# VITA-Group/Open-L2O

Hardware: AMD Instinct MI355X
Metric: unroll-steps/sec (batch x params x T), L2O-DM on Quadratic d=128 (higher is better)
Workload: dtype f32

## Files before the change

include/l2o_abi.h:

```cpp
#ifndef L2O_ABI_H_
#define L2O_ABI_H_

#include <stddef.h>
#include <stdint.h>

#ifdef __cplusplus
extern "C" {
#endif

#define L2O_ABI_VERSION 15

#define L2O_OK 0
#define L2O_ERR_ARG (-1)
#define L2O_ERR_UNSUPPORTED (-2)
#define L2O_ERR_HIP (-3)
#define L2O_ERR_TIMEOUT (-4)

#define L2O_NET_CW 0
#define L2O_NET_RNNPROP 1

#define L2O_PRE_IDENTITY 0
#define L2O_PRE_LOGSIGN 1
#define L2O_PRE_FC_ELU 2

#define L2O_PROB_SIMPLE 0
#define L2O_PROB_QUADRATIC 1
#define L2O_PROB_LASSO 2
#define L2O_PROB_RASTRIGIN 3
#define L2O_PROB_SQUARE_COS 4
#define L2O_PROB_MLP 5
#define L2O_PROB_MNIST_CONV 6
#define L2O_PROB_CIFAR_CONV 7
#define L2O_PROB_LENET 8
#define L2O_PROB_CONFOCAL 9

typedef struct l2o_net_cfg {
  int32_t kind;
  int32_t preprocess;
  int32_t n_layers;
  int32_t hidden;
  int32_t tanh_output;
  int32_t reserved;
  double scale;
  double logsign_k;
  double beta1;
  double beta2;
  uint64_t options;
} l2o_net_cfg;

#define L2O_PROB_W_SHARED 1
#define L2O_PROB_FG_TWO_PASS 2

typedef struct l2o_problem {
  int32_t kind;
  int32_t B_local;
  int32_t B_global;
  int32_t D;
  int32_t M;
  int32_t flags;
  double l1;
  double alpha;
  const float* W;
  const float* y;
  const float* C;
  const float* x_scale;
} l2o_problem;

int l2o_abi_version(void);
const char* l2o_last_error(void);
const char* l2o_build_id(void);
int l2o_last_unroll_form(void);
#define L2O_FORM_UNROLL 1
#define L2O_FORM_UNROLL_PAIR 2
#define L2O_FORM_UNROLL_LDS 5
#define L2O_FORM_UNROLL_CU 6
#define L2O_FORM_UNROLL_CU8 7
#define L2O_FORM_MLP_UNROLL 8
#define L2O_FORM_MLP_UNROLL_HIER 9
#define L2O_FORM_MLP_UNROLL_GENERIC 10
#define L2O_FORM_MLP_XCD 11
#define L2O_FORM_CONFOCAL_UNROLL 12
int l2o_last_unroll_variant(void);
#define L2O_VARIANT(ch, hist, exact, fast, kr, nv) \
  ((ch) | ((hist) << 4) | ((exact) << 5) | ((fast) << 6) | ((kr) << 8) | ((nv) << 12))
#define L2O_VARIANT_CH(w) ((w) & 0xf)
#define L2O_VARIANT_HIST(w) (((w) >> 4) & 1)
#define L2O_VARIANT_EXACT(w) (((w) >> 5) & 1)
#define L2O_VARIANT_FAST(w) (((w) >> 6) & 1)
#define L2O_VARIANT_KR(w) (((w) >> 8) & 7)
#define L2O_VARIANT_NV(w) (((w) >> 12) & 3)

#define L2O_OPT_PAIR 0
#define L2O_OPT_PAIR_PLAIN_STORES 1
#define L2O_OPT_UNROLL_CU 2
#define L2O_OPT_FG_TWO_PASS 3
#define L2O_OPT_MLP_GENERIC 4
#define L2O_OPT_BWD_BLOCKS 5
#define L2O_OPT_BWD_KERNEL 6
#define L2O_OPT_MLP_UNROLL 7
#define L2O_OPT_MLP_XCD_WAVES 8
#define L2O_OPT_EXACT_GATES 9
#define L2O_OPT_WPACK_NO_CLEAR 10
#define L2O_OPT_MLP_HIER 11
#define L2O_OPT_ONE_LDS 12
#define L2O_OPT_PAIR_FAST_LOAD 13
#define L2O_OPT_COUNT_ 14
#define L2O_OPT_FIELD_(o) ((o) == L2O_OPT_ONE_LDS ? L2O_OPT_BWD_BLOCKS : (o) == L2O_OPT_PAIR_FAST_LOAD ? 15 : (o))
#define L2O_OPTW(o, v) ((uint64_t)(8u | ((unsigned)(v) & 7u)) << (4 * L2O_OPT_FIELD_(o)))
#define L2O_OPTW_BWD_BLOCKS(n) ((uint64_t)((n) > 4095 ? 4095 : (n)) << 48)

int32_t l2o_coresident_workgroups(void* scratch, void* stream);

size_t l2o_wpack_floats(const l2o_net_cfg* cfg);
int l2o_wpack_host(const l2o_net_cfg* cfg,
                   const float* w_gates1, const float* b_gates1,
                   const float* w_gates2, const float* b_gates2,
                   const float* w_lin, const float* b_lin,
                   const float* w_fc, const float* b_fc,
                   float* wpack_out);

size_t l2o_state_floats(int64_t B, int64_t D);
int l2o_state_pack(const float* h1, const float* c1, const float* h2, const float* c2,
                   float* st, int64_t B, int64_t D, void* stream);
int l2o_state_unpack(const float* st, float* h1, float* c1, float* h2, float* c2,
                     int64_t B, int64_t D, void* stream);

int l2o_problem_fg(const l2o_problem* prob, const float* x ,
                   float* f_part , float* g ,
                   void* stream);

int l2o_problem_hvp(const l2o_problem* prob, const float* x , const float* u ,
                    float* out , float* scratch, void* stream);

#define L2O_MLP_GENERIC 1
typedef struct l2o_mlp {
  int32_t n_in;
  int32_t n_hidden;
  int32_t n_out;
  int32_t batch;
  int32_t activation;
  int32_t n_data;
  int32_t flags;
  int32_t reserved;
  const float* images;
  const int32_t* labels;
} l2o_mlp;
size_t l2o_mlp_scratch_floats(const l2o_mlp* mlp);
int l2o_mlp_fg(const l2o_mlp* mlp, const int32_t* indices ,
               const float* w1 , const float* b1 ,
               const float* w2 , const float* b2 ,
               float* loss , float* gw1, float* gb1, float* gw2, float* gb2,
               float* scratch , void* stream);

typedef struct l2o_mlp_deep {
  int32_t n_in, n_out, batch, activation , n_data, n_hidden_layers;
  int32_t hidden[3];
  int32_t reserved;
  const float* images;
  const int32_t* labels;
} l2o_mlp_deep;
size_t l2o_mlp_deep_scratch_floats(const l2o_mlp_deep* mlp);
int l2o_mlp_deep_fg(const l2o_mlp_deep* mlp, const int32_t* indices , const float* const* w,
                    float* loss , float* const* g, float* scratch , void* stream);

typedef struct l2o_mnist_conv {
  int32_t batch;
  int32_t n_data;
  int32_t batch_norm;
  int32_t flags;
  const float* images;
  const int32_t* labels;
} l2o_mnist_conv;
size_t l2o_mnist_conv_scratch_floats(const l2o_mnist_conv* conv);
int l2o_mnist_conv_fg(const l2o_mnist_conv* conv, const int32_t* indices ,
                      const float* const* w, float* loss , float* const* g,
                      float* scratch , void* stream);

typedef struct l2o_cifar_conv {
  int32_t batch;
  int32_t n_data;
  int32_t batch_norm;
  int32_t flags;
  const float* images;
  const int32_t* labels;
} l2o_cifar_conv;
size_t l2o_cifar_conv_scratch_floats(const l2o_cifar_conv* conv);
int l2o_cifar_conv_fg(const l2o_cifar_conv* conv, const int32_t* indices ,
                      const float* const* w, float* loss , float* const* g,
                      float* scratch , void* stream);

typedef struct l2o_lenet {
  int32_t batch;
  int32_t n_data;
  int32_t batch_norm;
  int32_t flags;
  const float* images;
  const int32_t* labels;
} l2o_lenet;
size_t l2o_lenet_scratch_floats(const l2o_lenet* net);
int l2o_lenet_fg(const l2o_lenet* net, const int32_t* indices ,
                 const float* const* w, float* loss , float* const* g,
                 float* scratch , void* stream);

typedef struct l2o_confocal {
  int32_t batch;
  int32_t num_points;
  int32_t roi[3];
  int32_t inference;
  int32_t flags;
  const float* img;
} l2o_confocal;
size_t l2o_confocal_scratch_floats(const l2o_confocal* net);
int l2o_confocal_fg(const l2o_confocal* net, const float* const* theta, const float* const* sim,
                    float* loss , float* const* g,
                    float* scratch , void* stream);

int l2o_mlp_unroll_supported(const l2o_net_cfg* cfg, const l2o_mlp* mlp, void* stream);
size_t l2o_mlp_unroll_workspace_bytes(const l2o_mlp* mlp);
int l2o_mlp_unroll(const l2o_net_cfg* cfg, const float* wpack , const l2o_mlp* mlp,
                   const int32_t* indices, float* const* x, float* const* st, float* const* m, float* const* v,
                   const float* const* x_scale, int32_t T, int32_t step0, float* fx, void* workspace, void* stream);
typedef struct l2o_mlp_hist {
  float* st[4];
  float* g[4];
  float* m[4];
  float* v[4];
} l2o_mlp_hist;
int l2o_mlp_unroll_record(const l2o_net_cfg* cfg, const float* wpack , const l2o_mlp* mlp,
                          const int32_t* indices, float* const* x, float* const* st, float* const* m, float* const* v,
                          const float* const* x_scale, int32_t T, int32_t step0, float* fx, const l2o_mlp_hist* hist,
                          void* workspace, void* stream);

typedef struct l2o_mlp_instance {
  const int32_t* indices;
  float* x[4];
  float* st[4];
  float* m[4];
  float* v[4];
  const float* x_scale[4];
  float* fx;
} l2o_mlp_instance;
int l2o_mlp_unroll_multi_supported(const l2o_net_cfg* cfg, const l2o_mlp* mlp, int32_t n_inst, void* stream);
size_t l2o_mlp_unroll_multi_workspace_bytes(const l2o_mlp* mlp, int32_t n_inst);
int l2o_mlp_unroll_multi(const l2o_net_cfg* cfg, const float* wpack , const l2o_mlp* mlp,
                         const l2o_mlp_instance* inst , int32_t n_inst, int32_t T, int32_t step0,
                         void* workspace, void* stream);
int l2o_mlp_unroll_multi_record(const l2o_net_cfg* cfg, const float* wpack , const l2o_mlp* mlp,
                                const l2o_mlp_instance* inst , int32_t n_inst, int32_t T, int32_t step0,
                                const l2o_mlp_hist* hist , void* workspace, void* stream);

int l2o_cwlstm_step(const l2o_net_cfg* cfg, const float* wpack ,
                    const float* g , float* m, float* v ,
                    double pow1, double pow2,
                    float* st , float* x ,
                    int64_t B, int64_t D, void* stream);

typedef struct l2o_gen_net {
  int32_t n_layers;
  int32_t hidden[3];
  int32_t in_dim;
  int32_t direct_inputs;
  const float* w_gates[3];
  const float* b_gates[3];
  const float* w_lin;
  const float* b_lin;
  const float* w_fc;
  const float* b_fc;
} l2o_gen_net;
size_t l2o_gen_state_floats(const l2o_gen_net* net, int64_t N);
int l2o_cwlstm_step_generic(const l2o_net_cfg* cfg ,
                            const l2o_gen_net* net, const float* g ,
                            const float* m_tilde ,
                            float* m, float* v ,
                            double pow1, double pow2, float* state ,
                            float* x , int64_t N, void* stream);

typedef struct l2o_gen_bwd_io {
  const float* g;
  const float* m;
  const float* v;
  const float* st_prev;
  const float* dx_next;
  const float* carry_in;
  float* carry_out;
  float* act[3];
  float* dz[3];
  float* tc;
  float* h_last;
  float* dd;
  float* feats;
  float* du;
  float* dg;
} l2o_gen_bwd_io;
int l2o_cwlstm_bwd_step_generic(const l2o_net_cfg* cfg, const l2o_gen_net* net, const l2o_gen_bwd_io* io, double pow1,
                                double pow2, int64_t N, void* stream);

typedef struct l2o_step_seg {
  const float* g;
  float* m;
  float* v;
  float* st;
  float* x;
  int64_t B, D;
  float* st_out;
  float* m_out;
  float* v_out;
} l2o_step_seg;
int l2o_cwlstm_step_multi(const l2o_net_cfg* cfg, const float* wpack , const l2o_step_seg* segs,
                          int32_t nseg, double pow1, double pow2, void* stream);

typedef struct l2o_net_weights {
  const float *w_gates1, *b_gates1, *w_gates2, *b_gates2, *w_lin, *b_lin, *w_fc, *b_fc;
  const float* wpack;
} l2o_net_weights;
typedef struct l2o_bwd_io {
  const float* g;
  const float* m;
  const float* v;
  const float* st_prev;
  const float* dx_next;
  const float* carry_in;
  float* carry_out;
  float* act1;
  float* dz1;
  float* act2;
  float* dz2;
  float* h2;
  float* dd;
  float* feats;
  float* du;
  int64_t a_stride;
  int64_t b_stride;
  float* dg;
} l2o_bwd_io;
int l2o_cwlstm_bwd_step(const l2o_net_cfg* cfg, const l2o_net_weights* w, const l2o_bwd_io* io,
                        double pow1, double pow2, int64_t B, int64_t D, void* stream);

typedef struct l2o_bwd_seg {
  const float* g;
  const float* m;
  const float* v;
  const float* st_prev;
  const float* dx_next;
  int64_t B, D;
} l2o_bwd_seg;
int l2o_cwlstm_bwd_multi(const l2o_net_cfg* cfg, const l2o_net_weights* w, const l2o_bwd_seg* segs, int32_t nseg,
                         const float* carry_in, float* carry_out, float* A, float* Bm,
                         double pow1, double pow2, void* stream);

typedef struct l2o_bwd_unroll_seg {
  int64_t B, D;
  const float* g_final;
} l2o_bwd_unroll_seg;
int l2o_cwlstm_bwd_unroll(const l2o_net_cfg* cfg, const l2o_net_weights* w, const l2o_bwd_unroll_seg* segs,
                          int32_t nseg, const float* const* table, int32_t T, int64_t step0,
                          const float* carry_in, float* carry_out, float* A, float* Bm, void* stream);
int l2o_cwlstm_bwd_unroll_compact(const l2o_net_cfg* cfg, const l2o_net_weights* w, const l2o_bwd_unroll_seg* segs,
                                  int32_t nseg, const float* const* table, int32_t T, int64_t step0,
                                  const float* carry_in, float* carry_out, float* Ac ,
                                  float* Bm , void* stream);

size_t l2o_atb_workspace_bytes(int64_t R, int32_t KA, int32_t KB);
int l2o_atb(const float* A, const float* B, int64_t R, int32_t KA, int32_t KB, float* out, void* workspace, void* stream);
int32_t l2o_cwlstm_wgrad_dims(const l2o_net_cfg* cfg, int32_t* KA, int32_t* KB);
int l2o_cwlstm_wgrad(const l2o_net_cfg* cfg, const float* A, const float* Bm, int64_t R, float* G ,
                     void* workspace, void* stream);
int l2o_cwlstm_wgrad_compact(const l2o_net_cfg* cfg, const float* Ac, const float* Bm, int32_t T, int64_t rows,
                             float* G , void* workspace, void* stream);

int l2o_adam_step(float* w, float* m, float* v, const float* g, int64_t n, float lr_t, double beta1,
                  double beta2, double epsilon, void* stream);
int l2o_adam_step_guarded(float* w, float* m, float* v, const float* g, int64_t n, float lr_t, double beta1,
                          double beta2, double epsilon, const void* unroll_workspace, void* stream);
int l2o_adam_step_gather(float* w, float* m, float* v, const float* G, const int32_t* map, int64_t n, float lr_t,
                         double beta1, double beta2, double epsilon, const void* unroll_workspace, void* stream);
int l2o_wpack_device(const l2o_net_cfg* cfg, const l2o_net_weights* w, float* wpack_out ,
                     void* stream);

size_t l2o_unroll_workspace_bytes(const l2o_net_cfg* cfg, const l2o_problem* prob, int32_t T);
int l2o_unroll(const l2o_net_cfg* cfg, const float* wpack ,
               const l2o_problem* prob, float* x ,
               float* st , float* m, float* v,
               int32_t T, int32_t step0,
               float* fx_part , void* workspace, void* stream);
typedef struct l2o_unroll_hist {
  float* st;
  float* g;
  float* m;
  float* v;
  float* g_final;
} l2o_unroll_hist;
int l2o_unroll_record(const l2o_net_cfg* cfg, const float* wpack ,
                      const l2o_problem* prob, float* x, float* st, float* m, float* v,
                      int32_t T, int32_t step0, float* fx_part, void* workspace,
                      const l2o_unroll_hist* hist, void* stream);
#define L2O_UNROLL_ZERO_STATE 1
int l2o_unroll_reduce(const l2o_net_cfg* cfg, const float* wpack , const l2o_problem* prob,
                      const float* x0 , float* x, float* st, float* m, float* v, int32_t T,
                      int32_t step0, int32_t flags, float* fx_part, float* fx , void* workspace,
                      const l2o_unroll_hist* hist, void* stream);
int l2o_unroll_workspace_init(void* workspace, size_t bytes, void* stream);
int64_t l2o_unroll_workspace_layout(const l2o_net_cfg* cfg, const l2o_problem* prob);
int l2o_unroll_status(const void* workspace_header_host );
int l2o_unroll_supported(const l2o_net_cfg* cfg, const l2o_problem* prob);
int l2o_unroll_record_supported(const l2o_net_cfg* cfg, const l2o_problem* prob);

int l2o_reduce_fx(const float* fx_part, int32_t T1, int32_t B_local, int32_t B_global,
                  float* fx , void* stream);

int l2o_suffix_sums(const float* const* g , const float* g_final, float* out, int64_t n, int32_t T,
                    void* stream);
size_t l2o_colsum_scratch_floats(int64_t batch, int32_t cols);
int l2o_colsum(const float* A, int64_t batch, int64_t rows, int32_t cols, float* out ,
               int32_t accumulate, float* scratch, void* stream);
int l2o_lincomb(float* out, const float* a, float ca, const float* b, float cb, const float* c, float cc, int64_t n,
                void* stream);
int l2o_rnnprop_input_adjoint(const float* Bm, int64_t ldb, int32_t du_col, int32_t H, const float* w_fc,
                              const float* g, const float* m, const float* v, double pow1, double pow2,
                              double beta1, double beta2, float* dm, float* dv, float* dg, int64_t n, void* stream);

#ifdef __cplusplus
}
#endif
#endif
```

open_l2o_amd/_abi.py:

```python
from __future__ import annotations

import ctypes as C
import os

_HERE = os.path.dirname(os.path.abspath(__file__))
LIB_PATH = os.environ.get("L2O_HIP_LIB") or os.path.join(_HERE, "libl2o_hip.so")

L2O_ABI_VERSION = 15
L2O_OK, L2O_ERR_ARG, L2O_ERR_UNSUPPORTED, L2O_ERR_HIP, L2O_ERR_TIMEOUT = 0, -1, -2, -3, -4

NET_CW, NET_RNNPROP = 0, 1
PRE_IDENTITY, PRE_LOGSIGN, PRE_FC_ELU = 0, 1, 2
PROB_SIMPLE, PROB_QUADRATIC, PROB_LASSO, PROB_RASTRIGIN, PROB_SQUARE_COS, PROB_MLP = 0, 1, 2, 3, 4, 5
PROB_MNIST_CONV = 6
PROB_CIFAR_CONV = 7
PROB_LENET = 8
PROB_CONFOCAL = 9
PROB_VGG16 = 10
PROB_NAS = 11

OPT_PAIR, OPT_PAIR_PLAIN_STORES, OPT_UNROLL_CU, OPT_FG_TWO_PASS, OPT_MLP_GENERIC, OPT_BWD_BLOCKS, OPT_BWD_KERNEL, \
    OPT_MLP_UNROLL, OPT_MLP_XCD_WAVES, OPT_EXACT_GATES, OPT_WPACK_NO_CLEAR, OPT_MLP_HIER, OPT_ONE_LDS, \
    OPT_PAIR_FAST_LOAD = range(14)
OPT_DEFAULTS = {OPT_PAIR: 1, OPT_PAIR_PLAIN_STORES: 1, OPT_UNROLL_CU: 1, OPT_FG_TWO_PASS: 0, OPT_MLP_GENERIC: 0,
                OPT_BWD_BLOCKS: 0, OPT_BWD_KERNEL: 0, OPT_MLP_UNROLL: 1, OPT_MLP_XCD_WAVES: 0, OPT_EXACT_GATES: 0,
                OPT_WPACK_NO_CLEAR: 0, OPT_MLP_HIER: 1, OPT_ONE_LDS: 1, OPT_PAIR_FAST_LOAD: 1}
FORM_NAMES = {1: "k_unroll", 2: "k_unroll_pair", 5: "k_unroll_lds", 6: "k_unroll_cu", 7: "k_unroll_cu8",
              8: "k_mlp_unroll (flat all-reduce)", 9: "k_mlp_unroll (XCD-hierarchical all-reduce)", 10: "k_mlp_unroll (generic loops)",
              11: "k_mlp_xcd (one optimizee instance per XCD)", 12: "k_cf_unroll (one workgroup per batch row)",
              13: "k_cf_unroll (several instances per launch: one workgroup per row of every instance)"}
FORMS_WITH_EXCHANGE = (2, 8, 9, 10, 11)
PROB_FG_TWO_PASS = 2
MLP_GENERIC = 1
_options = {}
OPTION_NAMES = {"pair": OPT_PAIR, "pair_plain_stores": OPT_PAIR_PLAIN_STORES, "unroll_cu": OPT_UNROLL_CU,
                "fg_two_pass": OPT_FG_TWO_PASS, "mlp_generic": OPT_MLP_GENERIC, "bwd_blocks": OPT_BWD_BLOCKS,
                "bwd_kernel": OPT_BWD_KERNEL, "mlp_unroll": OPT_MLP_UNROLL, "exact_gates": OPT_EXACT_GATES,
                "mlp_hier": OPT_MLP_HIER, "one_lds": OPT_ONE_LDS, "mlp_xcd_waves": OPT_MLP_XCD_WAVES,
                "pair_fast_load": OPT_PAIR_FAST_LOAD}
if os.environ.get("L2O_EXACT_GATES"):
    _options[OPT_EXACT_GATES] = 1
for _item in filter(None, os.environ.get("L2O_OPTIONS", "").split(",")):
    _name, _, _val = _item.partition("=")
    if _name.strip() not in OPTION_NAMES:
        raise ValueError("L2O_OPTIONS: unknown option %r (known: %s)" % (_name, ", ".join(sorted(OPTION_NAMES))))
    _options[OPTION_NAMES[_name.strip()]] = int(_val)


def set_option(opt, value):
    if opt not in OPT_DEFAULTS:
        raise ValueError("unknown option %r" % (opt,))
    old = get_option(opt)
    value = int(value)
    if value == OPT_DEFAULTS[opt]:
        _options.pop(opt, None)
    else:
        if not 0 <= value <= (4095 if opt == OPT_BWD_BLOCKS else 7):
            raise ValueError("option %d: value %d out of range" % (opt, value))
        _options[opt] = value
    return old


class option_scope(object):

    def __init__(self, settings):
        self.settings = dict(settings)

    def __enter__(self):
        self.old = {o: set_option(o, v) for o, v in self.settings.items()}
        return self

    def __exit__(self, *exc):
        for o, v in self.old.items():
            set_option(o, v)
        return False


def get_option(opt):
    if opt not in OPT_DEFAULTS:
        return -1
    return _options.get(opt, OPT_DEFAULTS[opt])


def options_word():
    w = 0
    for o, v in _options.items():
        if o == OPT_BWD_BLOCKS:
            w |= (v & 0xfff) << 48
        else:
            w |= (8 | (v & 7)) << (4 * {OPT_ONE_LDS: OPT_BWD_BLOCKS, OPT_PAIR_FAST_LOAD: 15}.get(o, o))
    return w


class NetCfg(C.Structure):
    _fields_ = [
        ("kind", C.c_int32), ("preprocess", C.c_int32), ("n_layers", C.c_int32),
        ("hidden", C.c_int32), ("tanh_output", C.c_int32), ("reserved", C.c_int32),
        ("scale", C.c_double), ("logsign_k", C.c_double),
        ("beta1", C.c_double), ("beta2", C.c_double), ("options", C.c_uint64),
    ]


class Problem(C.Structure):
    _fields_ = [
        ("kind", C.c_int32), ("B_local", C.c_int32), ("B_global", C.c_int32),
        ("D", C.c_int32), ("M", C.c_int32), ("flags", C.c_int32),
        ("l1", C.c_double), ("alpha", C.c_double),
        ("W", C.c_void_p), ("y", C.c_void_p), ("C", C.c_void_p), ("x_scale", C.c_void_p),
    ]


class Mlp(C.Structure):
    _fields_ = [
        ("n_in", C.c_int32), ("n_hidden", C.c_int32), ("n_out", C.c_int32), ("batch", C.c_int32),
        ("activation", C.c_int32), ("n_data", C.c_int32), ("flags", C.c_int32), ("reserved", C.c_int32),
        ("images", C.c_void_p), ("labels", C.c_void_p),
    ]


class MlpHist(C.Structure):
    _fields_ = [("st", C.c_void_p * 4), ("g", C.c_void_p * 4), ("m", C.c_void_p * 4), ("v", C.c_void_p * 4)]


class MlpDeep(C.Structure):
    _fields_ = [("n_in", C.c_int32), ("n_out", C.c_int32), ("batch", C.c_int32), ("activation", C.c_int32),
                ("n_data", C.c_int32), ("n_hidden_layers", C.c_int32), ("hidden", C.c_int32 * 3), ("reserved", C.c_int32),
                ("images", C.c_void_p), ("labels", C.c_void_p)]


class ImageNet(C.Structure):
    _fields_ = [("batch", C.c_int32), ("n_data", C.c_int32), ("batch_norm", C.c_int32), ("flags", C.c_int32),
                ("images", C.c_void_p), ("labels", C.c_void_p)]


class MnistConv(ImageNet):
    """struct l2o_mnist_conv"""


class CifarConv(ImageNet):
    """struct l2o_cifar_conv"""


class Lenet(ImageNet):
    """struct l2o_lenet"""


class Nas(ImageNet):
    """struct l2o_nas (include/l2o_nas_abi.h)"""


class Confocal(C.Structure):
    _fields_ = [("batch", C.c_int32), ("num_points", C.c_int32), ("roi", C.c_int32 * 3), ("inference", C.c_int32),
                ("flags", C.c_int32), ("img", C.c_void_p)]


CONFOCAL_MAX_VARS = 49


class ConfocalHist(C.Structure):
    _fields_ = [("st", C.c_void_p * CONFOCAL_MAX_VARS), ("g", C.c_void_p * CONFOCAL_MAX_VARS),
                ("m", C.c_void_p * CONFOCAL_MAX_VARS), ("v", C.c_void_p * CONFOCAL_MAX_VARS)]


CONFOCAL_MAX_INSTANCES = 32


class ConfocalInstance(C.Structure):
    _fields_ = [(n, C.c_void_p * CONFOCAL_MAX_VARS) for n in ("x", "st", "m", "v", "x_scale", "sim")] + \
               [("img", C.c_void_p), ("fx", C.c_void_p)]


class MlpInstance(C.Structure):
    _fields_ = [("indices", C.c_void_p), ("x", C.c_void_p * 4), ("st", C.c_void_p * 4), ("m", C.c_void_p * 4),
                ("v", C.c_void_p * 4), ("x_scale", C.c_void_p * 4), ("fx", C.c_void_p)]


class Vgg16(C.Structure):
    _fields_ = [("batch", C.c_int32), ("n_data", C.c_int32), ("flags", C.c_int32), ("channels", C.c_int32 * 5),
                ("images", C.c_void_p), ("labels", C.c_void_p)]


STEP_FG = ((MlpDeep, "l2o_mlp_deep"), (MnistConv, "l2o_mnist_conv"), (CifarConv, "l2o_cifar_conv"), (Lenet, "l2o_lenet"),
           (Confocal, "l2o_confocal"), (Vgg16, "l2o_vgg16"), (Nas, "l2o_nas"))


class GenNet(C.Structure):
    _fields_ = [("n_layers", C.c_int32), ("hidden", C.c_int32 * 3), ("in_dim", C.c_int32), ("direct_inputs", C.c_int32),
                ("w_gates", C.c_void_p * 3), ("b_gates", C.c_void_p * 3), ("w_lin", C.c_void_p), ("b_lin", C.c_void_p),
                ("w_fc", C.c_void_p), ("b_fc", C.c_void_p)]


class GenBwdIO(C.Structure):
    _fields_ = [(n, C.c_void_p) for n in ("g", "m", "v", "st_prev", "dx_next", "carry_in", "carry_out")] + \
               [("act", C.c_void_p * 3), ("dz", C.c_void_p * 3)] + \
               [(n, C.c_void_p) for n in ("tc", "h_last", "dd", "feats", "du", "dg")]


class KlstmNet(C.Structure):
    _fields_ = [("kw", C.c_int32), ("kh", C.c_int32), ("n_layers", C.c_int32), ("hidden", C.c_int32 * 2),
                ("preprocess", C.c_int32), ("tanh_output", C.c_int32), ("flags", C.c_int32), ("logsign_k", C.c_double),
                ("scale", C.c_double), ("w_gates", C.c_void_p * 2), ("b_gates", C.c_void_p * 2), ("w_lin", C.c_void_p),
                ("b_lin", C.c_void_p)]


class KlstmBwdIO(C.Structure):
    _fields_ = [(n, C.c_void_p) for n in ("g", "st_prev", "dx_next", "carry_in", "carry_out")] + \
               [("act", C.c_void_p * 2), ("dz", C.c_void_p * 2)] + [(n, C.c_void_p) for n in ("tc", "h_last", "dd")]


class NetWeights(C.Structure):
    _fields_ = [(n, C.c_void_p) for n in ("w_gates1", "b_gates1", "w_gates2", "b_gates2", "w_lin", "b_lin",
                                          "w_fc", "b_fc", "wpack")]


class BwdIO(C.Structure):
    _fields_ = [(n, C.c_void_p) for n in ("g", "m", "v", "st_prev", "dx_next", "carry_in", "carry_out", "act1",
                                          "dz1", "act2", "dz2", "h2", "dd", "feats", "du")] + \
               [("a_stride", C.c_int64), ("b_stride", C.c_int64), ("dg", C.c_void_p)]


UNROLL_ZERO_STATE = 1
PROB_W_SHARED = 1


class StepSeg(C.Structure):
    _fields_ = [("g", C.c_void_p), ("m", C.c_void_p), ("v", C.c_void_p), ("st", C.c_void_p), ("x", C.c_void_p),
                ("B", C.c_int64), ("D", C.c_int64), ("st_out", C.c_void_p), ("m_out", C.c_void_p), ("v_out", C.c_void_p)]


class BwdSeg(C.Structure):
    _fields_ = [(n, C.c_void_p) for n in ("g", "m", "v", "st_prev", "dx_next")] + [("B", C.c_int64), ("D", C.c_int64)]


class BwdUnrollSeg(C.Structure):
    _fields_ = [("B", C.c_int64), ("D", C.c_int64), ("g_final", C.c_void_p)]


class UnrollHist(C.Structure):
    _fields_ = [(n, C.c_void_p) for n in ("st", "g", "m", "v", "g_final")]


def _step_fg(pairs):
    out = {}
    for struct, stem in pairs:
        out[stem + "_fg"] = (C.c_int, [C.POINTER(struct)] + [C.c_void_p] * 6)
        out[stem + "_scratch_floats"] = (C.c_size_t, [C.POINTER(struct)])
    return out


def _prototypes():
    P, vp, i32, i64, dbl, flt, I, Z = C.POINTER, C.c_void_p, C.c_int32, C.c_int64, C.c_double, C.c_float, C.c_int, C.c_size_t
    cfg, prob, mlp, conf = P(NetCfg), P(Problem), P(Mlp), P(Confocal)
    bwd_unroll = [cfg, P(NetWeights), P(BwdUnrollSeg), i32, vp, i32, i64, vp, vp, vp, vp, vp]
    return {
        "l2o_abi.h": {
            "l2o_abi_version": (I, []),
            "l2o_last_error": (C.c_char_p, []),
            "l2o_build_id": (C.c_char_p, []),
            "l2o_last_unroll_form": (I, []),
            "l2o_last_unroll_variant": (I, []),
            "l2o_coresident_workgroups": (i32, [vp, vp]),
            "l2o_wpack_floats": (Z, [cfg]),
            "l2o_wpack_host": (I, [cfg] + [vp] * 9),
            "l2o_state_floats": (Z, [i64, i64]),
            "l2o_state_pack": (I, [vp, vp, vp, vp, vp, i64, i64, vp]),
            "l2o_state_unpack": (I, [vp, vp, vp, vp, vp, i64, i64, vp]),
            "l2o_problem_fg": (I, [prob, vp, vp, vp, vp]),
            "l2o_problem_hvp": (I, [prob, vp, vp, vp, vp, vp]),
            "l2o_mlp_fg": (I, [mlp] + [vp] * 12),
            "l2o_mlp_scratch_floats": (Z, [mlp]),
            "l2o_mlp_unroll": (I, [cfg, vp, mlp, vp, vp, vp, vp, vp, vp, i32, i32, vp, vp, vp]),
            "l2o_mlp_unroll_record": (I, [cfg, vp, mlp, vp, vp, vp, vp, vp, vp, i32, i32, vp, P(MlpHist), vp, vp]),
            "l2o_mlp_unroll_supported": (I, [cfg, mlp, vp]),
            "l2o_mlp_unroll_workspace_bytes": (Z, [mlp]),
            "l2o_mlp_unroll_multi": (I, [cfg, vp, mlp, P(MlpInstance), i32, i32, i32, vp, vp]),
            "l2o_mlp_unroll_multi_record": (I, [cfg, vp, mlp, P(MlpInstance), i32, i32, i32, P(MlpHist), vp, vp]),
            "l2o_mlp_unroll_multi_supported": (I, [cfg, mlp, i32, vp]),
            "l2o_mlp_unroll_multi_workspace_bytes": (Z, [mlp, i32]),
            **_step_fg(STEP_FG[:5]),
            "l2o_cwlstm_step": (I, [cfg, vp, vp, vp, vp, dbl, dbl, vp, vp, i64, i64, vp]),
            "l2o_cwlstm_step_multi": (I, [cfg, vp, P(StepSeg), i32, dbl, dbl, vp]),
            "l2o_cwlstm_step_generic": (I, [cfg, P(GenNet), vp, vp, vp, vp, dbl, dbl, vp, vp, i64, vp]),
            "l2o_cwlstm_bwd_step_generic": (I, [cfg, P(GenNet), P(GenBwdIO), dbl, dbl, i64, vp]),
            "l2o_gen_state_floats": (Z, [P(GenNet), i64]),
            "l2o_cwlstm_bwd_step": (I, [cfg, P(NetWeights), P(BwdIO), dbl, dbl, i64, i64, vp]),
            "l2o_cwlstm_bwd_multi": (I, [cfg, P(NetWeights), P(BwdSeg), i32, vp, vp, vp, vp, dbl, dbl, vp]),
            "l2o_cwlstm_bwd_unroll": (I, bwd_unroll),
            "l2o_cwlstm_bwd_unroll_compact": (I, bwd_unroll),
            "l2o_cwlstm_wgrad_compact": (I, [cfg, vp, vp, i32, i64, vp, vp, vp]),
            "l2o_unroll": (I, [cfg, vp, prob, vp, vp, vp, vp, i32, i32, vp, vp, vp]),
            "l2o_unroll_record": (I, [cfg, vp, prob, vp, vp, vp, vp, i32, i32, vp, vp, P(UnrollHist), vp]),
            "l2o_unroll_reduce": (I, [cfg, vp, prob, vp, vp, vp, vp, vp, i32, i32, i32, vp, vp, vp, P(UnrollHist), vp]),
            "l2o_unroll_workspace_init": (I, [vp, Z, vp]),
            "l2o_unroll_workspace_layout": (i64, [cfg, prob]),
            "l2o_cwlstm_wgrad": (I, [cfg, vp, vp, i64, vp, vp, vp]),
            "l2o_cwlstm_wgrad_dims": (i32, [cfg, P(i32), P(i32)]),
            "l2o_unroll_supported": (I, [cfg, prob]),
            "l2o_unroll_record_supported": (I, [cfg, prob]),
            "l2o_adam_step": (I, [vp, vp, vp, vp, i64, flt, dbl, dbl, dbl, vp]),
            "l2o_adam_step_guarded": (I, [vp, vp, vp, vp, i64, flt, dbl, dbl, dbl, vp, vp]),
            "l2o_adam_step_gather": (I, [vp, vp, vp, vp, vp, i64, flt, dbl, dbl, dbl, vp, vp]),
            "l2o_wpack_device": (I, [cfg, P(NetWeights), vp, vp]),
            "l2o_unroll_workspace_bytes": (Z, [cfg, prob, i32]),
            "l2o_unroll_status": (I, [vp]),
            "l2o_reduce_fx": (I, [vp, i32, i32, i32, vp, vp]),
            "l2o_atb": (I, [vp, vp, i64, i32, i32, vp, vp, vp]),
            "l2o_atb_workspace_bytes": (Z, [i64, i32, i32]),
            "l2o_suffix_sums": (I, [vp, vp, vp, i64, i32, vp]),
            "l2o_colsum": (I, [vp, i64, i64, i32, vp, i32, vp, vp]),
            "l2o_colsum_scratch_floats": (Z, [i64, i32]),
            "l2o_lincomb": (I, [vp, vp, flt, vp, flt, vp, flt, i64, vp]),
            "l2o_rnnprop_input_adjoint": (I, [vp, i64, i32, i32, vp, vp, vp, vp, dbl, dbl, dbl, dbl, vp, vp, vp, i64, vp]),
        },
        "l2o_confocal_unroll_abi.h": {
            "l2o_confocal_unroll": (I, [cfg, vp, conf, vp, vp, vp, vp, vp, vp, i32, i32, vp, vp, vp]),
            "l2o_confocal_unroll_record": (I, [cfg, vp, conf, vp, vp, vp, vp, vp, vp, i32, i32, vp, P(ConfocalHist), vp, vp]),
            "l2o_confocal_unroll_supported": (I, [cfg, conf, vp]),
            "l2o_confocal_unroll_scratch_floats": (Z, [conf, i32]),
        },
        "l2o_confocal_multi_abi.h": {
            "l2o_confocal_unroll_multi": (I, [cfg, vp, conf, P(ConfocalInstance), i32, i32, i32, vp, vp]),
            "l2o_confocal_unroll_multi_record": (I, [cfg, vp, conf, P(ConfocalInstance), i32, i32, i32, P(ConfocalHist), vp, vp]),
            "l2o_confocal_unroll_multi_supported": (I, [cfg, conf, i32, vp]),
            "l2o_confocal_unroll_multi_scratch_floats": (Z, [conf, i32, i32]),
        },
        "l2o_mlp_hvp_abi.h": {
            "l2o_mlp_hvp": (I, [P(MlpDeep)] + [vp] * 6),
            "l2o_mlp_hvp_scratch_floats": (Z, [P(MlpDeep)]),
        },
        "l2o_vgg16_abi.h": _step_fg(STEP_FG[5:6]),
        "l2o_nas_abi.h": _step_fg(STEP_FG[6:7]),
        "l2o_klstm_abi.h": {
            "l2o_klstm_supported": (I, [P(KlstmNet)]),
            "l2o_klstm_state_floats": (Z, [P(KlstmNet), i64]),
            "l2o_klstm_step": (I, [P(KlstmNet), vp, vp, vp, vp, i64, vp]),
            "l2o_klstm_bwd_step": (I, [P(KlstmNet), P(KlstmBwdIO), i64, vp]),
        },
    }


PROTOTYPES = _prototypes()
SYMBOLS, CONFOCAL_UNROLL_SYMBOLS, CONFOCAL_MULTI_SYMBOLS, MLP_HVP_SYMBOLS, VGG16_SYMBOLS, NAS_SYMBOLS, KLSTM_SYMBOLS = (
    tuple(PROTOTYPES[h]) for h in ("l2o_abi.h", "l2o_confocal_unroll_abi.h", "l2o_confocal_multi_abi.h", "l2o_mlp_hvp_abi.h",
                                   "l2o_vgg16_abi.h", "l2o_nas_abi.h", "l2o_klstm_abi.h"))


class L2OError(RuntimeError):
    def __init__(self, code, msg):
        super().__init__("libl2o_hip error %d: %s" % (code, msg))
        self.code = code


class L2OUnsupported(L2OError):
    """L2O_ERR_UNSUPPORTED: no fused kernel for this configuration."""


class L2OPartnerTimeout(L2OError):
    """L2O_ERR_TIMEOUT (l2o_unroll_status): a workgroup of a kernel that exchanges data with partner workgroups gave up
    waiting -- that launch's outputs are invalid.  Recoverable: the host re-runs the unroll on an exchange-free form."""


def source_build_id():
    import glob
    import hashlib
    csrc = os.path.join(_HERE, "csrc")
    names = ["Makefile"] + \
        [os.path.basename(p) for ext in ("*.hip", "*.h") for p in glob.glob(os.path.join(csrc, ext))] + \
        ["../../include/" + os.path.basename(p) for p in glob.glob(os.path.join(csrc, "../../include/*.h"))]
    h = hashlib.sha256()
    try:
        for n in sorted(names):
            with open(os.path.join(csrc, n), "rb") as f:
                h.update(f.read())
    except OSError:
        return None
    return h.hexdigest()[:16]


_lib = None


def build_id():
    return lib().l2o_build_id().decode("ascii", "replace")


def last_unroll_form():
    w = int(lib().l2o_last_unroll_form())
    return FORM_NAMES.get(w & 0xff), w >> 8


def last_unroll_variant():
    w = int(lib().l2o_last_unroll_variant())
    return {"CH": w & 0xf, "HIST": (w >> 4) & 1, "EXACT": (w >> 5) & 1, "FAST": (w >> 6) & 1, "KR": (w >> 8) & 7,
            "NV": (w >> 12) & 3}


def declare(library):
    missing = [name for protos in PROTOTYPES.values() for name in protos if not hasattr(library, name)]
    if missing:
        raise RuntimeError("open_l2o_amd: %s has no %s: the library is stale (built from older sources) -- rebuild it with "
                           "`make -C open_l2o_amd/csrc`" % (LIB_PATH, ", ".join(missing)))
    for protos in PROTOTYPES.values():
        for name, (restype, argtypes) in protos.items():
            fn = getattr(library, name)
            fn.restype, fn.argtypes = restype, argtypes
    return library


def lib():
    global _lib
    if _lib is not None:
        return _lib
    if not os.path.exists(LIB_PATH):
        raise RuntimeError(
            "open_l2o_amd: %s is missing -- build it with `python -c 'import __graft_entry__ as g; "
            "g.build()'` or `make -C open_l2o_amd/csrc`.  There is no CPU fallback." % LIB_PATH)
    L = declare(C.CDLL(LIB_PATH))
    if L.l2o_abi_version() != L2O_ABI_VERSION:
        raise RuntimeError("libl2o_hip.so ABI version %d != binding version %d"
                           % (L.l2o_abi_version(), L2O_ABI_VERSION))
    _lib = L
    return L


def check(rc):
    if rc == L2O_OK:
        return
    msg = lib().l2o_last_error().decode("utf-8", "replace")
    if rc == L2O_ERR_UNSUPPORTED:
        raise L2OUnsupported(rc, msg)
    if rc == L2O_ERR_TIMEOUT:
        raise L2OPartnerTimeout(rc, msg)
    if rc == L2O_ERR_ARG:
        raise ValueError("libl2o_hip: " + msg)
    raise L2OError(rc, msg)
```

open_l2o_amd/_engine.py:

```python
from __future__ import annotations

import collections
import ctypes as C
import dataclasses
from typing import Optional

import numpy as np
import torch

from . import _abi


@dataclasses.dataclass
class NetSpec:
    kind: int
    preprocess: int
    layers: tuple
    scale: float = 1.0
    tanh_output: bool = False
    logsign_k: float = 0.0
    beta1: float = 0.95
    beta2: float = 0.95

    @property
# ... 76 lines not shown
    """problems.NAS (struct l2o_nas): images [n_data, 3072] (32x32x3)"""


@dataclasses.dataclass
class Vgg16Desc:
    batch: int
    channels: tuple
    images: torch.Tensor
    labels: torch.Tensor


@dataclasses.dataclass
class ConfocalDesc:
    batch: int
    num_points: int
    roi: tuple
    img: torch.Tensor = None


StepOptimizee = collections.namedtuple("StepOptimizee", "method desc struct stem scratch nvars sampled")
STEP_OPTIMIZEES = {
    _abi.PROB_MLP: StepOptimizee("mlp_deep_fg", MlpDeepDesc, _abi.MlpDeep, "l2o_mlp_deep", "_mlp_deep_scratch",
                                 lambda d: 2 * len(d.hidden) + 2, True),
    _abi.PROB_MNIST_CONV: StepOptimizee("mnist_conv_fg", MnistConvDesc, _abi.MnistConv, "l2o_mnist_conv",
                                        "_mnist_conv_scratch", lambda d: 10 if d.batch_norm else 6, True),
    _abi.PROB_CIFAR_CONV: StepOptimizee("cifar_conv_fg", CifarConvDesc, _abi.CifarConv, "l2o_cifar_conv",
                                        "_cifar_conv_scratch", lambda d: 10 if d.batch_norm else 6, True),
    _abi.PROB_LENET: StepOptimizee("lenet_fg", LenetDesc, _abi.Lenet, "l2o_lenet", "_lenet_scratch",
                                   lambda d: 14 if d.batch_norm else 10, True),
    _abi.PROB_CONFOCAL: StepOptimizee("confocal_fg", ConfocalDesc, _abi.Confocal, "l2o_confocal", "_confocal_scratch",
                                      lambda d: 6 * d.num_points + 1, False),
    _abi.PROB_VGG16: StepOptimizee("vgg16_fg", Vgg16Desc, _abi.Vgg16, "l2o_vgg16", "_vgg16_scratch", lambda d: 28, True),
    _abi.PROB_NAS: StepOptimizee("nas_fg", NasDesc, _abi.Nas, "l2o_nas", "_nas_scratch",
                                 lambda d: 18 if d.batch_norm else 10, True),
}
_ENTRY_OF_METHOD = {entry.method: entry for entry in STEP_OPTIMIZEES.values()}


def step_optimizee(kind):
    return STEP_OPTIMIZEES.get(kind)


def _ptr(t):
    if t is None:
        return None
    assert t.dtype == torch.float32 and t.is_contiguous(), "C-ABI wants contiguous fp32"
    return C.c_void_p(t.data_ptr())


def _addr(t):
    return 0 if t is None else t.data_ptr()


def _ptr_array(ts, optional=False):
    if ts is None or (optional and all(t is None for t in ts)):
        return None
    return (C.c_void_p * len(ts))(*[None if t is None else _ptr(t).value for t in ts])


def _fill(s, values, checked=False):
    for name, ctype in s._fields_:
        v = values.get(name)
        if v is None:
            continue
        if ctype is C.c_void_p:
            setattr(s, name, _ptr(v).value if checked else v.data_ptr())
        elif issubclass(ctype, C.Array):
            field = getattr(s, name)
            for k, t in enumerate(v):
                if t is not None:
                    field[k] = _ptr(t).value if checked else t.data_ptr()
        else:
            setattr(s, name, int(v))
    return s


def _net_weights(weights):
    return _fill(_abi.NetWeights(), weights)


def _check_confocal(name, d, lists, sim, img):
    nv, inference = 6 * d.num_points + 1, d.img is not None
    if any(len(ts) != nv for ts in lists) or (sim is None) != inference or (sim is not None and len(sim) != nv):
        raise ValueError("%s: %d variables for %d points" % (name, len(lists[0]), d.num_points))
    if any(t.numel() != d.batch for t in lists[0]) \
            or (inference and (img is None or img.numel() != d.batch * int(np.prod(d.roi)))):
        raise ValueError("%s: every variable holds [batch] floats, img [batch, V]" % name)


def _upload_lstm_stack(engine, c, params, layers):
    c.n_layers = len(layers)
    tensors = []
    for l, H in enumerate(layers):
        c.hidden[l] = H
        for name, field in (("w_gates", c.w_gates), ("b_gates", c.b_gates)):
            t = engine.tensor(params["lstm_%d" % (l + 1)][name])
            tensors.append(t)
            field[l] = t.data_ptr()
    wl, bl = engine.tensor(params["linear"]["w"]), engine.tensor(params["linear"]["b"])
    c.w_lin, c.b_lin = wl.data_ptr(), bl.data_ptr()
    return tensors + [wl, bl]


class HipEngine(object):

    name = "hip"

    def __init__(self, device=None):
        if not torch.cuda.is_available():
            raise RuntimeError("open_l2o_amd.HipEngine needs a ROCm GPU (torch.cuda.is_available() is "
                               "False); there is no CPU fallback")
        self.lib = _abi.lib()
        self.device = torch.device(device if device is not None else "cuda:%d" % torch.cuda.current_device())
        self._workspace = None
        self._last_ws = None
        self._mlp_scratch = None
        with torch.cuda.device(self.device):
            scratch = torch.zeros(16, dtype=torch.int32, device=self.device)
            self.coresident_cus = int(self.lib.l2o_coresident_workgroups(C.c_void_p(scratch.data_ptr()), self._stream()))
        if self.coresident_cus <= 0:
            _abi.check(self.coresident_cus)

    def tensor(self, a):
        return torch.as_tensor(np.ascontiguousarray(a, dtype=np.float32)).to(self.device)

    def sample(self, kind, shape, a, b, seed):
        g = self.__dict__.get("_gen")
        if g is None:
            g = self._gen = torch.Generator(device=self.device)
        g.manual_seed(int(seed))
        if kind == "normal":
            t = torch.randn(shape, generator=g, device=self.device, dtype=torch.float32)
            return t.mul_(float(b)).add_(float(a))
        t = torch.rand(shape, generator=g, device=self.device, dtype=torch.float32)
        return t.mul_(float(b) - float(a)).add_(float(a))

    def sample_int(self, out, high, seed):
        g = self.__dict__.get("_gen_int")
        if g is None:
            g = self._gen_int = torch.Generator(device=self.device)
        g.manual_seed(int(seed))
        return torch.randint(0, int(high), tuple(out.shape), generator=g, device=self.device, dtype=torch.int32, out=out)

    def empty_int(self, *shape):
        return torch.empty(*shape, dtype=torch.int32, device=self.device)

    def zeros(self, *shape):
        return torch.zeros(*shape, dtype=torch.float32, device=self.device)

    def empty(self, *shape):
        return torch.empty(*shape, dtype=torch.float32, device=self.device)

    def to_numpy(self, t):
        return t.detach().cpu().numpy()

    def _stream(self):
        return C.c_void_p(torch.cuda.current_stream(self.device).cuda_stream)

    def pack_weights(self, spec: NetSpec, params: dict, key=None):
        host = pack_weights_host(self.lib, spec, params)
        return self.tensor(host) if key is None else self.upload(key, host)

    def pack_weights_device(self, spec: NetSpec, weights: dict, out):
        cc = spec.to_c()
        w = _net_weights(weights)
        w.wpack = None
        sig = (spec.preprocess, tuple(spec.layers), spec.kind)
        if getattr(out, "_l2o_packed", None) == sig:
            cc.options |= (8 | 1) << (4 * _abi.OPT_WPACK_NO_CLEAR)
        _abi.check(self.lib.l2o_wpack_device(C.byref(cc), C.byref(w), _ptr(out), self._stream()))
        try:
            out._l2o_packed = sig
        except AttributeError:
            pass

    def adam_step(self, w, m, v, g, lr_t, beta1, beta2, epsilon, guarded=False):
        ws = self._last_ws if guarded else None
        if ws is not None:
            _abi.check(self.lib.l2o_adam_step_guarded(_ptr(w), _ptr(m), _ptr(v), _ptr(g), int(w.numel()), float(lr_t),
                                                      float(beta1), float(beta2), float(epsilon), C.c_void_p(ws.data_ptr()),
                                                      self._stream()))
        else:
            _abi.check(self.lib.l2o_adam_step(_ptr(w), _ptr(m), _ptr(v), _ptr(g), int(w.numel()), float(lr_t),
                                              float(beta1), float(beta2), float(epsilon), self._stream()))

    def adam_step_gather(self, w, m, v, G, gmap, lr_t, beta1, beta2, epsilon, guarded=False):
        ws = self._last_ws if guarded else None
        _abi.check(self.lib.l2o_adam_step_gather(_ptr(w), _ptr(m), _ptr(v), _ptr(G), C.c_void_p(gmap.data_ptr()),
                                                 int(w.numel()), float(lr_t), float(beta1), float(beta2), float(epsilon),
                                                 None if ws is None else C.c_void_p(ws.data_ptr()), self._stream()))

    def upload(self, key, a):
        a = np.ascontiguousarray(a, dtype=np.float32).reshape(-1)
        ups = self.__dict__.setdefault("_uploads", {})
        ent = ups.get(key)
        if ent is None or ent[0].numel() != a.size:
            ent = ups[key] = [self.empty(a.size), torch.empty(a.size, dtype=torch.float32).pin_memory(), None]
        dev, pin, ev = ent
        if ev is not None:
            ev.synchronize()
        pin.numpy()[:] = a
        dev.copy_(pin, non_blocking=True)
        ent[2] = torch.cuda.Event()
        ent[2].record(torch.cuda.current_stream(self.device))
        return dev

    def state_floats(self, B, D):
        return int(self.lib.l2o_state_floats(B, D))

    def state_alloc(self, B, D):
        return self.zeros(self.state_floats(B, D))

    def state_pack(self, h1, c1, h2, c2, B, D):
        st = self.empty(self.state_floats(B, D))
        _abi.check(self.lib.l2o_state_pack(_ptr(h1), _ptr(c1), _ptr(h2), _ptr(c2), _ptr(st), B, D,
                                           self._stream()))
        return st

    def state_unpack(self, st, B, D, H=20):
        outs = [self.empty(B * D, H) for _ in range(4)]
        _abi.check(self.lib.l2o_state_unpack(_ptr(st), *[_ptr(o) for o in outs], B, D, self._stream()))
        return outs

    def _cprob(self, p: ProblemDesc):
        c = _abi.Problem()
        c.kind, c.B_local, c.B_global, c.D, c.M = p.kind, p.B_local, p.B_global, p.D, p.M
        c.l1, c.alpha = float(p.l1), float(p.alpha)
        c.flags = (_abi.PROB_W_SHARED if p.w_shared else 0) | \
                  (_abi.PROB_FG_TWO_PASS if _abi.get_option(_abi.OPT_FG_TWO_PASS) else 0)
        c.W, c.y, c.C, c.x_scale = _ptr(p.W), _ptr(p.y), _ptr(p.C), _ptr(p.x_scale)
        return c

    def problem_fg(self, p: ProblemDesc, x, f_part, g):
        cp = self._cprob(p)
        _abi.check(self.lib.l2o_problem_fg(C.byref(cp), _ptr(x), _ptr(f_part), _ptr(g), self._stream()))

    def problem_hvp(self, p: ProblemDesc, x, u, out):
        cp = self._cprob(p)
        scr = self._cached_buffer("_hvp_scratch", max(p.B_local, 1))
        _abi.check(self.lib.l2o_problem_hvp(C.byref(cp), _ptr(x), _ptr(u), _ptr(out), _ptr(scr), self._stream()))

    def int_tensor(self, a):
        return torch.as_tensor(np.ascontiguousarray(a, dtype=np.int32)).to(self.device)

    def mlp_fg(self, d: MlpDesc, indices, w1, b1, w2, b2, loss, grads):
        c = self._cmlp(d)
        g = [None] * 4 if grads is None else [_ptr(t) for t in grads]
        scr = self._cached_buffer("_mlp_scratch", int(self.lib.l2o_mlp_scratch_floats(C.byref(c))))
        _abi.check(self.lib.l2o_mlp_fg(C.byref(c), C.c_void_p(indices.data_ptr()), _ptr(w1), _ptr(b1), _ptr(w2),
                                       _ptr(b2), _ptr(loss), *g, _ptr(scr), self._stream()))

    def _cmlp(self, d: MlpDesc):
        c = _abi.Mlp()
        c.n_in, c.n_hidden, c.n_out, c.batch = d.n_in, d.n_hidden, d.n_out, d.batch
        c.activation, c.n_data = d.activation, int(d.images.shape[0])
        c.flags = _abi.MLP_GENERIC if _abi.get_option(_abi.OPT_MLP_GENERIC) else 0
        c.images, c.labels = C.c_void_p(d.images.data_ptr()), C.c_void_p(d.labels.data_ptr())
        return c

    def _cached_buffer(self, attr, n, dtype=torch.float32):
        buf = self.__dict__.get(attr)
        if buf is None or buf.numel() < n:
            buf = (torch.zeros if dtype == torch.uint8 else torch.empty)(n, dtype=dtype, device=self.device)
            setattr(self, attr, buf)
        return buf

    def _step_fg(self, entry, c, d, indices, ws, loss, grads, unsupported, miscount=None):
        n = int(getattr(self.lib, entry.stem + "_scratch_floats")(C.byref(c))) if c is not None else 0
        if not n:
            raise _abi.L2OUnsupported(_abi.L2O_ERR_UNSUPPORTED, unsupported)
        scr = self._cached_buffer(entry.scratch, n)
        if miscount is not None and (len(ws) != entry.nvars(d) or (grads is not None and len(grads) != len(ws))):
            raise ValueError(miscount)
        _abi.check(getattr(self.lib, entry.stem + "_fg")(C.byref(c), C.c_void_p(indices.data_ptr()), _ptr_array(ws),
                                                         _ptr(loss), _ptr_array(grads), _ptr(scr), self._stream()))

    def mlp_deep_fg(self, d: MlpDeepDesc, indices, ws, loss, grads):
        self._step_fg(STEP_OPTIMIZEES[_abi.PROB_MLP], self._cmlp_deep(d, d.hidden), d, indices, ws, loss, grads,
                      "l2o_mlp_deep_fg: unsupported MLP shape %r" % (d.hidden,))

    @staticmethod
    def _cmlp_deep(d, hidden):
        c = _abi.MlpDeep()
        c.n_in, c.n_out, c.batch, c.activation = d.n_in, d.n_out, d.batch, d.activation
        c.n_data, c.n_hidden_layers = int(d.images.shape[0]), len(hidden)
        for k, h in enumerate(hidden[:len(c.hidden)]):
            c.hidden[k] = int(h)
        c.images, c.labels = C.c_void_p(d.images.data_ptr()), C.c_void_p(d.labels.data_ptr())
        return c

    def mlp_hvp(self, d, indices, ws, us, outs):
        hidden = (d.n_hidden,) if isinstance(d, MlpDesc) else tuple(d.hidden)
        c = self._cmlp_deep(d, hidden)
        n = int(self.lib.l2o_mlp_hvp_scratch_floats(C.byref(c)))
        if not n:
            raise _abi.L2OUnsupported(_abi.L2O_ERR_UNSUPPORTED, "l2o_mlp_hvp: unsupported MLP shape %r" % (hidden,))
        if not len(ws) == len(us) == len(outs) == 2 * len(hidden) + 2:
            raise ValueError("l2o_mlp_hvp: %d / %d / %d arrays for hidden layers %r" % (len(ws), len(us), len(outs), hidden))
        scr = self._cached_buffer("_mlp_hvp_scratch", n)
        _abi.check(self.lib.l2o_mlp_hvp(C.byref(c), C.c_void_p(indices.data_ptr()), _ptr_array(ws), _ptr_array(us),
                                        _ptr_array(outs), _ptr(scr), self._stream()))

    def _image_net_fg(self, method, d, indices, ws, loss, grads):
        entry = _ENTRY_OF_METHOD[method]
        c = entry.struct()
        c.batch, c.n_data, c.batch_norm, c.flags = d.batch, int(d.images.shape[0]), 1 if d.batch_norm else 0, 0
# ... 202 lines not shown
            if len(seg) > 7:
                a.st_out, a.m_out, a.v_out = _ptr(seg[7]), _ptr(seg[8]), _ptr(seg[9])
        cc = spec.to_c()
        ccp, n, stream = C.byref(cc), len(segs), self._stream()
        fn, check = self.lib.l2o_cwlstm_step_multi, _abi.check
        keep = (cc, arr, segs)

        def call(wpack_ptr, pow1, pow2, _keep=keep):
            rc = fn(ccp, wpack_ptr, arr, n, pow1, pow2, stream)
            if rc:
                check(rc)
        return call

    class GenNet(object):

        def __init__(self, engine, spec, params, direct=False):
            layers = tuple(int(h) for h in spec.layers)
            c = _abi.GenNet()
            self.tensors = _upload_lstm_stack(engine, c, params, layers)
            c.in_dim = 2 if spec.preprocess == _abi.PRE_LOGSIGN else 1
            if spec.preprocess == _abi.PRE_FC_ELU:
                wf, bf = engine.tensor(params["input_projection"]["w"]), engine.tensor(params["input_projection"]["b"])
                self.tensors += [wf, bf]
                c.w_fc, c.b_fc = wf.data_ptr(), bf.data_ptr()
                c.in_dim = int(wf.shape[1])
            c.direct_inputs = 1 if direct else 0
            self.c, self.layers = c, layers

    def gen_net(self, spec: NetSpec, params: dict, direct=False):
        return HipEngine.GenNet(self, spec, params, direct)

    def gen_state_alloc(self, gen, N):
        return self.zeros(int(self.lib.l2o_gen_state_floats(C.byref(gen.c), int(N))))

    def lstm_step_generic(self, spec: NetSpec, gen, g, m_tilde, m, v, pow1, pow2, st, x, N):
        cc = spec.to_c()
        _abi.check(self.lib.l2o_cwlstm_step_generic(C.byref(cc), C.byref(gen.c), _ptr(g), _ptr(m_tilde), _ptr(m), _ptr(v),
                                                    float(pow1), float(pow2), _ptr(st), _ptr(x), int(N), self._stream()))

    def bwd_step_generic(self, spec: NetSpec, gen, io: dict, pow1, pow2, N):
        c, cc = _fill(_abi.GenBwdIO(), io), spec.to_c()
        _abi.check(self.lib.l2o_cwlstm_bwd_step_generic(C.byref(cc), C.byref(gen.c), C.byref(c), float(pow1), float(pow2),
                                                        int(N), self._stream()))

    class KlstmNet(object):

        def __init__(self, engine, net):
            c = _abi.KlstmNet()
            c.kw, c.kh = net.kernel_shape
            c.preprocess, c.tanh_output, c.flags = int(net.preprocess), int(bool(net.tanh_output)), 0
            c.logsign_k, c.scale = float(net.logsign_k), float(net.scale)
            self.tensors = _upload_lstm_stack(engine, c, net.variables, net.layers)
            self.c = c

    def klstm_net(self, net):
        return HipEngine.KlstmNet(self, net)

    def klstm_step(self, net, g, st_in, st_out, x, N):
        _abi.check(self.lib.l2o_klstm_step(C.byref(net.device_net(self).c), _ptr(g), _ptr(st_in), _ptr(st_out), _ptr(x),
                                           int(N), self._stream()))

    def klstm_bwd_step(self, net, io: dict, N):
        c = _fill(_abi.KlstmBwdIO(), io, checked=True)
        _abi.check(self.lib.l2o_klstm_bwd_step(C.byref(net.device_net(self).c), C.byref(c), int(N), self._stream()))

    def lstm_step(self, spec: NetSpec, wpack, g, m, v, pow1, pow2, st, x, B, D):
        if isinstance(wpack, HipEngine.GenNet):
            return self.lstm_step_generic(spec, wpack, g, None, m, v, pow1, pow2, st, x, B * D)
        cc = spec.to_c()
        _abi.check(self.lib.l2o_cwlstm_step(C.byref(cc), _ptr(wpack), _ptr(g), _ptr(m), _ptr(v),
                                            float(pow1), float(pow2), _ptr(st), _ptr(x), B, D,
                                            self._stream()))

    MAX_STEP_SEGS = 8

    def lstm_step_multi(self, spec: NetSpec, wpack, segs, pow1, pow2):
        if isinstance(wpack, HipEngine.GenNet):
            for seg in segs:
                g, m, v, st, x, B, D = seg[:7]
                if len(seg) > 7 and seg[7] is not None:
                    st_out, m_out, v_out = seg[7:10]
                    st_out.copy_(st)
                    if m is not None:
                        m_out.copy_(m); v_out.copy_(v)
                        m, v = m_out, v_out
                    st = st_out
                self.lstm_step_generic(spec, wpack, g, None, m, v, pow1, pow2, st, x, B * D)
            return
        for i in range(0, len(segs), self.MAX_STEP_SEGS):
            chunk = segs[i:i + self.MAX_STEP_SEGS]
            arr = (_abi.StepSeg * len(chunk))()
            for a, seg in zip(arr, chunk):
                g, m, v, st, x, B, D = seg[:7]
                a.g, a.m, a.v, a.st, a.x, a.B, a.D = _ptr(g), _ptr(m), _ptr(v), _ptr(st), _ptr(x), B, D
                if len(seg) > 7:
                    a.st_out, a.m_out, a.v_out = _ptr(seg[7]), _ptr(seg[8]), _ptr(seg[9])
            cc = spec.to_c()
            _abi.check(self.lib.l2o_cwlstm_step_multi(C.byref(cc), _ptr(wpack), arr, len(chunk), float(pow1),
                                                      float(pow2), self._stream()))

    def bwd_step(self, spec: NetSpec, weights: dict, io: dict, pow1, pow2, B, D):
        cc = spec.to_c()
        w = _net_weights(weights)
        b = _fill(_abi.BwdIO(), io)
        _abi.check(self.lib.l2o_cwlstm_bwd_step(C.byref(cc), C.byref(w), C.byref(b), float(pow1), float(pow2),
                                                B, D, self._stream()))

    def bwd_multi(self, spec: NetSpec, weights: dict, segs, carry_in, carry_out, A, Bm, pow1, pow2):
        cc = spec.to_c()
        w = _net_weights(weights)
        arr = (_abi.BwdSeg * len(segs))()
        for a, sg in zip(arr, segs):
            _fill(a, sg)
        _abi.check(self.lib.l2o_cwlstm_bwd_multi(C.byref(cc), C.byref(w), arr, len(segs), _ptr(carry_in),
                                                 _ptr(carry_out), _ptr(A), _ptr(Bm), float(pow1), float(pow2),
                                                 self._stream()))

    bwd_unroll_any_d = True

    bwd_unroll_compact = True

    def bwd_unroll(self, spec: NetSpec, weights: dict, panels, T, step0, A, Bm, carry_in=None, carry_out=None,
                   table=None, compact=False):
        cc = spec.to_c()
        w = _net_weights(weights)
        if table is None:
            table = self.bwd_table(panels, T)
        arr = (_abi.BwdUnrollSeg * len(panels))()
        for a, pn in zip(arr, panels):
            a.B, a.D = int(pn["B"]), int(pn["D"])
            a.g_final = None if pn.get("g_final") is None else pn["g_final"].data_ptr()
        fn = self.lib.l2o_cwlstm_bwd_unroll_compact if compact else self.lib.l2o_cwlstm_bwd_unroll
        _abi.check(fn(C.byref(cc), C.byref(w), arr, len(panels), C.c_void_p(table.data_ptr()), int(T),
                      int(step0), _ptr(carry_in), _ptr(carry_out), _ptr(A), _ptr(Bm), self._stream()))
        self._bwd_table = table

    def bwd_table(self, panels, T):
        ptr = lambda x: 0 if x is None else x.data_ptr()
        rows = []
        for t in range(T):
            for pn in panels:
                rows.append([ptr(pn["gs"][t]), ptr(pn["ms"][t]) if pn.get("ms") else 0, ptr(pn["vs"][t]) if pn.get("vs") else 0,
                             ptr(pn["sts"][t]), ptr(pn["dxs"][t]) if pn.get("dxs") else 0])
        return torch.tensor(rows, dtype=torch.int64).to(self.device, non_blocking=False)

    def unroll_supported(self, spec: NetSpec, p: ProblemDesc, record=False):
        cc, cp = spec.to_c(), self._cprob(p)
        fn = self.lib.l2o_unroll_record_supported if record else self.lib.l2o_unroll_supported
        return bool(fn(C.byref(cc), C.byref(cp)))

    def unroll(self, spec: NetSpec, wpack, p: ProblemDesc, x, st, m, v, T, step0, fx_part, hist=None, fx=None, x0=None,
               zero_state=False):
        assert fx is not None or (x0 is None and not zero_state)
        cc, cp = spec.to_c(), self._cprob(p)
        nbytes = int(self.lib.l2o_unroll_workspace_bytes(C.byref(cc), C.byref(cp), int(T)))
        ws = None
        if nbytes:
            old = self._workspace
            layout = int(self.lib.l2o_unroll_workspace_layout(C.byref(cc), C.byref(cp)))
            ws = self._cached_buffer("_workspace", nbytes, torch.uint8)
            if ws is old and layout != self.__dict__.get("_ws_layout"):
                _abi.check(self.lib.l2o_unroll_workspace_init(C.c_void_p(ws.data_ptr()), ws.numel(), self._stream()))
            self._ws_layout = layout
        self._last_ws = ws
        wsp = None if ws is None else C.c_void_p(ws.data_ptr())
        flags = _abi.UNROLL_ZERO_STATE if zero_state else 0
        h = None if hist is None else _fill(_abi.UnrollHist(), hist)
        if fx is not None:
            _abi.check(self.lib.l2o_unroll_reduce(C.byref(cc), _ptr(wpack), C.byref(cp), _ptr(x0), _ptr(x), _ptr(st), _ptr(m),
                                                  _ptr(v), int(T), int(step0), flags, _ptr(fx_part), _ptr(fx),
                                                  wsp, None if h is None else C.byref(h), self._stream()))
        elif hist is None:
            _abi.check(self.lib.l2o_unroll(C.byref(cc), _ptr(wpack), C.byref(cp), _ptr(x), _ptr(st), _ptr(m),
                                           _ptr(v), int(T), int(step0), _ptr(fx_part), wsp, self._stream()))
        else:
            _abi.check(self.lib.l2o_unroll_record(C.byref(cc), _ptr(wpack), C.byref(cp), _ptr(x), _ptr(st), _ptr(m),
                                                  _ptr(v), int(T), int(step0), _ptr(fx_part), wsp, C.byref(h),
                                                  self._stream()))

    def prepared_unroll(self, spec: NetSpec, wpack, p: ProblemDesc, x, st, m, v, T, fx_part, x0, zero_state):
        cc, cp = spec.to_c(), self._cprob(p)
        nbytes = int(self.lib.l2o_unroll_workspace_bytes(C.byref(cc), C.byref(cp), int(T)))
        ws, layout = None, None
        if nbytes:
            ws = self._workspace
            layout = int(self.lib.l2o_unroll_workspace_layout(C.byref(cc), C.byref(cp)))
            if ws is None or ws.numel() < nbytes or layout != self.__dict__.get("_ws_layout"):
                return None
        wsp = None if ws is None else C.c_void_p(ws.data_ptr())
        flags = _abi.UNROLL_ZERO_STATE if zero_state else 0
        args_a = (C.byref(cc), _ptr(wpack), C.byref(cp), _ptr(x0), _ptr(x), _ptr(st), _ptr(m), _ptr(v), int(T))
        args_b = (flags, _ptr(fx_part))
        fn, check, stream = self.lib.l2o_unroll_reduce, _abi.check, self._stream
        keep = (cc, cp, wpack, p, x, st, m, v, fx_part, x0, ws)
        eng = self

        def call(fx, step0=1, _keep=keep):
            if eng._workspace is not ws or (ws is not None and eng.__dict__.get("_ws_layout") != layout):
                return False
            rc = fn(*args_a, int(step0), *args_b, C.c_void_p(fx.data_ptr()), wsp, None, stream())
            if rc:
                check(rc)
            eng._last_ws = ws
            return True
        return call

    def prefetch_unroll_status(self):
        ws = self._last_ws
        if ws is None:
            return
        pin = self.__dict__.get("_status_pin")
        if pin is None:
            pin = self._status_pin = torch.zeros(4, dtype=torch.uint8).pin_memory()
        pin.copy_(ws[:4], non_blocking=True)
        self._status_pending = ws

    def last_unroll_form(self):
        return _abi.last_unroll_form()

    def last_unroll_variant(self):
        return _abi.last_unroll_variant()

    def last_unroll_exchanges(self):
        return (int(self.lib.l2o_last_unroll_form()) & 0xff) in _abi.FORMS_WITH_EXCHANGE

    def last_loop_ticks(self):
        ws = self._last_ws
        if ws is None:
            return None
        loop, total = (int(v) for v in ws[16:32].view(torch.int64).cpu())
        return (loop, total) if loop > 0 and total >= loop else None

    def unroll_status_tensor(self):
        ws = self._last_ws
        return None if ws is None else ws[:4].view(torch.int32)

    def inject_unroll_fault(self, on=True):
        for ws in (self._workspace, self.__dict__.get("_mlp_ws")):
            if ws is not None:
                ws[8:12].view(torch.int32).fill_(1 if on else 0)

    def check_unroll_status(self):
        ws = self._last_ws
        if ws is not None:
            if self.__dict__.pop("_status_pending", None) is ws:
                hdr = self._status_pin.numpy().tobytes()
            else:
                hdr = ws[:4].cpu().numpy().tobytes()
            if hdr != b"\0\0\0\0":
                ws.zero_()
            _abi.check(self.lib.l2o_unroll_status(hdr))

    def _atb_workspace(self, R, KA, KB):
        n = int(self.lib.l2o_atb_workspace_bytes(int(R), int(KA), int(KB)))
        return self._cached_buffer("_atb_ws", (n + 3) // 4)

    def atb(self, A, B):
        R, KA = A.shape
        KB = B.shape[1]
        ws = self._atb_workspace(R, KA, KB)
        out = self.empty(KA, KB)
        _abi.check(self.lib.l2o_atb(_ptr(A), _ptr(B), int(R), int(KA), int(KB), _ptr(out), _ptr(ws), self._stream()))
        return out

    def wgrad(self, spec: NetSpec, A, B):
        R, KA = A.shape
        KB = B.shape[1]
        cc = spec.to_c()
        ka, kb = C.c_int32(0), C.c_int32(0)
        _abi.check(self.lib.l2o_cwlstm_wgrad_dims(C.byref(cc), C.byref(ka), C.byref(kb)))
        assert (ka.value, kb.value) == (KA, KB), ((ka.value, kb.value), (KA, KB))
        ws = self._atb_workspace(R, KA, KB)
        out = self.empty(KA, KB)
        _abi.check(self.lib.l2o_cwlstm_wgrad(C.byref(cc), _ptr(A), _ptr(B), int(R), _ptr(out), _ptr(ws), self._stream()))
        return out

    def wgrad_compact(self, spec: NetSpec, Ac, Bm):
        T, R, KB = Bm.shape
        cc = spec.to_c()
        ka, kb = C.c_int32(0), C.c_int32(0)
        _abi.check(self.lib.l2o_cwlstm_wgrad_dims(C.byref(cc), C.byref(ka), C.byref(kb)))
        KA = ka.value
        assert kb.value == KB and tuple(Ac.shape) == (T + 1, R, KA - 40), (tuple(Ac.shape), (T + 1, R, KA - 40), KB)
        ws = self._atb_workspace(T * R, KA, KB)
        out = self.empty(KA, KB)
        _abi.check(self.lib.l2o_cwlstm_wgrad_compact(C.byref(cc), _ptr(Ac), _ptr(Bm), int(T), int(R), _ptr(out), _ptr(ws),
                                                     self._stream()))
        return out

    def suffix_sums(self, gs, g_final, out):
        T, n = len(gs), g_final.numel()
        if T == 0:
            return out
        ptrs = tuple(g.data_ptr() for g in gs)
        cache = self.__dict__.setdefault("_suffix_tables", {})
        table = cache.get(ptrs)
        if table is None:
            if len(cache) >= 16:
                cache.clear()
            pin = torch.tensor(ptrs, dtype=torch.int64).pin_memory()
            table = torch.empty(T, dtype=torch.int64, device=self.device)
            table.copy_(pin, non_blocking=True)
            cache[ptrs] = table
            self._suffix_pin = pin
        _abi.check(self.lib.l2o_suffix_sums(C.c_void_p(table.data_ptr()), _ptr(g_final), _ptr(out), n, T, self._stream()))
        return out

    def colsum(self, A, out=None, accumulate=False):
        A3 = A if A.dim() == 3 else A.unsqueeze(0)
        assert A3.is_contiguous()
        b, rows, cols = A3.shape
        if out is None:
            out = self.empty(b, cols) if A.dim() == 3 else self.empty(cols)
        scr = self._cached_buffer("_colsum_scratch", int(self.lib.l2o_colsum_scratch_floats(b, cols)))
        _abi.check(self.lib.l2o_colsum(_ptr(A3), b, rows, cols, _ptr(out), 1 if accumulate else 0, _ptr(scr), self._stream()))
        return out

    def lincomb(self, out, a, ca=1.0, b=None, cb=0.0, c=None, cc=0.0):
        _abi.check(self.lib.l2o_lincomb(_ptr(out), _ptr(a), float(ca), _ptr(b), float(cb), _ptr(c), float(cc), out.numel(),
                                        self._stream()))
        return out

    def rnnprop_input_adjoint(self, Bm, du_col, H, w_fc, g, m, v, pow1, pow2, beta1, beta2, dm, dv, dg):
        n = g.numel()
        _abi.check(self.lib.l2o_rnnprop_input_adjoint(_ptr(Bm), int(Bm.stride(0)), int(du_col), int(H), _ptr(w_fc), _ptr(g),
                                                      _ptr(m), _ptr(v), float(pow1), float(pow2), float(beta1), float(beta2),
                                                      _ptr(dm), _ptr(dv), _ptr(dg), n, self._stream()))

    def reduce_fx(self, fx_part, T1, B_local, B_global, fx):
        _abi.check(self.lib.l2o_reduce_fx(_ptr(fx_part), int(T1), int(B_local), int(B_global), _ptr(fx),
                                          self._stream()))

    def synchronize(self):
        torch.cuda.synchronize(self.device)


def pack_weights_host(lib, spec: NetSpec, params: dict):
    cc = spec.to_c()
    n = int(lib.l2o_wpack_floats(C.byref(cc)))
    if n == 0:
        raise _abi.L2OUnsupported(
            _abi.L2O_ERR_UNSUPPORTED,
            "no HIP kernel for an optimizer net with layers=%r (implemented: (20, 20) and ())" % (spec.layers,))
    out = np.zeros((n,), np.float32)

    def arr(mod, var):
        if mod not in params:
            return None
        return np.ascontiguousarray(params[mod][var], dtype=np.float32)

    keep = [arr("lstm_1", "w_gates"), arr("lstm_1", "b_gates"), arr("lstm_2", "w_gates"),
            arr("lstm_2", "b_gates"), arr("linear", "w"), arr("linear", "b"),
            arr("input_projection", "w"), arr("input_projection", "b")]
    ptrs = [None if a is None else a.ctypes.data_as(C.c_void_p) for a in keep]
    _abi.check(lib.l2o_wpack_host(C.byref(cc), *ptrs, out.ctypes.data_as(C.c_void_p)))
    return out


_default_engine = None


def default_engine():
    global _default_engine
    if _default_engine is None:
        _default_engine = HipEngine()
    return _default_engine


def set_default_engine(engine):
    global _default_engine
    _default_engine = engine
```

open_l2o_amd/csrc/l2o_unroll.hip:

```cpp
#include "l2o_host.h"
#include "l2o_step.h"
#include "l2o_problem_fg.h"
#include "l2o_unroll.h"
#include "l2o_unroll_pair.h"
#include "l2o_unroll_lds.h"
#include "l2o_unroll_cu.h"
#include "l2o_unroll_cu8.h"
#include "l2o_ilp_kernels.h"

__global__ void k_combine_halves(const float* __restrict__ fx_half, float* __restrict__ fx_part, int nb, int nparts,
                                 float inv_bg, float* __restrict__ fx, unsigned long long* __restrict__ xbuf, long xwords,
                                 PairWs* ws, int b0, int B_local);
__global__ void k_coresident_probe(unsigned* ctr, unsigned* min_seen);

static int check_problem(const l2o_problem* p) {
  if (!p) return fail(L2O_ERR_ARG, "problem is NULL");
  if (p->B_local <= 0 || p->B_global < p->B_local || p->D <= 0)
    return fail(L2O_ERR_ARG, "bad problem sizes B_local=%d B_global=%d D=%d", p->B_local, p->B_global, p->D);
  switch (p->kind) {
    case L2O_PROB_SIMPLE: return L2O_OK;
    case L2O_PROB_QUADRATIC:
    case L2O_PROB_LASSO:
      if (!p->W || !p->y || p->M <= 0) return fail(L2O_ERR_ARG, "problem needs W, y and M > 0");
      if (p->kind == L2O_PROB_QUADRATIC && p->M != p->D) return fail(L2O_ERR_ARG, "quadratic needs M == D");
      return L2O_OK;
    case L2O_PROB_RASTRIGIN:
    case L2O_PROB_SQUARE_COS:
      if (!p->W || !p->y || !p->C || p->M != p->D)
        return fail(L2O_ERR_ARG, "rastrigin / square_cos need W, y, C and M == D");
      return L2O_OK;
    default: return fail(L2O_ERR_UNSUPPORTED, "problem kind %d has no HIP kernel", p->kind);
  }
}

struct UnrollGeom { int CH, nw; size_t lds; };
static bool unroll_geom(const l2o_problem* p, UnrollGeom* g) {
  const int D = p->D, M = p->M;
  g->nw = tiles_per_problem(D);
  if (g->nw > 8 || M > 16 * g->nw) return false;
  const int need = g->nw;
  g->CH = need <= 1 ? 1 : (need <= 2 ? 2 : (need <= 4 ? 4 : 8));
  const int SQ = 16 * g->CH, S = SQ + 16;
  g->lds = sizeof(float) * (2 * (size_t)SQ * S + 3 * (size_t)SQ + 8);
  return g->lds <= 160 * 1024;
}

static int pair_chunk(const l2o_problem* p, const UnrollGeom& g, hipStream_t s) {
  if (!opt(L2O_OPT_PAIR) || g.CH < 2) return 0;
  const int cap = coresident_cus(s) / 2;
  if (p->B_local <= cap) return p->B_local;
  if (cap < 8) return 0;
  const int n = (p->B_local + cap - 1) / cap;
  const int chunk = (((p->B_local + n - 1) / n) + 7) & ~7;
  return chunk <= cap ? chunk : (cap & ~7);
}
struct PairLayout { size_t xbuf_off, xbuf_bytes, fxh_off, total; int npg; size_t lds; };
static PairLayout pair_layout(const l2o_problem* p, const UnrollGeom& g, int T) {
  PairLayout L;
  const int SQ = 16 * g.CH;
  L.npg = SQ;
  L.xbuf_off = sizeof(PairWs);
  L.xbuf_bytes = (size_t)p->B_local * 2 * 2 * L.npg * sizeof(unsigned long long);
  L.fxh_off = L.xbuf_off + L.xbuf_bytes;
  L.total = L.fxh_off + sizeof(float) * (size_t)(T + 1) * g.CH * p->B_local;
  L.lds = 0;
  return L;
}

template <int PRE, int KIND>
static int launch_unroll_ch(const UnrollArgs& a, const UnrollGeom& g, hipStream_t s, const l2o_problem* prob,
                            void* workspace, float* fx, bool* fx_done) {
  const bool hist = a.hist_st != nullptr;
  int chunk = workspace ? pair_chunk(prob, g, s) : 0;
  {
    const int one_lds = (int)opt(L2O_OPT_ONE_LDS);
#ifdef L2O_LDS_ABL_ANYNW
    const bool shape_ok = g.nw >= 1 && a.pp.M <= 16 * g.nw;
#else
    const bool shape_ok = g.CH == 8 && g.nw >= 5;
#endif
    const bool plain = !(opt(L2O_OPT_EXACT_GATES) && !hist);
    if ((one_lds == 2 || (one_lds == 1 && (chunk == 0 || a.pp.B_local > chunk))) && shape_ok && plain) {
      UnrollArgs al = a;
      al.ticks = workspace ? &reinterpret_cast<PairWs*>(workspace)->ticks : nullptr;
      void (*fl)(UnrollArgs) = hist ? k_unroll_lds<PRE, KIND, true> : k_unroll_lds<PRE, KIND, false>;
      const size_t lds = sizeof(float) * ((size_t)LstmCoreLds<PRE>::kFragWords + 2 * 128 + 8);
      const int rc = launch(fl, dim3(a.pp.B_local), dim3(64 * g.nw), lds, s, al);
      if (rc) return rc;
      note_form(L2O_FORM_UNROLL_LDS);
      note_variant(0, hist, false, false, 0, 0);
      return L2O_OK;
    }
  }
  if (chunk > 0) {
    const PairLayout L = pair_layout(prob, g, a.T);
    UnrollPairArgs pa;
    pa.u = a;
    pa.ws = reinterpret_cast<PairWs*>(workspace);
    pa.xbuf = reinterpret_cast<unsigned long long*>(static_cast<char*>(workspace) + L.xbuf_off);
    pa.fx_half = reinterpret_cast<float*>(static_cast<char*>(workspace) + L.fxh_off);
    pa.use_salt = a.T + 1 < 0xffff ? 1u : 0u;
    pa.plain_stores = opt(L2O_OPT_PAIR_PLAIN_STORES) ? 1u : 0u;
    pa.b0 = 0;
    pa.nb = a.pp.B_local;
    const int B = a.pp.B_local;
    const bool one_launch = chunk >= B;
    const bool exact = opt(L2O_OPT_EXACT_GATES) != 0 && !hist;
    bool fast_launched = false;
    {
      void (*fn)(UnrollPairArgs) = nullptr;
      const size_t dyn_lds = L.lds;
      const int SQ = 16 * g.CH;
      const bool fast = opt(L2O_OPT_PAIR_FAST_LOAD) != 0 && a.pp.M == SQ && a.pp.D == SQ;
      pa.fast_load = fast ? 1u : 0u;
      fast_launched = fast;
#define L2O_PAIR_FN(C)                                                                                       \
  (fast ? (hist ? k_unroll_pair<PRE, KIND, C, true, false, true>                                             \
                : (exact ? k_unroll_pair<PRE, KIND, C, false, true, true> : k_unroll_pair<PRE, KIND, C, false, false, true>)) \
        : (hist ? k_unroll_pair<PRE, KIND, C, true> : (exact ? k_unroll_pair<PRE, KIND, C, false, true> : k_unroll_pair<PRE, KIND, C, false>)))
      switch (g.CH) {
        case 2: fn = L2O_PAIR_FN(2); break;
        case 4: fn = L2O_PAIR_FN(4); break;
        default: fn = L2O_PAIR_FN(8); break;
      }
#undef L2O_PAIR_FN
      for (int b0 = 0; b0 < B; b0 += chunk) {
        pa.b0 = b0;
        pa.nb = B - b0 < chunk ? B - b0 : chunk;
        hipLaunchKernelGGL(fn, dim3((pa.nb + 7) / 8 * 16), dim3(64 * (g.CH / 2)), dyn_lds, s, pa);
        HIP_TRY(hipGetLastError());
        hipLaunchKernelGGL(k_combine_halves, dim3(a.T + 1), dim3(256), 0, s, pa.fx_half, a.fx_part, pa.nb, g.CH,
                           a.pp.inv_bg, one_launch ? fx : nullptr, pa.xbuf, (long)pa.nb * 2 * 2 * L.npg, pa.ws, b0, B);
        HIP_TRY(hipGetLastError());
      }
    }
    note_form(L2O_FORM_UNROLL_PAIR, (B + chunk - 1) / chunk);
    note_variant(g.CH, hist, exact, fast_launched, 0, 0);
    if (fx_done) *fx_done = fx != nullptr && one_launch;
    return L2O_OK;
  }
  void (*fn)(UnrollArgs) = nullptr;
  const bool exact1 = opt(L2O_OPT_EXACT_GATES) != 0 && !hist;
  switch (g.CH) {
    case 1: fn = hist ? k_unroll<PRE, KIND, 1, true> : (exact1 ? k_unroll<PRE, KIND, 1, false, true> : k_unroll<PRE, KIND, 1, false>); break;
    case 2: fn = hist ? k_unroll<PRE, KIND, 2, true> : (exact1 ? k_unroll<PRE, KIND, 2, false, true> : k_unroll<PRE, KIND, 2, false>); break;
    case 4: fn = hist ? k_unroll<PRE, KIND, 4, true> : (exact1 ? k_unroll<PRE, KIND, 4, false, true> : k_unroll<PRE, KIND, 4, false>); break;
    default: fn = hist ? k_unroll<PRE, KIND, 8, true> : k_unroll<PRE, KIND, 8, false>; break;
  }
  const int rc = launch(fn, dim3(a.pp.B_local), dim3(64 * g.nw), g.lds, s, a);
  if (rc) return rc;
  note_form(L2O_FORM_UNROLL);
  note_variant(g.CH, hist, exact1 && g.CH <= 4, false, 0, 0);
  return L2O_OK;
}

template <int PRE>
static int launch_unroll_kind(const UnrollArgs& a, const UnrollGeom& g, int kind, hipStream_t s,
                              const l2o_problem* prob, void* workspace, float* fx, bool* fx_done) {
  switch (kind) {
    case L2O_PROB_QUADRATIC: return launch_unroll_ch<PRE, L2O_PROB_QUADRATIC>(a, g, s, prob, workspace, fx, fx_done);
    case L2O_PROB_LASSO: return launch_unroll_ch<PRE, L2O_PROB_LASSO>(a, g, s, prob, workspace, fx, fx_done);
    case L2O_PROB_RASTRIGIN: return launch_unroll_ch<PRE, L2O_PROB_RASTRIGIN>(a, g, s, prob, workspace, fx, fx_done);
    case L2O_PROB_SQUARE_COS: return launch_unroll_ch<PRE, L2O_PROB_SQUARE_COS>(a, g, s, prob, workspace, fx, fx_done);
    default: return fail(L2O_ERR_UNSUPPORTED, "no fused kernel for problem kind %d", kind);
  }
}

static bool unroll_cu_eligible(const l2o_problem* p) {
  if (!opt(L2O_OPT_UNROLL_CU)) return false;
  if (p->D < 4 || p->D > 512 || (p->D & 3) || p->M <= 0) return false;
  return unroll_cu_layout(p->D).lds + sizeof(float) * bx::kBiasWords <= 160 * 1024;
}
template <int PRE, int KR>
static int launch_unroll_cu8(const UnrollArgs& a, hipStream_t s) {
  const UnrollCu8Layout L = unroll_cu8_layout(a.pp.D, PRE, KR);
  const bool hist = a.hist_st != nullptr;
  void (*fn)(UnrollArgs) = a.pp.D <= 256 ? (hist ? k_unroll_cu8<PRE, 1, KR, true> : k_unroll_cu8<PRE, 1, KR, false>)
                                         : (hist ? k_unroll_cu8<PRE, 2, KR, true> : k_unroll_cu8<PRE, 2, KR, false>);
  note_form(L2O_FORM_UNROLL_CU8);
  note_variant(0, hist, false, false, KR, a.pp.D <= 256 ? 1 : 2);
  return launch(fn, dim3(a.pp.B_local), dim3(kCu8Threads), L.lds, s, a);
}
template <int PRE>
static int launch_unroll_cu(const UnrollArgs& a_in, hipStream_t s) {
  const int form = (int)opt(L2O_OPT_UNROLL_CU);
  const bool hist0 = a_in.hist_st != nullptr;
  auto fits = [&](int kr) { return unroll_cu8_layout(a_in.pp.D, PRE, kr).lds + sizeof(float) * bx::kBiasWords <= 160 * 1024; };
  int KR = 0;
  if (form == 1) {
    KR = hist0 ? 2 : (PRE == L2O_PRE_FC_ELU ? 4 : 3);
    if (hist0 && !fits(2) && PRE != L2O_PRE_FC_ELU) KR = 3;
  } else if (form >= 3 && form <= 5) KR = 7 - form;
  if (KR && fits(KR))
    return KR == 4 ? launch_unroll_cu8<PRE, 4>(a_in, s) : (KR == 3 ? launch_unroll_cu8<PRE, 3>(a_in, s) : launch_unroll_cu8<PRE, 2>(a_in, s));
  const UnrollCuLayout L = unroll_cu_layout(a_in.pp.D);
  const UnrollArgs& a = a_in;
  const bool hist = a.hist_st != nullptr;
  void (*fn)(UnrollArgs) = a.pp.D <= 256 ? (hist ? k_unroll_cu<PRE, 1, true> : k_unroll_cu<PRE, 1, false>)
                                         : (hist ? k_unroll_cu<PRE, 2, true> : k_unroll_cu<PRE, 2, false>);
  note_form(L2O_FORM_UNROLL_CU);
  note_variant(0, hist, false, false, 0, a.pp.D <= 256 ? 1 : 2);
  return launch(fn, dim3(a.pp.B_local), dim3(kCuThreads), L.lds, s, a);
}

extern "C" {

static int launch_problem_fg(const ProbParams& pp, const float* x, float* f_part, float* g, void* stream) {
  const size_t lds = sizeof(float) * ((size_t)((pp.D + 3) & ~3) + ((pp.M + 3) & ~3) + 4 * kFgThreads + kFgWaves);
  if (lds > 160 * 1024) return fail(L2O_ERR_UNSUPPORTED, "problem too large for k_problem_fg (D=%d M=%d)", pp.D, pp.M);
  const bool vec = pp.kind != L2O_PROB_SIMPLE && (pp.D & 3) == 0 && ((uintptr_t)pp.W & 15) == 0;
  if (vec && pp.D >= 64 && pp.D <= 2048 && ((uintptr_t)x & 15) == 0 && (!pp.x_scale || ((uintptr_t)pp.x_scale & 15) == 0) &&
      !pp.w_shared && !opt(L2O_OPT_FG_TWO_PASS)) {
    const size_t lds1 = sizeof(float) * ((size_t)kFgWaves * pp.D + kFgWaves);
    void (*f1)(ProbParams, const float*, float*, float*) =
        pp.D <= 256 ? k_problem_fg1<1> : pp.D <= 512 ? k_problem_fg1<2> : pp.D <= 1024 ? k_problem_fg1<4> : k_problem_fg1<8>;
    return launch(f1, dim3(pp.B_local), dim3(kFgThreads), lds1, (hipStream_t)stream, pp, x, f_part, g);
  }
  void (*fn)(ProbParams, const float*, float*, float*) = vec ? k_problem_fg<true> : k_problem_fg<false>;
  return launch(fn, dim3(pp.B_local), dim3(kFgThreads), lds, (hipStream_t)stream, pp, x, f_part, g);
}

int l2o_problem_fg(const l2o_problem* prob, const float* x, float* f_part, float* g, void* stream) {
  OptScope opt_scope((prob && (prob->flags & L2O_PROB_FG_TWO_PASS)) ? L2O_OPTW(L2O_OPT_FG_TWO_PASS, 1) : 0);
  int rc = check_problem(prob);
  if (rc) return rc;
  if (!x || !f_part) return fail(L2O_ERR_ARG, "l2o_problem_fg: NULL x / f_part");
  return launch_problem_fg(make_prob_params(prob), x, f_part, g, stream);
}

int l2o_problem_hvp(const l2o_problem* prob, const float* x, const float* u, float* out, float* scratch, void* stream) {
  OptScope opt_scope((prob && (prob->flags & L2O_PROB_FG_TWO_PASS)) ? L2O_OPTW(L2O_OPT_FG_TWO_PASS, 1) : 0);
  int rc = check_problem(prob);
  if (rc) return rc;
  if (!x || !u || !out || !scratch) return fail(L2O_ERR_ARG, "l2o_problem_hvp: NULL argument");
  ProbParams pp = make_prob_params(prob);
  pp.hvp = 1;
  rc = launch_problem_fg(pp, u, scratch, out, stream);
  if (rc) return rc;
  if (pp.kind == L2O_PROB_RASTRIGIN || pp.kind == L2O_PROB_SQUARE_COS) {
    const size_t n = (size_t)pp.B_local * pp.D;
    hipLaunchKernelGGL(k_hvp_sep, dim3((unsigned)((n + 255) / 256)), dim3(256), 0, (hipStream_t)stream, pp, x, u, out, n);
    HIP_TRY(hipGetLastError());
  }
  return L2O_OK;
}

int l2o_cwlstm_step_multi(const l2o_net_cfg* cfg, const float* wpack, const l2o_step_seg* segs, int32_t nseg,
                          double pow1, double pow2, void* stream) {
  OptScope opt_scope(cfg_optw(cfg));
  if (!cfg || !wpack || !segs || nseg < 1) return fail(L2O_ERR_ARG, "l2o_cwlstm_step: bad argument");
  if (nseg > kMaxStepSegs) return fail(L2O_ERR_UNSUPPORTED, "l2o_cwlstm_step_multi: at most %d segments", kMaxStepSegs);
  for (int i = 0; i < nseg; ++i)
    if (!segs[i].g || !segs[i].x || segs[i].B <= 0 || segs[i].D <= 0)
      return fail(L2O_ERR_ARG, "l2o_cwlstm_step: bad argument (segment %d)", i);
  const NetParams np = make_net_params(cfg, wpack);
  hipStream_t s = (hipStream_t)stream;
  if (cfg->n_layers == 0) {
    if (cfg->kind != L2O_NET_CW || cfg->preprocess == L2O_PRE_FC_ELU)
      return fail(L2O_ERR_UNSUPPORTED, "layers=() is implemented for CoordinateWiseDeepLSTM only");
    for (int i = 0; i < nseg; ++i) {
      const size_t n = (size_t)segs[i].B * segs[i].D;
      const dim3 grid((unsigned)((n + 255) / 256));
      if (cfg->preprocess == L2O_PRE_LOGSIGN)
        hipLaunchKernelGGL(k_linear_step<L2O_PRE_LOGSIGN>, grid, dim3(256), 0, s, np, segs[i].g, segs[i].x, n);
      else
        hipLaunchKernelGGL(k_linear_step<L2O_PRE_IDENTITY>, grid, dim3(256), 0, s, np, segs[i].g, segs[i].x, n);
    }
    HIP_TRY(hipGetLastError());
    return L2O_OK;
  }
  if (!net_ok_for_mfma(cfg)) return fail(L2O_ERR_UNSUPPORTED, "l2o_cwlstm_step: only layers=(20,20) / () nets");
  StepSegs sg;
  std::memset(&sg, 0, sizeof(sg));
  sg.n = nseg;
  int64_t ntiles = 0;
  for (int i = 0; i < nseg; ++i) {
    if (!segs[i].st) return fail(L2O_ERR_ARG, "l2o_cwlstm_step: NULL state");
    if (cfg->preprocess == L2O_PRE_FC_ELU && (!segs[i].m || !segs[i].v))
      return fail(L2O_ERR_ARG, "l2o_cwlstm_step: RNNProp needs m and v");
    sg.tpp[i] = tiles_per_problem(segs[i].D);
    sg.D[i] = (int)segs[i].D;
    ntiles += segs[i].B * sg.tpp[i];
    if (ntiles > INT32_MAX) return fail(L2O_ERR_UNSUPPORTED, "l2o_cwlstm_step: too many coordinates");
    sg.tile_end[i] = (int)ntiles;
    sg.g[i] = segs[i].g; sg.m[i] = segs[i].m; sg.v[i] = segs[i].v; sg.st[i] = segs[i].st; sg.x[i] = segs[i].x;
    sg.st_out[i] = segs[i].st_out ? segs[i].st_out : segs[i].st;
    sg.m_out[i] = segs[i].m_out ? segs[i].m_out : segs[i].m;
    sg.v_out[i] = segs[i].v_out ? segs[i].v_out : segs[i].v;
  }
  int blocks = (int)((ntiles + 3) / 4);
  if (blocks > 256) blocks = 256;
  const dim3 grid(blocks), block(256);
  const float om1 = (float)(1.0 - pow1), om2 = (float)(1.0 - pow2);
  with_pre(cfg->preprocess, [&](auto pre) { hipLaunchKernelGGL(k_cwlstm_step<decltype(pre)::value>, grid, block, 0, s, np, sg, om1, om2); });
  HIP_TRY(hipGetLastError());
  return L2O_OK;
}

int l2o_cwlstm_step(const l2o_net_cfg* cfg, const float* wpack, const float* g, float* m, float* v, double pow1,
                    double pow2, float* st, float* x, int64_t B, int64_t D, void* stream) {
  OptScope opt_scope(cfg_optw(cfg));
  l2o_step_seg seg;
  std::memset(&seg, 0, sizeof(seg));
  seg.g = g; seg.m = m; seg.v = v; seg.st = st; seg.x = x; seg.B = B; seg.D = D;
  return l2o_cwlstm_step_multi(cfg, wpack, &seg, 1, pow1, pow2, stream);
}

int l2o_unroll_supported(const l2o_net_cfg* cfg, const l2o_problem* prob) {
  OptScope opt_scope(cfg_optw(cfg));
  if (!cfg || !prob || !net_ok_for_mfma(cfg)) return 0;
  if (prob->kind != L2O_PROB_QUADRATIC && prob->kind != L2O_PROB_LASSO && prob->kind != L2O_PROB_RASTRIGIN &&
      prob->kind != L2O_PROB_SQUARE_COS)
    return 0;
  if (prob->D <= 0 || prob->M <= 0) return 0;
  UnrollGeom g;
  return (unroll_geom(prob, &g) || unroll_cu_eligible(prob)) ? 1 : 0;
}

int l2o_unroll_record_supported(const l2o_net_cfg* cfg, const l2o_problem* prob) {
  OptScope opt_scope(cfg_optw(cfg));
  return l2o_unroll_supported(cfg, prob);
}

size_t l2o_unroll_workspace_bytes(const l2o_net_cfg* cfg, const l2o_problem* prob, int32_t T) {
  OptScope opt_scope(cfg_optw(cfg));
  if (!l2o_unroll_supported(cfg, prob) || T < 0) return 0;
  UnrollGeom g;
  if (!unroll_geom(prob, &g) || g.CH < 2) return 0;
  return pair_layout(prob, g, T).total;
}

int l2o_unroll_status(const void* workspace_header_host) {
  if (!workspace_header_host) return L2O_OK;
  const unsigned st = *static_cast<const unsigned*>(workspace_header_host);
  if (st == 0) return L2O_OK;
  if (st == 2)
    return fail(L2O_ERR_TIMEOUT, "l2o_mlp_unroll: a workgroup's all-reduce inputs never arrived (status 2): the persistent "
                             "launch was not fully co-resident (a shared / masked device?); the iterate and LSTM state "
                             "of that launch are invalid.  Run l2o_coresident_workgroups once so that the library "
                             "sizes against what is really available, or switch the fused form off "
                             "(L2O_OPT_MLP_UNROLL = 0 / L2O_NO_MLP_UNROLL=1)");
  return fail(L2O_ERR_TIMEOUT, "l2o_unroll: partner workgroup timed out (status %u): the two halves of a problem were not "
                           "co-resident (a shared / masked device?); the iterate and LSTM state of that launch are "
                           "invalid.  Run l2o_coresident_workgroups once so that the library sizes against what is "
                           "really available, or use one CU per problem (L2O_OPT_PAIR = 0 / L2O_NO_PAIR=1)", st);
}

static int unroll_impl(const l2o_net_cfg* cfg, const float* wpack, const l2o_problem* prob, float* x, float* st,
                       float* m, float* v, int32_t T, int32_t step0, float* fx_part, void* workspace,
                       const l2o_unroll_hist* hist, float* fx, void* stream, const float* x0 = nullptr, int flags = 0);

int l2o_unroll(const l2o_net_cfg* cfg, const float* wpack, const l2o_problem* prob, float* x, float* st, float* m,
               float* v, int32_t T, int32_t step0, float* fx_part, void* workspace, void* stream) {
  OptScope opt_scope(cfg_optw(cfg));
  return unroll_impl(cfg, wpack, prob, x, st, m, v, T, step0, fx_part, workspace, nullptr, nullptr, stream);
}

int l2o_unroll_record(const l2o_net_cfg* cfg, const float* wpack, const l2o_problem* prob, float* x, float* st,
                      float* m, float* v, int32_t T, int32_t step0, float* fx_part, void* workspace,
                      const l2o_unroll_hist* hist, void* stream) {
  OptScope opt_scope(cfg_optw(cfg));
  return unroll_impl(cfg, wpack, prob, x, st, m, v, T, step0, fx_part, workspace, hist, nullptr, stream);
}

int l2o_unroll_reduce(const l2o_net_cfg* cfg, const float* wpack, const l2o_problem* prob, const float* x0, float* x,
                      float* st, float* m, float* v, int32_t T, int32_t step0, int32_t flags, float* fx_part, float* fx,
                      void* workspace, const l2o_unroll_hist* hist, void* stream) {
  OptScope opt_scope(cfg_optw(cfg));
  if (!fx) return fail(L2O_ERR_ARG, "l2o_unroll_reduce: NULL fx");
  if (flags & ~L2O_UNROLL_ZERO_STATE)
    return fail(L2O_ERR_ARG, "l2o_unroll_reduce: unknown flags %d", flags);
  return unroll_impl(cfg, wpack, prob, x, st, m, v, T, step0, fx_part, workspace, hist, fx, stream, x0, flags);
}

int32_t l2o_coresident_workgroups(void* scratch, void* stream) {
  if (!scratch) return fail(L2O_ERR_ARG, "l2o_coresident_workgroups: NULL scratch");
  hipStream_t s = (hipStream_t)stream;
  const int dev = device_ordinal(s);
  if (dev >= 0 && dev < 64) {
    const int m = g_measured_cus[dev].load(std::memory_order_relaxed);
    if (m > 0) return m;
  }
  const int n = device_cu_count(s);
  if (n <= 0) return fail(L2O_ERR_HIP, "l2o_coresident_workgroups: no device");
  unsigned* d = static_cast<unsigned*>(scratch);
  constexpr int kLds = 100 * 1024;
  HIP_TRY(hipFuncSetAttribute(reinterpret_cast<const void*>(k_coresident_probe), hipFuncAttributeMaxDynamicSharedMemorySize, kLds));
  int got = 0;
  for (int pass = 0; pass < 3; ++pass) {
    const unsigned init[2] = {0u, 0xffffffffu};
    HIP_TRY(hipMemcpyAsync(d, init, sizeof(init), hipMemcpyHostToDevice, s));
    hipLaunchKernelGGL(k_coresident_probe, dim3(n), dim3(256), kLds, s, d, d + 1);
    HIP_TRY(hipGetLastError());
    unsigned out[2] = {0u, 0u};
    HIP_TRY(hipMemcpyAsync(out, d, sizeof(out), hipMemcpyDeviceToHost, s));
    HIP_TRY(hipStreamSynchronize(s));
    const int seen = (int)out[1];
    if (seen > got && seen <= n) got = seen;
    if (got == n) break;
  }
  if (got <= 0) got = n;
  if (dev >= 0 && dev < 64) g_measured_cus[dev].store(got, std::memory_order_relaxed);
  return got;
}

int l2o_unroll_workspace_init(void* workspace, size_t bytes, void* stream) {
  if (!workspace && bytes) return fail(L2O_ERR_ARG, "l2o_unroll_workspace_init: NULL workspace");
  if (bytes) HIP_TRY(hipMemsetAsync(workspace, 0, bytes, (hipStream_t)stream));
  return L2O_OK;
}

int64_t l2o_unroll_workspace_layout(const l2o_net_cfg* cfg, const l2o_problem* prob) {
  OptScope opt_scope(cfg_optw(cfg));
  UnrollGeom g;
  if (!cfg || !prob || !l2o_unroll_supported(cfg, prob) || !unroll_geom(prob, &g) || g.CH < 2) return 0;
  return ((int64_t)prob->B_local << 8) | g.CH;
}

static int unroll_impl(const l2o_net_cfg* cfg, const float* wpack, const l2o_problem* prob, float* x, float* st,
                       float* m, float* v, int32_t T, int32_t step0, float* fx_part, void* workspace,
                       const l2o_unroll_hist* hist, float* fx, void* stream, const float* x0, int flags) {
  int rc = check_problem(prob);
  if (rc) return rc;
  if (!cfg || !wpack || !x || !st || !fx_part || T < 0) return fail(L2O_ERR_ARG, "l2o_unroll: bad argument");
  if (hist && (!hist->st || !hist->g || !hist->g_final ||
               (cfg->preprocess == L2O_PRE_FC_ELU && (!hist->m || !hist->v))))
    return fail(L2O_ERR_ARG, "l2o_unroll_record: incomplete history buffers");
  if (!l2o_unroll_supported(cfg, prob))
    return fail(L2O_ERR_UNSUPPORTED, "l2o_unroll: no fused kernel for kind=%d D=%d M=%d net(kind=%d,layers=%d)",
                prob->kind, prob->D, prob->M, cfg->kind, cfg->n_layers);
  UnrollGeom g;
  const bool lds_form = unroll_geom(prob, &g);
  UnrollArgs a;
  a.np = make_net_params(cfg, wpack);
  a.pp = make_prob_params(prob);
  a.x = x; a.st = st; a.m = m; a.v = v; a.fx_part = fx_part;
  a.x_in = x0; a.zero_state = (flags & L2O_UNROLL_ZERO_STATE) ? 1 : 0;
  a.ticks = nullptr;
  a.T = T;
  a.hist_st = hist ? hist->st : nullptr;
  a.hist_g = hist ? hist->g : nullptr;
  a.hist_m = hist ? hist->m : nullptr;
  a.hist_v = hist ? hist->v : nullptr;
  a.hist_gfinal = hist ? hist->g_final : nullptr;
  pow_ff(cfg->beta1, step0, &a.p1_hi, &a.p1_lo);
  pow_ff(cfg->beta2, step0, &a.p2_hi, &a.p2_lo);
  hipStream_t s = (hipStream_t)stream;
  bool fx_done = false;
  rc = L2O_OK;
  if (cfg->preprocess == L2O_PRE_FC_ELU && (!m || !v)) return fail(L2O_ERR_ARG, "l2o_unroll: RNNProp needs m and v");
  if (!lds_form) {
    rc = with_pre(cfg->preprocess, [&](auto pre) { return launch_unroll_cu<decltype(pre)::value>(a, s); });
  } else {
    rc = with_pre(cfg->preprocess, [&](auto pre) {
      return launch_unroll_kind<decltype(pre)::value>(a, g, prob->kind, s, prob, workspace, fx, &fx_done);
    });
  }
  if (rc) return rc;
  if (fx && !fx_done)
    return l2o_reduce_fx(fx_part, T + 1, prob->B_local, prob->B_global, fx, stream);
  return L2O_OK;
}

}
```

open_l2o_amd/csrc/l2o_unroll_pair.h:

```cpp
#pragma once
#include "l2o_lstm_bx3.h"
#include "l2o_params.h"

struct PairWs {
  unsigned status;
  unsigned seq;
  unsigned fault;
  unsigned pad0;
  long long ticks;
  long long ticks_total;
  unsigned pad[8];
  long long phases[16];
};
static_assert(sizeof(PairWs) == 64 + 128, "workspace header layout (include/l2o_abi.h)");

struct UnrollPairArgs {
  UnrollArgs u;
  PairWs* ws;
  unsigned long long* xbuf;
  float* fx_half;
  unsigned use_salt;
  unsigned plain_stores;
  int b0, nb;
  unsigned fast_load;
};

__device__ __forceinline__ unsigned long long pack_granule(float v, unsigned tag) {
  return ((unsigned long long)tag << 32) | (unsigned long long)__float_as_uint(v);
}

template <int N>
__device__ __forceinline__ void lds_read_f4(float4 (&v)[N], const float* p) {
  const unsigned addr = (unsigned)(size_t)(__attribute__((address_space(3))) const char*)p;
  static_assert(N == 1 || N == 2 || N == 4 || N == 8, "");
  if constexpr (N == 1)
    asm volatile("ds_read_b128 %0, %1\n\ts_waitcnt lgkmcnt(0)" : "=&v"(v[0]) : "v"(addr) : "memory");
  if constexpr (N == 2)
    asm volatile("ds_read_b128 %0, %2\n\tds_read_b128 %1, %2 offset:64\n\ts_waitcnt lgkmcnt(0)"
                 : "=&v"(v[0]), "=&v"(v[1]) : "v"(addr) : "memory");
  if constexpr (N == 4)
    asm volatile("ds_read_b128 %0, %4\n\tds_read_b128 %1, %4 offset:64\n\tds_read_b128 %2, %4 offset:128\n\t"
                 "ds_read_b128 %3, %4 offset:192\n\ts_waitcnt lgkmcnt(0)"
                 : "=&v"(v[0]), "=&v"(v[1]), "=&v"(v[2]), "=&v"(v[3]) : "v"(addr) : "memory");
  if constexpr (N == 8)
    asm volatile("ds_read_b128 %0, %8\n\tds_read_b128 %1, %8 offset:64\n\tds_read_b128 %2, %8 offset:128\n\t"
                 "ds_read_b128 %3, %8 offset:192\n\tds_read_b128 %4, %8 offset:256\n\tds_read_b128 %5, %8 offset:320\n\t"
                 "ds_read_b128 %6, %8 offset:384\n\tds_read_b128 %7, %8 offset:448\n\ts_waitcnt lgkmcnt(0)"
                 : "=&v"(v[0]), "=&v"(v[1]), "=&v"(v[2]), "=&v"(v[3]), "=&v"(v[4]), "=&v"(v[5]), "=&v"(v[6]), "=&v"(v[7])
                 : "v"(addr) : "memory");
}

template <int N>
__device__ __forceinline__ void lds_load_f4(l2o::f32x4 (&v)[N], const float* p) {
  const auto* q = reinterpret_cast<const __attribute__((address_space(3))) l2o::f32x4*>(
      (const __attribute__((address_space(3))) float*)p);
#pragma unroll
  for (int m = 0; m < N; ++m) v[m] = q[4 * m];
}
__device__ __forceinline__ void dot4v(const float4 a, const l2o::f32x4 b, float4& acc) {
  acc.x = __builtin_fmaf(a.x, b[0], acc.x);
  acc.y = __builtin_fmaf(a.y, b[1], acc.y);
  acc.z = __builtin_fmaf(a.z, b[2], acc.z);
  acc.w = __builtin_fmaf(a.w, b[3], acc.w);
}

#ifndef L2O_GEMV_PK
#define L2O_GEMV_PK 1
#endif
#ifndef L2O_GEMV_PK_G
#define L2O_GEMV_PK_G L2O_GEMV_PK
#endif
struct Acc4pk { l2o::bx::f32x2 lo, hi; };
__device__ __forceinline__ void dot4pk(const l2o::f32x4 a, const l2o::f32x4 b, Acc4pk& acc) {
  acc.lo = __builtin_elementwise_fma(__builtin_shufflevector(a, a, 0, 1), __builtin_shufflevector(b, b, 0, 1), acc.lo);
  acc.hi = __builtin_elementwise_fma(__builtin_shufflevector(a, a, 2, 3), __builtin_shufflevector(b, b, 2, 3), acc.hi);
}
__device__ __forceinline__ float hsum4pk(const Acc4pk& a) { return (a.lo.x + a.lo.y) + (a.hi.x + a.hi.y); }
__device__ __forceinline__ l2o::f32x4 as_quad(const float4 v) { return l2o::f32x4{v.x, v.y, v.z, v.w}; }
__device__ __forceinline__ void dot4q(const l2o::f32x4 a, const l2o::f32x4 b, float4& acc) {
  acc.x = __builtin_fmaf(a[0], b[0], acc.x);
  acc.y = __builtin_fmaf(a[1], b[1], acc.y);
  acc.z = __builtin_fmaf(a[2], b[2], acc.z);
  acc.w = __builtin_fmaf(a[3], b[3], acc.w);
}

#ifndef L2O_PAIR_LDS_BARRIERS
#define L2O_PAIR_LDS_BARRIERS 0
#endif
#ifdef L2O_PROFILE_PHASES
#define L2O_LAUNCH_MARK(i)                                                                  \
  do {                                                                                      \
    __builtin_amdgcn_sched_barrier(0);                                                      \
    launch_marks[i] = (unsigned)(__builtin_readcyclecounter() - kernel_t0);                 \
    __builtin_amdgcn_sched_barrier(0);                                                      \
  } while (0)
#define L2O_LAUNCH_MARK_LANDED(i)                                                           \
  do {                                                                                      \
    __builtin_amdgcn_sched_barrier(0);                                                      \
    asm volatile("s_waitcnt vmcnt(0) lgkmcnt(0)" ::: "memory");                             \
    L2O_LAUNCH_MARK(i);                                                                     \
  } while (0)
#else
#define L2O_LAUNCH_MARK(i) do {} while (0)
#define L2O_LAUNCH_MARK_LANDED(i) do {} while (0)
#endif

template <int PRE, int KIND, int CH, bool HIST, bool EXACT>
__device__ __forceinline__ void unroll_pair_body_gather(const UnrollPairArgs& pa) {
  const long long kernel_t0 = __builtin_readcyclecounter();
#ifdef L2O_PROFILE_PHASES
  unsigned launch_marks[8] = {0, 0, 0, 0, 0, 0, 0, 0};
#endif
  constexpr int SQ = 16 * CH;
  constexpr int NWH = CH / 2;
  constexpr int NC = 16 * NWH;
  __shared__ __attribute__((aligned(16))) float xs[NC];
  __shared__ __attribute__((aligned(16))) float rs[SQ];
  const UnrollArgs& a = pa.u;
  const ProbParams& pp = a.pp;
  const int D = pp.D, M = pp.M;
  const int tid = threadIdx.x, lane = tid & 63, wv = tid >> 6;
  const int c = lane & 15, q = lane >> 4;
  const int bid = blockIdx.x;
  const unsigned salt = pa.use_salt ? ((pa.ws->seq + 1u) & 0x7fffu) << 16 : 0u;
#ifdef L2O_PROFILE_PHASES
  asm volatile("" ::"s"(salt));
#endif
  L2O_LAUNCH_MARK(0);
  const int half = (bid >> 3) & 1;
  const int bl = ((bid >> 4) << 3) | (bid & 7);
  if (bl >= pa.nb) return;
  const int b = pa.b0 + bl;
  const int tile_in_prob = half * NWH + wv;
  const int gq = q, gr = c;

  const float* Wb = pp.W + (pp.w_shared ? (size_t)0 : (size_t)b * M * D);
  const int col0 = half * NC;
  float4 wr[2][NWH], wt[CH];
#pragma unroll
  for (int p = 0; p < 2; ++p) {
    const int row = (2 * wv + p) * kTile + gr;
#pragma unroll
    for (int m = 0; m < NWH; ++m) {
      float e[4];
#pragma unroll
      for (int k = 0; k < 4; ++k) {
        const int col = col0 + 16 * m + 4 * gq + k;
        e[k] = (row < M && col < D) ? Wb[(size_t)row * D + col] : 0.0f;
      }
      wr[p][m] = make_float4(e[0], e[1], e[2], e[3]);
    }
  }
  {
    const int col = col0 + wv * kTile + gr;
#pragma unroll
    for (int m = 0; m < CH; ++m) {
      float e[4];
#pragma unroll
      for (int k = 0; k < 4; ++k) {
        const int row = 16 * m + 4 * gq + k;
        e[k] = (row < M && col < D) ? Wb[(size_t)row * D + col] : 0.0f;
      }
      wt[m] = make_float4(e[0], e[1], e[2], e[3]);
    }
  }
  constexpr bool kPk = L2O_GEMV_PK != 0;
  l2o::f32x4 wrq[2][NWH], wtq[CH];
#pragma unroll
  for (int m = 0; m < NWH; ++m) { wrq[0][m] = as_quad(wr[0][m]); wrq[1][m] = as_quad(wr[1][m]); }
#pragma unroll
  for (int m = 0; m < CH; ++m) wtq[m] = as_quad(wt[m]);
  const int myrow = (2 * wv + (gq & 1)) * kTile + gr;
  const float myy = (gq < 2 && myrow < M) ? pp.y[(size_t)b * M + myrow] : 0.0f;
  const bool row_counted = gq < 2 && (half == 0 ? (myrow < NC) : (myrow >= NC));

  using Core = LstmCorePair<PRE, !EXACT, false>;
  Core core;
  core.load(a.np.wpack, lane);
  core.pin();
  __shared__ __attribute__((aligned(16))) float bias_s[Core::kBiasFloats];
  core.stage_bias(bias_s, a.np.wpack, tid, blockDim.x, q);
  L2O_LAUNCH_MARK(1);
  const int j = tile_in_prob * kTile + c;
  const bool live = j < D;
  const size_t idx = (size_t)b * D + j;
  const int tpp = (D + kTile - 1) / kTile;
  const bool tile_real = tile_in_prob < tpp;
  TileState s;
  float* st_tile = a.st + ((size_t)b * tpp + (tile_real ? tile_in_prob : 0)) * kStateFloatsPerTile;
  if (tile_real && !a.zero_state) load_tile_state(s, st_tile, lane);
  else {
#pragma unroll
    for (int t = 0; t < kNT; ++t) s.h1[t] = s.c1[t] = s.h2[t] = s.c2[t] = 0.0f;
  }
  float xv = live ? (a.x_in ? a.x_in : a.x)[idx] : 0.0f;
  const float sc = (live && pp.x_scale) ? pp.x_scale[idx] : 1.0f;
  float cj = 0.0f;
  constexpr bool kCos = KIND == L2O_PROB_RASTRIGIN || KIND == L2O_PROB_SQUARE_COS;
  if (kCos) cj = live ? pp.C[idx] : 0.0f;
  float mv = 0.0f, vv = 0.0f;
  if (PRE == L2O_PRE_FC_ELU && !a.zero_state) { mv = live ? a.m[idx] : 0.0f; vv = live ? a.v[idx] : 0.0f; }
  float p1h = a.p1_hi, p1l = a.p1_lo, p2h = a.p2_hi, p2l = a.p2_lo;
  constexpr bool kSq = KIND == L2O_PROB_QUADRATIC || KIND == L2O_PROB_SQUARE_COS;
  const float coef = kSq ? 1.0f : 0.5f;
  const float cg = (KIND == L2O_PROB_QUADRATIC ? 2.0f : 1.0f) * pp.inv_bg;
  const float kTwoPi = pp.twopi;
  const float* xsq = xs + 4 * gq;
  const float* rsq = rs + 4 * gq;
  unsigned long long* mine = pa.xbuf + ((size_t)bl * 2 + half) * 2 * SQ;
  const unsigned long long* theirs = pa.xbuf + ((size_t)bl * 2 + (half ^ 1)) * 2 * SQ;
  bool dead = false;
  if (pa.ws->fault != 0) {
    dead = true;
    if (tid == 0) atomicExch(&pa.ws->status, 1u);
  }
  L2O_LAUNCH_MARK_LANDED(2);
  __shared__ __attribute__((aligned(16))) int same_xcd_s4[4];
  int& same_xcd_s = same_xcd_s4[0];
  if (tid == 0) {
    unsigned my_xcc;
    asm volatile("s_getreg_b32 %0, hwreg(HW_REG_XCC_ID)" : "=s"(my_xcc));
    my_xcc &= 0xfu;
    const unsigned kHsTag = 0x80000000u | salt | 0xffffu;
    __hip_atomic_store(mine + SQ, ((unsigned long long)kHsTag << 32) | my_xcc, __ATOMIC_RELAXED, __HIP_MEMORY_SCOPE_AGENT);
    unsigned long long g = 0;
    int spins = 0;
    bool ok = true;
#pragma nounroll
    for (;;) {
      g = __hip_atomic_load(theirs + SQ, __ATOMIC_RELAXED, __HIP_MEMORY_SCOPE_AGENT);
      if ((unsigned)(g >> 32) == kHsTag) break;
      if (dead || ++spins > (1 << 20)) { ok = false; break; }
      __builtin_amdgcn_s_sleep(1);
    }
    same_xcd_s = ok && pa.plain_stores && ((unsigned)g & 0xfu) == my_xcc;
  }
  __syncthreads();
  const bool same_xcd = same_xcd_s != 0;
  L2O_LAUNCH_MARK(3);

  constexpr bool kBiasRegs = kPairBiasRegs<PRE, KIND, CH, HIST, EXACT, false>;
#define L2O_PAIR_FX_PTR 0
#include "l2o_unroll_pair_loop.h"
#undef L2O_PAIR_FX_PTR
}

template <int PRE, int KIND, int CH, bool HIST, bool EXACT>
__device__ __forceinline__ void unroll_pair_body(const UnrollPairArgs& pa) {
  const long long kernel_t0 = __builtin_readcyclecounter();
#ifdef L2O_PROFILE_PHASES
  unsigned launch_marks[8] = {0, 0, 0, 0, 0, 0, 0, 0};
#endif
  constexpr int SQ = 16 * CH;
  constexpr int NWH = CH / 2;
  constexpr int NC = 16 * NWH;
  __shared__ __attribute__((aligned(16))) float xs[NC];
  __shared__ __attribute__((aligned(16))) float rs[SQ];
  const UnrollArgs& a = pa.u;
  const ProbParams& pp = a.pp;
  const int D = pp.D, M = pp.M;
  const int tid = threadIdx.x, lane = tid & 63, wv = tid >> 6;
  const int c = lane & 15, q = lane >> 4;
  const int bid = blockIdx.x;
  const int half = (bid >> 3) & 1;
  const int bl = ((bid >> 4) << 3) | (bid & 7);
  if (bl >= pa.nb) return;
  const int b = pa.b0 + bl;
  const int tile_in_prob = half * NWH + wv;
  const int gq = q, gr = c;

  using Core = LstmCorePair<PRE, !EXACT, true>;
  constexpr bool kStage = Core::kStageFrags > 0 && NWH >= 2;
  __shared__ float4 frag_stage[kStage ? Core::kStageFrags * 64 : 1];
  static_assert(sizeof(frag_stage) + sizeof(float) * (NC + SQ + Core::kBiasFloats + 4) <= 64 * 1024, "static LDS");
  if constexpr (kStage) {
    const int wvs = __builtin_amdgcn_readfirstlane(wv);
    const float* src = a.np.wpack + Core::kStageOff + lane * 4;
#pragma unroll
    for (int f = 0; f < (Core::kStageFrags + NWH - 1) / NWH; ++f) {
      const int fr = NWH * f + wvs;
      if (Core::kStageFrags % NWH == 0 || fr < Core::kStageFrags)
        __builtin_amdgcn_global_load_lds((gbl_void*)(src + fr * bx::kFragWords), (lds_void*)(frag_stage + fr * 64), 16, 0, 0);
    }
  }

  const float* Wb = pp.W + (pp.w_shared ? (size_t)0 : (size_t)b * M * D);
  const int col0 = half * NC;
  float4 wr[2][NWH], wt[CH];
  if (pa.fast_load && M == SQ && D == SQ && (reinterpret_cast<size_t>(pp.W) & 15) == 0) {
    const float4* Wq = reinterpret_cast<const float4*>(Wb + (size_t)(2 * wv * kTile + gr) * SQ + col0 + 4 * gq);
#pragma unroll
    for (int p = 0; p < 2; ++p)
#pragma unroll
      for (int m = 0; m < NWH; ++m) wr[p][m] = Wq[(p * kTile * SQ + 16 * m) / 4];
    const float* Wc = Wb + (size_t)(4 * gq) * SQ + col0 + wv * kTile + gr;
#pragma unroll
    for (int m = 0; m < CH; ++m)
      wt[m] = make_float4(Wc[(16 * m + 0) * SQ], Wc[(16 * m + 1) * SQ], Wc[(16 * m + 2) * SQ], Wc[(16 * m + 3) * SQ]);
  } else {
#pragma unroll
    for (int p = 0; p < 2; ++p) {
      const int row = (2 * wv + p) * kTile + gr;
#pragma unroll
      for (int m = 0; m < NWH; ++m) {
        float e[4];
#pragma unroll
        for (int k = 0; k < 4; ++k) {
          const int col = col0 + 16 * m + 4 * gq + k;
          e[k] = (row < M && col < D) ? Wb[(size_t)row * D + col] : 0.0f;
        }
        wr[p][m] = make_float4(e[0], e[1], e[2], e[3]);
      }
    }
    const int col = col0 + wv * kTile + gr;
#pragma unroll
    for (int m = 0; m < CH; ++m) {
      float e[4];
#pragma unroll
      for (int k = 0; k < 4; ++k) {
        const int row = 16 * m + 4 * gq + k;
        e[k] = (row < M && col < D) ? Wb[(size_t)row * D + col] : 0.0f;
      }
      wt[m] = make_float4(e[0], e[1], e[2], e[3]);
    }
  }
  unsigned hdr_lane = 0;
  asm volatile("" : "+v"(hdr_lane));
  const unsigned* hdr = &pa.ws->seq + hdr_lane;
  const unsigned seq_v = hdr[0], fault_v = hdr[1];
  static_assert(offsetof(PairWs, fault) == offsetof(PairWs, seq) + sizeof(unsigned), "seq and fault are neighbours");
  const int myrow = (2 * wv + (gq & 1)) * kTile + gr;
  const float y_ld = pp.y[(size_t)b * M + (myrow < M ? myrow : 0)];
  const bool row_counted = gq < 2 && (half == 0 ? (myrow < NC) : (myrow >= NC));
  const int j = tile_in_prob * kTile + c;
  const bool live = j < D;
  const size_t idx = (size_t)b * D + j;
  const size_t idx_ld = (size_t)b * D + (live ? j : 0);
  const int tpp = (D + kTile - 1) / kTile;
  const bool tile_real = tile_in_prob < tpp;
  float* st_tile = a.st + ((size_t)b * tpp + (tile_real ? tile_in_prob : 0)) * kStateFloatsPerTile;
  float4 st_ld[5];
  fetch_tile_state(st_ld, st_tile, lane);
  const float x_ld = (a.x_in ? a.x_in : a.x)[idx_ld];
  float sc_ld = 1.0f;
  if (pp.x_scale) sc_ld = pp.x_scale[idx_ld];
  constexpr bool kCos = KIND == L2O_PROB_RASTRIGIN || KIND == L2O_PROB_SQUARE_COS;
  float cj_ld = 0.0f;
  if (kCos) cj_ld = pp.C[idx_ld];
  float m_ld = 0.0f, v_ld = 0.0f;
  if (PRE == L2O_PRE_FC_ELU && !a.zero_state) { m_ld = a.m[idx_ld]; v_ld = a.v[idx_ld]; }

  Core core;
  float bias_ld[kStage ? (Core::kBiasFloats + 64 * NWH - 1) / (64 * NWH) : 1];
  if constexpr (kStage) {
    core.load_small(a.np.wpack, lane);
    core.template fetch_bias<64 * NWH>(bias_ld, a.np.wpack, tid);
    asm volatile("" ::"s"(a.zero_state));
  } else
    core.load(a.np.wpack, lane);
  __builtin_amdgcn_sched_barrier(0);
  L2O_LAUNCH_MARK(1);

  if constexpr (kStage) {
    L2O_LAUNCH_MARK_LANDED(2);
    asm volatile("s_waitcnt vmcnt(0)" ::: "memory");
  }
  const unsigned seq_w = __builtin_amdgcn_readfirstlane(seq_v), fault_w = __builtin_amdgcn_readfirstlane(fault_v);
  const unsigned salt = pa.use_salt ? ((seq_w + 1u) & 0x7fffu) << 16 : 0u;
  unsigned long long* mine = pa.xbuf + ((size_t)bl * 2 + half) * 2 * SQ;
  const unsigned long long* theirs = pa.xbuf + ((size_t)bl * 2 + (half ^ 1)) * 2 * SQ;
  const unsigned kHsTag = 0x80000000u | salt | 0xffffu;
  unsigned my_xcc = 0;
  if (tid == 0) {
    asm volatile("s_getreg_b32 %0, hwreg(HW_REG_XCC_ID)" : "=s"(my_xcc));
    my_xcc &= 0xfu;
    __hip_atomic_store(mine + SQ, ((unsigned long long)kHsTag << 32) | my_xcc, __ATOMIC_RELAXED, __HIP_MEMORY_SCOPE_AGENT);
  }
  L2O_LAUNCH_MARK(0);
  __builtin_amdgcn_sched_barrier(0);
  __shared__ __attribute__((aligned(16))) float bias_s[Core::kBiasFloats];
  if constexpr (kStage) core.template put_bias<64 * NWH>(bias_s, bias_ld, tid, q);
  else core.stage_bias(bias_s, a.np.wpack, tid, 64 * NWH, q);
  if constexpr (kStage) {
    asm volatile("s_waitcnt lgkmcnt(0)" ::: "memory");
    __builtin_amdgcn_s_barrier();
    asm volatile("" ::: "memory");
    core.read_stage(frag_stage, lane);
    __builtin_amdgcn_sched_barrier(0);
  } else
    core.pin();
  constexpr bool kPk = L2O_GEMV_PK != 0;
  l2o::f32x4 wrq[2][NWH], wtq[CH];
#pragma unroll
  for (int m = 0; m < NWH; ++m) { wrq[0][m] = as_quad(wr[0][m]); wrq[1][m] = as_quad(wr[1][m]); }
#pragma unroll
  for (int m = 0; m < CH; ++m) wtq[m] = as_quad(wt[m]);
  TileState s;
  unpack_tile_state(s, st_ld);
  if (!(tile_real && !a.zero_state)) {
#pragma unroll
    for (int t = 0; t < kNT; ++t) s.h1[t] = s.c1[t] = s.h2[t] = s.c2[t] = 0.0f;
  }
  const float myy = (gq < 2 && myrow < M) ? y_ld : 0.0f;
  float xv = live ? x_ld : 0.0f;
  const float sc = live ? sc_ld : 1.0f;
  const float cj = live ? cj_ld : 0.0f;
  float mv = live ? m_ld : 0.0f, vv = live ? v_ld : 0.0f;
  float p1h = a.p1_hi, p1l = a.p1_lo, p2h = a.p2_hi, p2l = a.p2_lo;
  constexpr bool kSq = KIND == L2O_PROB_QUADRATIC || KIND == L2O_PROB_SQUARE_COS;
  const float coef = kSq ? 1.0f : 0.5f;
  const float cg = (KIND == L2O_PROB_QUADRATIC ? 2.0f : 1.0f) * pp.inv_bg;
  const float kTwoPi = pp.twopi;
  const float* xsq = xs + 4 * gq;
  const float* rsq = rs + 4 * gq;
  bool dead = false;
  if (fault_w != 0) {
    dead = true;
    if (tid == 0) atomicExch(&pa.ws->status, 1u);
  }
  if constexpr (!kStage) L2O_LAUNCH_MARK_LANDED(2);
  __shared__ __attribute__((aligned(16))) int same_xcd_s4[4];
  int& same_xcd_s = same_xcd_s4[0];
  if (tid == 0) {
    unsigned long long g = 0;
    int spins = 0;
    bool ok = true;
#pragma nounroll
    for (;;) {
      g = __hip_atomic_load(theirs + SQ, __ATOMIC_RELAXED, __HIP_MEMORY_SCOPE_AGENT);
      if ((unsigned)(g >> 32) == kHsTag) break;
      if (dead || ++spins > (1 << 20)) { ok = false; break; }
      __builtin_amdgcn_s_sleep(1);
    }
    same_xcd_s = ok && pa.plain_stores && ((unsigned)g & 0xfu) == my_xcc;
  }
  __syncthreads();
  const bool same_xcd = same_xcd_s != 0;
  if constexpr (kStage) core.pin();
  L2O_LAUNCH_MARK(3);

  constexpr bool kBiasRegs = kPairBiasRegs<PRE, KIND, CH, HIST, EXACT, true>;
#define L2O_PAIR_FX_PTR 1
#include "l2o_unroll_pair_loop.h"
#undef L2O_PAIR_FX_PTR
}

template <int PRE, int KIND, int CH, bool HIST, bool EXACT = false, bool FAST = false>
__global__ __launch_bounds__(256) void k_unroll_pair(UnrollPairArgs pa) {
  if constexpr (FAST) unroll_pair_body<PRE, KIND, CH, HIST, EXACT>(pa);
  else unroll_pair_body_gather<PRE, KIND, CH, HIST, EXACT>(pa);
}
```

open_l2o_amd/csrc/l2o_unroll_pair_loop.h:

```cpp
  f32x4 acc1[kNT], acc2[kNT];
  core.init(s, q);
  if constexpr (kBiasRegs) {
    core.hold_bias();
    core.arm(acc1, acc2);
  } else
    core.preload(acc1, acc2);
  PhaseClock pc;
  pc.start();

  xs[wv * kTile + c] = live ? xv * sc : 0.0f;
  const size_t hist_n = (size_t)pp.B_local * D;
  const bool pub_plain = gq < 2 && same_xcd;
  unsigned poll_salt = salt | (dead ? 0x80000000u : 0u);
#ifdef L2O_ABLATE_EXCHANGE
  poll_salt = salt | 0x80000000u;
#endif
#if L2O_PAIR_FX_PTR
  float* fxp = pa.fx_half + (size_t)bl * (2 * NWH) + half * NWH + wv;
  const size_t fx_stride = (size_t)pa.nb * (2 * NWH);
#endif
  L2O_LAUNCH_MARK(4);
  const long long loop_t0 = __builtin_readcyclecounter();
  if constexpr (!HIST) {
    for (int t = 0; t < a.T; ++t) {
#include "l2o_unroll_pair_step_head.h"
#include "l2o_unroll_pair_step_tail.h"
    }
    {
      const int t = a.T;
#include "l2o_unroll_pair_step_head.h"
    }
  } else
  for (int t = 0;; ++t) {
#include "l2o_unroll_pair_step_head.h"
    if (t == a.T && !HIST) break;
#include "l2o_unroll_pair_step_tail.h"
  }
  L2O_LAUNCH_MARK(5);
#ifdef L2O_PROFILE_PHASES
  if (blockIdx.x == 0 && tid == 0) pc.dump(pa.ws->phases);
#endif
  if (bid == 0 && tid == 0) pa.ws->ticks = __builtin_readcyclecounter() - loop_t0;

  if (live && q == 0) {
    a.x[idx] = xv;
    if (PRE == L2O_PRE_FC_ELU) { a.m[idx] = mv; a.v[idx] = vv; }
  }
  if (tile_real) store_tile_state(s, st_tile, lane);
  if (bid == 0 && tid == 0) pa.ws->ticks_total = __builtin_readcyclecounter() - kernel_t0;
  L2O_LAUNCH_MARK(6);
  L2O_LAUNCH_MARK_LANDED(7);
#ifdef L2O_PROFILE_PHASES
  if (bid == 0 && tid == 0) {
#pragma unroll
    for (int i = 0; i < 8; ++i) pa.ws->pad[i] = launch_marks[i];
  }
#endif
```

open_l2o_amd/csrc/l2o_util_kernels.h:

```cpp
#pragma once
#include "l2o_bwd_mfma.h"
#include "l2o_unroll_pair.h"

__global__ void k_state_repack(float* __restrict__ h1, float* __restrict__ c1, float* __restrict__ h2,
                               float* __restrict__ c2, float* __restrict__ st, int B, int D, int tpp,
                               int to_packed) {
  const size_t gid = (size_t)blockIdx.x * blockDim.x + threadIdx.x;
  const size_t total = (size_t)B * tpp * 64 * 20;
  if (gid >= total) return;
  const int e = gid % 20;
  const int lane = (gid / 20) % 64;
  const size_t tile = gid / (20 * 64);
  const int b = tile / tpp, tw = tile % tpp;
  const int c = lane & 15, q = lane >> 4;
  const int j = tw * kTile + c;
  const int arr = e / 5, t = e % 5, u = 4 * t + q;
  const size_t paddr = tile * kStateFloatsPerTile + ((size_t)(e >> 2) * 64 + lane) * 4 + (e & 3);
  float* ref = arr == 0 ? h1 : (arr == 1 ? c1 : (arr == 2 ? h2 : c2));
  if (j < D) {
    const size_t raddr = ((size_t)b * D + j) * kH + u;
    if (to_packed) st[paddr] = ref[raddr];
    else ref[raddr] = st[paddr];
  } else if (to_packed) {
    st[paddr] = 0.0f;
  }
}

__global__ void k_reduce_fx(const float* __restrict__ fx_part, int T1, int B_local, float inv_bg,
                            float* __restrict__ fx) {
  const int t = blockIdx.x;
  const int lane = threadIdx.x;
  float acc = 0.0f;
  for (int b = lane; b < B_local; b += 64) acc += fx_part[(size_t)t * B_local + b];
  acc = wave_sum64(acc);
  if (lane == 0) fx[t] = acc * inv_bg;
}

__global__ __launch_bounds__(256) void k_combine_halves(const float* __restrict__ fx_half, float* __restrict__ fx_part,
                                                        int nb, int nparts, float inv_bg, float* __restrict__ fx,
                                                        unsigned long long* __restrict__ xbuf, long xwords, PairWs* ws,
                                                        int b0, int B_local) {
  const int t = blockIdx.x, tid = threadIdx.x, lane = tid & 63;
  if (tid >= 64) {
    const long npairs = xwords >> 1;
    const long per2 = (npairs + gridDim.x - 1) / gridDim.x;
    const long lo = (long)t * per2, hi = lo + per2 < npairs ? lo + per2 : npairs;
    ulonglong2* xpair = reinterpret_cast<ulonglong2*>(xbuf);
    for (long e = lo + (tid - 64); e < hi; e += 192) xpair[e] = make_ulonglong2(0ull, 0ull);
    return;
  }
  const bool bump = t == 0 && tid == 0;
  unsigned seq0 = 0;
  if (bump) seq0 = ws->seq;
  float acc = 0.0f;
  if (nb <= 128 && (nparts == 2 || nparts == 4 || nparts == 8)) {
    const int bA = lane, bB = lane + 64;
    const bool hA = bA < nb, hB = bB < nb;
    const float* pA = fx_half + ((size_t)t * nb + (hA ? bA : 0)) * nparts;
    const float* pB = fx_half + ((size_t)t * nb + (hB ? bB : 0)) * nparts;
    float fA, fB;
    if (nparts == 8) {
      const float4 a0 = *reinterpret_cast<const float4*>(pA), a1 = *reinterpret_cast<const float4*>(pA + 4);
      const float4 c0 = *reinterpret_cast<const float4*>(pB), c1 = *reinterpret_cast<const float4*>(pB + 4);
      fA = ((a0.x + a0.y) + a0.z) + a0.w;
      fA = (((fA + a1.x) + a1.y) + a1.z) + a1.w;
      fB = ((c0.x + c0.y) + c0.z) + c0.w;
      fB = (((fB + c1.x) + c1.y) + c1.z) + c1.w;
    } else if (nparts == 4) {
      const float4 a0 = *reinterpret_cast<const float4*>(pA), c0 = *reinterpret_cast<const float4*>(pB);
      fA = ((a0.x + a0.y) + a0.z) + a0.w;
      fB = ((c0.x + c0.y) + c0.z) + c0.w;
    } else {
      const float2 a0 = *reinterpret_cast<const float2*>(pA), c0 = *reinterpret_cast<const float2*>(pB);
      fA = a0.x + a0.y;
      fB = c0.x + c0.y;
    }
    if (hA) { fx_part[(size_t)t * B_local + b0 + bA] = fA; acc += fA; }
    if (hB) { fx_part[(size_t)t * B_local + b0 + bB] = fB; acc += fB; }
  } else {
    for (int b = lane; b < nb; b += 64) {
      const float* p = fx_half + ((size_t)t * nb + b) * nparts;
      float f = p[0];
      for (int k = 1; k < nparts; ++k) f += p[k];
      fx_part[(size_t)t * B_local + b0 + b] = f;
      acc += f;
    }
  }
  if (fx) {
    acc = l2o::wave_sum64(acc);
    if (lane == 0) fx[t] = acc * inv_bg;
  }
  if (bump) {
    if (xwords & 1) xbuf[xwords - 1] = 0ull;
    ws->seq = seq0 + 1u;
  }
}

__global__ __launch_bounds__(256) void k_coresident_probe(unsigned* ctr, unsigned* min_seen) {
  extern __shared__ float probe_lds[];
  if (threadIdx.x == 0) {
    probe_lds[0] = 1.0f;
    atomicAdd(ctr, 1u);
    for (int i = 0; i < 8; ++i) __builtin_amdgcn_s_sleep(127);
    const unsigned v = __hip_atomic_load(ctr, __ATOMIC_RELAXED, __HIP_MEMORY_SCOPE_AGENT);
    atomicMin(min_seen, v);
  }
}

extern "C" {
__host__ __device__ static inline uint16_t bf16_rne(float f) {
  uint32_t u = __builtin_bit_cast(uint32_t, f);
  u += 0x7fffu + ((u >> 16) & 1u);
  return (uint16_t)(u >> 16);
}
__host__ __device__ static inline double bf16_value(uint16_t h) {
  return (double)__builtin_bit_cast(float, (uint32_t)h << 16);
}
__host__ __device__ static inline void bf16_split3(double v, uint16_t (&out)[3]) {
  for (int s = 0; s < 3; ++s) {
    out[s] = bf16_rne((float)v);
    v -= bf16_value(out[s]);
  }
}

__host__ __device__ static void wpack_lane(int pre, int l, int t_lo, int t_hi, int tile_lo, int tile_hi,
                                           const float* wg1, const float* bg1, const float* wg2,
                                           const float* bg2, const float* wl, const float* bl, const float* wfc,
                                           const float* bfc, float* out, int ch_lo = 0, int ch_hi = 4, int r_lo = 0,
                                           int r_hi = 4) {
  const bool fc = pre == L2O_PRE_FC_ELU;
  const int P = fc ? kH : (pre == L2O_PRE_LOGSIGN ? 2 : 1);
  const int G = 4 * kH;
  auto col = [](int t, int rho) { return (rho & 3) * kH + 4 * t + (rho >> 2); };
  const int rho = l & 15, kq = l >> 4;
  const int q = l >> 4;
  for (int t = t_lo; t < t_hi && ch_lo == 0; ++t) {
    const int cA = col(t, rho);
    if (fc) {
      for (int kk = 0; kk < 10; ++kk) {
        const int row = kk < 5 ? 4 * kk + kq : kH + 4 * (kk - 5) + kq;
        out[(wp_row_a1(pre) + kk * kNT + t) * 64 + l] = wg1[row * G + cA];
      }
    } else {
      for (int kk = 0; kk < 5; ++kk)
        out[(wp_row_a1(pre) + kk * kNT + t) * 64 + l] = wg1[(P + 4 * kk + kq) * G + cA];
      float v = 0.0f;
      if (kq == 0) v = wg1[0 * G + cA];
      else if (kq == 1) v = P == 2 ? wg1[1 * G + cA] : 0.0f;
      else if (kq == 2) v = bg1[cA];
      out[(wp_row_a1(pre) + 5 * kNT + t) * 64 + l] = v;
    }
    for (int kk = 0; kk < 10; ++kk) {
      const int row = kk < 5 ? 4 * kk + kq : kH + 4 * (kk - 5) + kq;
      out[(wp_row_a2(pre) + kk * kNT + t) * 64 + l] = wg2[row * G + cA];
    }
    for (int r = 0; r < 4; ++r) {
      const int cD = col(t, 4 * q + r);
      out[(wp_row_b1(pre) + t * 4 + r) * 64 + l] = fc ? bg1[cD] : 0.0f;
      out[(wp_row_b2(pre) + t * 4 + r) * 64 + l] = bg2[cD];
    }
    out[(wp_row_wl(pre) + t) * 64 + l] = wl[4 * t + q];
    if (fc) {
      out[(wp_row_fc(pre) + t) * 64 + l] = wfc[0 * kH + 4 * t + q];
      out[(wp_row_fc(pre) + kNT + t) * 64 + l] = wfc[1 * kH + 4 * t + q];
      out[(wp_row_fc(pre) + 2 * kNT + t) * 64 + l] = bfc[4 * t + q];
    }
  }
  if (t_lo == 0 && t_hi > 0 && ch_lo == 0) out[wp_row_bl(pre) * 64 + l] = bl[0];
  {
    uint32_t* ow = reinterpret_cast<uint32_t*>(out);
    constexpr double kL2E = 1.4426950408889634074;
    auto gscale = [&](int r) { return r == 1 ? 2.0 * kL2E : -kL2E; };
    for (int t = t_lo; t < t_hi; ++t) {
      const int cA = col(t, rho), r = rho & 3;
      for (int ch = ch_lo; ch < ch_hi && ch < bx::nchunks(pre); ++ch) {
        uint16_t sl[5][3], bs[3] = {0, 0, 0};
        for (int i = 0; i < 5; ++i) {
          const int u = 4 * i + kq;
          double v;
          if (ch == bx::kChL1H) v = wg1[(P + u) * G + cA];
          else if (ch == bx::kChL2A) v = wg2[u * G + cA];
          else if (ch == bx::kChL2B) v = wg2[(kH + u) * G + cA];
          else v = wg1[u * G + cA];
          bf16_split3(v * gscale(r), sl[i]);
        }
        for (int sp = 0; sp < 3; ++sp)
          for (int rg = 0; rg < 4; ++rg) {
            auto slot = [&](int i) -> uint32_t { return i < 5 ? sl[i][sp] : (i == 7 && kq == 0 ? bs[sp] : 0); };
            ow[bx::frag_off(pre, false, ch, t, sp) + l * 4 + rg] = slot(2 * rg) | (slot(2 * rg + 1) << 16);
          }
        {
          for (int j = 0; j < bx::kPack; ++j)
            for (int rg = 0; rg < 4; ++rg) {
              uint32_t word = 0;
              for (int h = 0; h < 2; ++h) {
                const bx::SlotDesc d = bx::slot_desc(j, rg, h);
                uint16_t v16 = 0;
                if (d.unit < 5) v16 = sl[d.unit][d.w];
                else if (bx::bias_level(kq, h) >= 0) v16 = bs[bx::bias_level(kq, h)];
                word |= (uint32_t)v16 << (16 * h);
              }
              ow[bx::frag_off(pre, true, ch, t, j) + l * 4 + rg] = word;
            }
        }
      }
      if (ch_lo != 0) continue;
      if ((l & 15) == 0)
        for (int rr = 0; rr < 4; ++rr) {
          const int cD = col(t, 4 * q + rr);
          const double fb = rr == 2 ? 1.0 : 0.0;
          out[bx::bias_off(pre) + ((0 * kNT + t) * 4 + q) * 4 + rr] = (float)(((double)bg1[cD] + fb) * gscale(rr));
          out[bx::bias_off(pre) + ((1 * kNT + t) * 4 + q) * 4 + rr] = (float)(((double)bg2[cD] + fb) * gscale(rr));
        }
      if (!fc)
        for (int rr = 0; rr < 4; ++rr) {
          const int cD = col(t, 4 * q + rr);
          out[bx::win_off(pre) + t * 256 + l * 4 + rr] = (float)((double)wg1[0 * G + cD] * gscale(rr));
          out[bx::win_off(pre) + (kNT + t) * 256 + l * 4 + rr] =
              P == 2 ? (float)((double)wg1[1 * G + cD] * gscale(rr)) : 0.0f;
        }
    }
  }
  {
    uint32_t* ow = reinterpret_cast<uint32_t*>(out) + bxb::base(pre);
    for (int tile = tile_lo; tile < tile_hi; ++tile) {
      const bool l2 = tile < bxb::tiles2();
      const int m = l2 ? tile : tile - bxb::tiles2();
      const float* W = l2 ? wg2 : wg1;
      const int first = l2 ? 0 : (fc ? 0 : -1), second = l2 ? kH : (fc ? kH : P);
      const int row = bxb::src_row(m, rho, first, second);
      if (row < 0) continue;
      for (int r = r_lo; r < r_hi; ++r) {
        uint16_t sl[8][3];
        for (int i = 0; i < 8; ++i)
          for (int sp = 0; sp < 3; ++sp) sl[i][sp] = 0;
        for (int i = 0; i < 5; ++i) bf16_split3((double)W[row * G + r * kH + 4 * i + kq], sl[i]);
        for (int sp = 0; sp < 3; ++sp)
          for (int j = 0; j < 4; ++j)
            ow[bxb::frag_rel(tile, r, sp) + l * 4 + j] = (uint32_t)sl[2 * j][sp] | ((uint32_t)sl[2 * j + 1][sp] << 16);
      }
    }
  }
}

__global__ void k_wpack(int pre, const float* wg1, const float* bg1, const float* wg2, const float* bg2, const float* wl,
                        const float* bl, const float* wfc, const float* bfc, float* out) {
  const int b = blockIdx.x, nch = bx::nchunks(pre);
  if (b < kNT * nch) {
// ... 24 lines not shown
```

open_l2o_amd/meta.py:

```python
from __future__ import annotations

import collections
import os

import numpy as np
import torch

from . import _abi, _engine, networks
from ._engine import ProblemDesc
from ._graph_adam import AdamMixin
from ._graph_bptt import BpttMixin
from ._graph_core import (Fetch, Placeholder, Variable, PackedState, _make_nets, _DEFAULT_CONFIG, _DevGrad, _LazyHost,
                          _term_vars, _world, _all_reduce, synced_scale, local_slice, _Slot, set_random_seed, rng, _RngBox)
from ._graph_steps import StepPlanMixin, is_sampled, is_multivar

MetaLoss = collections.namedtuple("MetaLoss", "loss, update, reset, fx, x")
MetaStep = collections.namedtuple("MetaStep", "step, update, reset, fx, x")
_LaunchBuffers = collections.namedtuple("_LaunchBuffers", "scales step0 xs states ms vs descs panels")
_LaunchOpts = collections.namedtuple("_LaunchOpts", "commit recovering restart fold fast use_graph")


def _copy_all(dst, src):
    if hasattr(torch, "_foreach_copy_") and len(dst) > 1:
        torch._foreach_copy_(dst, src)
# ... 183 lines not shown
    def _rerun(self, feed, commit, restart, off):
        self._reuse_minibatches = True
        try:
            with _abi.option_scope({opt: 0 for opt in off}):
                return self.launch(feed, commit, restart=restart, _recovering=True)
        finally:
            self._reuse_minibatches = False

    def _wants_snapshot(self, restart_fused):
        if restart_fused or os.environ.get("L2O_NO_RECOVERY") or not hasattr(self.engine, "last_unroll_exchanges"):
            return False
        if self.__dict__.get("_last_launch", {}).get("restart") is not None:
            return False
        return self.__dict__.get("_exchanges", True)

    def _reduce_status(self):
        eng = self.engine
        if not (self.sharded and hasattr(eng, "unroll_status_tensor")):
            return None
        stw = eng.unroll_status_tensor() if self.last_path in ("fused", "mlp_unroll") else None
        red = self.__dict__.get("_status_red")
        if red is None:
            red = self._status_red = torch.zeros(1, dtype=torch.int32, device=eng.device)
        if stw is None:
            red.zero_()
        else:
            red.copy_(stw)
        _all_reduce(red, op="MAX")
        if stw is not None:
            stw.copy_(red)
        return red

    def _sync_or_recover(self, fx, xs, feed, commit):
        eng = self.engine
        self.wait_fx()
        has_status = hasattr(eng, "check_unroll_status")
        fused = self.last_path in ("fused", "mlp_unroll") and has_status
        red = self._reduce_status() if has_status else None
        if fused and hasattr(eng, "prefetch_unroll_status"):
            eng.prefetch_unroll_status()
        fx_host = eng.to_numpy(fx)
        if not fused and red is None:
            return fx_host, fx, xs
        if fused and hasattr(eng, "last_unroll_exchanges"):
            self._exchanges = bool(eng.last_unroll_exchanges())
        try:
            if fused:
                self._check_unroll_status()
            if red is not None and int(red[0]):
                raise _abi.L2OPartnerTimeout(_abi.L2O_ERR_TIMEOUT, "a peer rank's unroll reported a partner timeout")
        except _abi.L2OPartnerTimeout as err:
            info = self.__dict__.get("_last_launch", {})
            other = getattr(eng, "_deferred_graph", None)
            other = other() if other is not None else None
            if other is not None and other is not self and other.__dict__.get("_guarded_pending", 0):
                other._take_back_pending()
                raise
            can = not os.environ.get("L2O_NO_RECOVERY") and (info.get("restart") is not None or info.get("snapshot")
                                                             or not info.get("commit", True))
            if red is not None:
                flag = torch.full((1,), 1 if can else 0, dtype=torch.int32, device=eng.device)
                _all_reduce(flag, op="MIN")
                can = bool(int(flag[0]))
            if not can:
                raise
            import warnings
            warnings.warn("open_l2o_amd: %s -- re-running this unroll on the exchange-free kernels" % (err,), RuntimeWarning)
            self.recoveries = self.__dict__.get("recoveries", 0) + 1
            if info.get("restart") is None and info.get("snapshot"):
                self._restore_snapshot()
            fx, xs = self._rerun(feed, commit, info.get("restart"), (_abi.OPT_PAIR, _abi.OPT_MLP_UNROLL))
            self.wait_fx()
            fx_host = eng.to_numpy(fx)
            self._check_unroll_status()
        return fx_host, fx, xs

    def deterministic(self):
        return all(not is_sampled(t.kind) for t in self.terms)

    def execute_many(self, n):
        assert n >= 1
        if not self.deterministic():
            return self._execute_many_sampled(n)
        L = self.len_unroll
        self.len_unroll = n * L
        try:
            feed = {self.step: 1} if self.rnnprop else {}
            fx, xs = self.launch(feed, commit=True)
            fx_host, _, _ = self._sync_or_recover(fx, xs, feed, True)
        finally:
            self.len_unroll = L
        return [np.float32(fx_host[(k + 1) * L]) for k in range(n)]

    def many_ok(self):
        if self.deterministic():
            return True
        self._ensure_init()
        eng = self.engine
        if not hasattr(eng, "prepared_mlp_fg") or os.environ.get("L2O_NO_STEP_PLAN") or self.sharded:
            return False
        states = [s.state for s in self.slots]
        return self._plan_ok(self.slots, states, len(self.x))

    def launch(self, feed=None, commit=True, events=None, use_graph=False, record=None, restart=None, _recovering=False):
        self._ensure_init()
        T, feed = self.len_unroll, feed or {}
        if not _recovering:
            self._last_launch = {"restart": restart if (restart is not None and commit and record is None) else None,
                                 "snapshot": False, "commit": bool(commit)}
        out, fast = self._replay_prepared(feed, commit, events, record, restart, _recovering)
        if out is not None:
            return out
        fold = restart is not None and commit and record is None and len(self.x) == 1 and hasattr(self.engine, "mlp_unroll")
        if restart is not None and not fold:
            self.rewind(restart)
        b = self._launch_buffers(feed, commit)
        ring = self._fx_ring(T)
        path = self.last_path = self._choose_path(record, T, b)
        if fold and path != "fused":
            self.rewind(restart)
            fold = False
        rotate = path == "fused" and record is None
        i = ring["i"] if rotate else 0
        ring["i"] = (i + 1) % len(ring["bufs"]) if rotate else 0
        self._claim_fx(ring, i)
        fx = ring["bufs"][i]
        if events is not None:
            events[0].record()
        if record is not None:
            record.update(step0=b.step0, shapes=[tuple(pn.shape) for pn in b.panels])
            if self.second_derivatives:
                record["x"] = []
                record["descs"] = b.descs
        getattr(self, "_path_" + path)(b, T, fx, record, _LaunchOpts(commit, _recovering, restart, fold, fast, use_graph))
        if events is not None:
            events[1].record()
        if self.sharded:
            self._queue_fx(ring, i)
        if commit:
            for s, st in zip(self.slots, b.states):
                s.state = st
        return fx, b.xs

    def _replay_prepared(self, feed, commit, events, record, restart, recovering):
        eng, T = self.engine, self.len_unroll
        if not (commit and record is None and events is None and len(self.x) == 1 and len(self.slots) == 1
                and hasattr(eng, "prepared_unroll") and all(ph not in feed for ph in self.scale)
                and isinstance(self.slots[0].state, PackedState) and self.slots[0].state.packed is not None
                and (not self.rnnprop or self.step in feed)):
            return None, None
        s0 = self.slots[0]
        objs = (None if restart is None else restart[0], self.x[0].value, s0.state.packed, s0.m, s0.v,
                getattr(s0.net, "_wpack", None)) + tuple(v.value for v in self.constants)
        key = (T, restart is not None, _abi.options_word()) + tuple(id(o) for o in objs)
        ent = self.__dict__.setdefault("_fast_unrolls", {}).get(key)
        if ent is not None:
            if restart is None and not recovering and self._wants_snapshot(False):
                self._snapshot(self.slots)
            ring = self._fx_cache[T]
            i = ring["i"]
            ring["i"] = (i + 1) % len(ring["bufs"])
            self._claim_fx(ring, i)
            fx = ring["bufs"][i]
            if ent["call"](fx, int(feed[self.step]) if self.rnnprop else 1):
                self.last_path = "fused"
                if self.sharded:
                    self._queue_fx(ring, i)
                return (fx, [self.x[0].value]), None
            self._fast_unrolls.pop(key, None)
        return None, (key, objs)

    def _register_prepared(self, fast, b, T, fx_part, x0v, fold):
        s, d = self.slots[0], b.descs[0]
        fu = self._fast_unrolls
        if len(fu) >= 16:
            fu.pop(next(iter(fu)))
        call = self.engine.prepared_unroll(s.net.spec, s.net.wpack(self.engine), d, b.panels[0], b.states[0].packed, b.ms[0],
                                           b.vs[0], T, fx_part, x0v, fold)
        if call is not None and getattr(s.net, "_wpack", None) is fast[1][5]:
            fu[fast[0]] = {"call": call, "keep": fast[1]}

    def _launch_buffers(self, feed, commit):
        eng = self.engine
        scales = []
        sbufs = self.__dict__.setdefault("_scale_bufs", {})
        for ph, var in zip(self.scale, self.x):
            ent = None
            if ph in feed:
                src = feed[ph]
                ent = sbufs.get(var.decl.name)
                if ent is None or ent[0] is not src:
                    new = eng.tensor(var._local(src).reshape(self._panel_shape(var)))
                    if ent is not None and ent[1].shape == new.shape:
                        ent[1].copy_(new)
                        new = ent[1]
                    ent = sbufs[var.decl.name] = (src, new)
            scales.append(None if ent is None else ent[1])
        step0 = self._step0(feed)
        xs = [v.value if commit else v.value.clone() for v in self.x]
        states, ms, vs = [], [], []
        for s in self.slots:
            states.append(s.state.clone() if isinstance(s.state, (PackedState, networks.KernelState)) and not commit
                          else s.state)
            ms.append(s.m if (commit or s.m is None) else s.m.clone())
            vs.append(s.v if (commit or s.v is None) else s.v.clone())
        multivar = [is_multivar(self.term_of[v.decl.name].kind) for v in self.x]
        descs = [None if mv else self._desc(v, sc) for v, sc, mv in zip(self.x, scales, multivar)]
        panels = [xv.view(*self._panel_shape(var)) for xv, var in zip(xs, self.x)]
        self._mlp_scales = [sc if mv else None for sc, mv in zip(scales, multivar)]
        return _LaunchBuffers(scales, step0, xs, states, ms, vs, descs, panels)

    def _step0(self, feed):
        if self.rnnprop and self.step not in feed:
            raise ValueError("You must feed a value for placeholder 'step' (DM/util.py:59-60)")
        return int(feed[self.step]) if self.rnnprop else 1

    def _choose_path(self, record, T, b):
        slots, env = self.slots, os.environ
        if record is None:
            if self._fused_ok(b.descs):
                return "fused"
            if self._mlp_unroll_ok(slots, b.states, b.scales):
                return "mlp_unroll"
        elif not self.second_derivatives:
            if T > 0 and self._fused_ok(b.descs, record=True) and isinstance(b.states[0], PackedState) \
                    and b.states[0].packed is not None:
                return "fused"
            if not env.get("L2O_NO_MLP_UNROLL_RECORD") and \
                    self._mlp_unroll_ok(slots, b.states, b.scales) >= (1 if env.get("L2O_MLP_UNROLL_RECORD_GENERIC") else 2):
                return "mlp_unroll"
        return "confocal_unroll" if self._confocal_unroll_ok(slots, b.states) else "steps"

    def _path_fused(self, b, T, fx, record, o):
        eng, s, d, panel = self.engine, self.slots[0], b.descs[0], b.panels[0]
        fx_part = self._scratch("fx_part", (T + 1) * d.B_local)
        if record is not None:
            fp = self._fused_hist_plan(T, panel, b.states[0].packed)
            eng.unroll(s.net.spec, s.net.wpack(eng), d, panel, b.states[0].packed, b.ms[0], b.vs[0], T, b.step0, fx_part,
                       hist=fp["hist"], fx=fx)
            record.update(g=fp["g"], st=fp["st"], m=fp["m"], v=fp["v"], g_final=fp["g_final"], plan=fp)
            return
        x0v = o.restart[0].view(panel.shape) if o.fold else None
        if o.commit and not o.recovering and self._wants_snapshot(o.fold):
            self._snapshot(self.slots)
        eng.unroll(s.net.spec, s.net.wpack(eng), d, panel, b.states[0].packed, b.ms[0], b.vs[0], T, b.step0, fx_part, fx=fx,
                   x0=x0v, zero_state=o.fold)
        if o.fast is not None and (o.restart is None or o.fold) and d.x_scale is None:
            self._register_prepared(o.fast, b, T, fx_part, x0v, o.fold)

    def _path_mlp_unroll(self, b, T, fx, record, o):
        self._draw_minibatches(T)
        if record is None and o.commit and not o.recovering and self._wants_snapshot(False):
            self._snapshot(self.slots)
        self._run_fused_unroll("mlp", T, b.step0, b.panels, self.slots, b.states, b.ms, b.vs, b.scales, fx, record=record)

    def _path_confocal_unroll(self, b, T, fx, record, o):
        self._run_fused_unroll("confocal", T, b.step0, b.panels, self.slots, b.states, b.ms, b.vs, b.scales, fx, record=record)

    def _path_steps(self, b, T, fx, record, o):
        self._draw_minibatches(T)
        args = (T, b.step0, b.descs, b.panels, self.slots, b.states, b.ms, b.vs, fx)
        if record is None:
            self._run_steps_graphed(o.use_graph and o.commit and all(sc is None for sc in b.scales), *args)
        else:
            self._run_steps(*args, record=record)

    def _run_steps_graphed(self, wanted, T, step0, descs, panels, slots, states, ms, vs, fx):
        graphable = (wanted and all(isinstance(st, PackedState) for st in states) and hasattr(torch.cuda, "CUDAGraph")
                     and self.engine.device.type == "cuda")
        if not graphable:
            self._run_steps(T, step0, descs, panels, slots, states, ms, vs, fx)
        else:
            cache = self.__dict__.setdefault("_hip_graphs", {})
            entry = cache.get(step0)
            if entry is None:
                self._run_steps(T, step0, descs, panels, slots, states, ms, vs, fx)
                cache[step0] = "warm"
            else:
                if entry == "warm":
                    g = torch.cuda.CUDAGraph()
                    with torch.cuda.graph(g):
                        self._run_steps(T, step0, descs, panels, slots, states, ms, vs, fx)
                    cache[step0] = entry = g
                entry.replay()

    FX_RING = 64

    def _claim_fx(self, ring, i):
        if i in ring.get("pending", ()):
            self._flush_fx(ring)
        if ring["work"][i] is not None:
            ring["work"][i].wait()
            ring["work"][i] = None

    def _queue_fx(self, ring, i):
        ring["pending"].append(i)
        if len(ring["pending"]) >= len(ring["bufs"]) - 1:
            self._flush_fx(ring)

    def _flush_fx(self, ring):
        pend = sorted(ring.get("pending", ()))
        ring["pending"] = []
        k = 0
        while k < len(pend):
            e = k
            while e + 1 < len(pend) and pend[e + 1] == pend[e] + 1:
                e += 1
            w = _all_reduce(ring["store"][pend[k]:pend[e] + 1], async_op=True)
            for j in range(k, e + 1):
                ring["work"][pend[j]] = w
            k = e + 1

    def wait_fx(self):
        for ring in self._fx_cache.values():
            if ring.get("pending"):
                self._flush_fx(ring)
            done = set()
            for k, w in enumerate(ring["work"]):
                if w is not None:
                    if id(w) not in done:
                        w.wait()
                        done.add(id(w))
                    ring["work"][k] = None

    def train_step(self, feed, commit, learning_rate, defer=False):
        record = {}
        fx, xs = self.launch(feed, commit, record=record)
        eng, T = self.engine, self.len_unroll
        grads = self._backward(T, record)
        self.wait_fx()
        fused = self.last_path in ("fused", "mlp_unroll") and hasattr(eng, "check_unroll_status")
        early = all(self._device_adam(self.nets[k]) for k in grads)
        if self.sharded and hasattr(eng, "check_unroll_status"):
            self._reduce_status()
        if early:
            self._adam_apply(grads, learning_rate, guarded=fused)
        pend = self.__dict__.setdefault("_guarded_pending", 0)
        if defer and early:
            self._guarded_pending = pend + (1 if fused else 0)
            if fused:
                import weakref
                eng._deferred_graph = weakref.ref(self)
            return self._result(None, xs)
        if fused and hasattr(eng, "prefetch_unroll_status"):
            eng.prefetch_unroll_status()
        fx_host = eng.to_numpy(fx)
        if fused:
            self._guarded_pending = pend + (1 if early else 0)
            self._check_unroll_status()
        self._guarded_pending = 0
        if not early:
            self._adam_apply(grads, learning_rate)
        return self._result(fx_host, xs)

    def _check_unroll_status(self):
        try:
            self.engine.check_unroll_status()
        except Exception:
            self._take_back_pending()
            raise

    def _take_back_pending(self):
        n = self.__dict__.get("_guarded_pending", 0)
        if n and "_adam" in self.__dict__:
            self.__dict__["_adam"]["t"] -= n
        self._guarded_pending = 0

    def gradients(self, feed=None):
        T = self.len_unroll
        self.len_unroll = 0
        feed = dict(feed or {})
        if self.rnnprop:
            feed.setdefault(self.step, 1)
        try:
            rec = {}
            self.launch(feed, commit=False, record=rec)
        finally:
            self.len_unroll = T
        return rec["g_final"]

    def rewind(self, x0):
        _copy_all(*self.rewind_lists(x0))

    def rewind_lists(self, x0):
        self._ensure_init()
        dst, src = [v.value for v in self.x], list(x0)
        zeros = self.__dict__.setdefault("_rewind_zeros", {})
        for t in self._state_tensors(self.slots):
            z = zeros.get(tuple(t.shape))
            if z is None or z.device != t.device:
                z = zeros[tuple(t.shape)] = torch.zeros_like(t)
            dst.append(t)
            src.append(z)
        return dst, src

    def _state_tensors(self, slots):
        ts = []
        for s in slots:
            if isinstance(s.state, PackedState) and s.state.packed is not None:
                ts.append(s.state.packed)
            elif isinstance(s.state, networks.KernelState):
                ts.append(s.state.buf)
            if s.m is not None:
                ts += [s.m, s.v]
        return ts

    def _local_shape(self, var):
        if self.sharded:
            return (self.shard[1] - self.shard[0],) + tuple(var.shape[1:])
        return var.shape

    def _scratch(self, name, n):
        buf = getattr(self, "_scr_" + name, None)
        if buf is None or buf.numel() < n:
            buf = self.engine.zeros(n)
            setattr(self, "_scr_" + name, buf)
        return buf[:n]


class MtUnroll(object):

    def __init__(self, graph, mti):
        self.graph, self.mti = graph, mti
        self.len_unroll = graph.len_unroll
        self.learning_rate = 0.01
        T = self.len_unroll
        self.keys = list(graph.net_keys)
        self.sizes = [int(sum(int(np.prod(graph.x[j].shape)) for j in subset)) for subset in graph.subsets]
        self.total = int(sum(self.sizes))
        for k in self.keys:
            if isinstance(graph.nets[k], networks.KernelDeepLSTM):
                raise NotImplementedError("imitation unrolls are not implemented for KernelDeepLSTM (net %r): they feed a "
                                          "flat [T, P] gradient sequence per subset, not filters" % (k,))
            if not isinstance(graph.nets[k], networks.StandardDeepLSTM):
                raise NotImplementedError("imitation unrolls are implemented for the LSTM optimizer networks")
        self.labels = [Placeholder("mt%d_label_subset%d" % (mti, j), (T, P)) for j, P in enumerate(self.sizes)]
        self.inputs = [Placeholder("mt%d_input_subset%d" % (mti, j), (T, P)) for j, P in enumerate(self.sizes)]
        self.state = None

    @property
    def engine(self):
        return self.graph.engine

    def reset(self):
        eng, g = self.engine, self.graph
        self.state, self.m, self.v = [], [], []
        for k, P in zip(self.keys, self.sizes):
            self.state.append(PackedState.zeros(eng, 1, P, g.nets[k].spec.layers))
            self.m.append(eng.zeros(1, P) if g.rnnprop else None)
            self.v.append(eng.zeros(1, P) if g.rnnprop else None)

    def _forward(self, feed, commit, record=None):
        eng, g = self.engine, self.graph
        if self.state is None:
            self.reset()
        T = self.len_unroll
        feed = feed or {}
        for ph in self.inputs + self.labels:
            if ph not in feed:
                raise ValueError("You must feed a value for placeholder %r" % (ph.name,))
        step0 = g._step0(feed)
        b1, b2 = float(np.float32(g.beta1)), float(np.float32(g.beta2))
        states = [st if commit else st.clone() for st in self.state]
        ms = [m if (commit or m is None) else m.clone() for m in self.m]
        vs = [v if (commit or v is None) else v.clone() for v in self.v]
        loss = eng.zeros(1)
# ... 157 lines not shown
```

Measured before the change: 10.78 billion.

## Defer per-unroll loss combine into a ring and batch-flush with one kernel

Adds a deferred-loss path for the two-CU pair unroll. Each unroll writes its per-half losses into a workspace ring slot and skips the per-call k_combine_halves launch. A single k_flush_halves launch later reduces many slots at once into the fx buffers, and the Python side triggers flushes on reads and status checks. This removes one kernel launch per unroll call, at the cost of a larger workspace, new sequence-word bookkeeping in the kernel, and more complex synchronisation logic.

```diff
diff --git a/include/l2o_abi.h b/include/l2o_abi.h
--- a/include/l2o_abi.h
+++ b/include/l2o_abi.h
@@ -105,6 +105,7 @@
 #define L2O_OPT_ONE_LDS 12
 #define L2O_OPT_PAIR_FAST_LOAD 13
 #define L2O_OPT_COUNT_ 14
+#define L2O_OPT_PAIR_DEFER_LOSS 14
 #define L2O_OPT_FIELD_(o) ((o) == L2O_OPT_ONE_LDS ? L2O_OPT_BWD_BLOCKS : (o) == L2O_OPT_PAIR_FAST_LOAD ? 15 : (o))
 #define L2O_OPTW(o, v) ((uint64_t)(8u | ((unsigned)(v) & 7u)) << (4 * L2O_OPT_FIELD_(o)))
 #define L2O_OPTW_BWD_BLOCKS(n) ((uint64_t)((n) > 4095 ? 4095 : (n)) << 48)
@@ -400,6 +401,16 @@
                       int32_t step0, int32_t flags, float* fx_part, float* fx , void* workspace,
                       const l2o_unroll_hist* hist, void* stream);
 int l2o_unroll_workspace_init(void* workspace, size_t bytes, void* stream);
+typedef int32_t L2O_UNROLL_DEFER_SLOTS_FN(const l2o_net_cfg* cfg, const l2o_problem* prob, int32_t T);
+typedef int L2O_UNROLL_DEFER_FN(const l2o_net_cfg* cfg, const float* wpack , const l2o_problem* prob,
+                                const float* x0 , float* x, float* st, float* m, float* v, int32_t T,
+                                int32_t step0, int32_t flags, void* workspace, int32_t slot, void* stream);
+typedef int L2O_UNROLL_FLUSH_FN(const l2o_net_cfg* cfg, const l2o_problem* prob, int32_t T, void* workspace, int32_t slot0,
+                                int32_t count, float* fx_base , int64_t fx_stride ,
+                                void* stream);
+L2O_UNROLL_DEFER_SLOTS_FN l2o_unroll_defer_slots;
+L2O_UNROLL_DEFER_FN l2o_unroll_defer;
+L2O_UNROLL_FLUSH_FN l2o_unroll_flush;
 int64_t l2o_unroll_workspace_layout(const l2o_net_cfg* cfg, const l2o_problem* prob);
 int l2o_unroll_status(const void* workspace_header_host );
 int l2o_unroll_supported(const l2o_net_cfg* cfg, const l2o_problem* prob);
diff --git a/open_l2o_amd/_abi.py b/open_l2o_amd/_abi.py
--- a/open_l2o_amd/_abi.py
+++ b/open_l2o_amd/_abi.py
@@ -25,6 +25,9 @@
 OPT_DEFAULTS = {OPT_PAIR: 1, OPT_PAIR_PLAIN_STORES: 1, OPT_UNROLL_CU: 1, OPT_FG_TWO_PASS: 0, OPT_MLP_GENERIC: 0,
                 OPT_BWD_BLOCKS: 0, OPT_BWD_KERNEL: 0, OPT_MLP_UNROLL: 1, OPT_MLP_XCD_WAVES: 0, OPT_EXACT_GATES: 0,
                 OPT_WPACK_NO_CLEAR: 0, OPT_MLP_HIER: 1, OPT_ONE_LDS: 1, OPT_PAIR_FAST_LOAD: 1}
+OPT_PAIR_DEFER_LOSS = 14
+OPT_DEFAULTS[OPT_PAIR_DEFER_LOSS] = 1
+HOST_OPTIONS = (OPT_PAIR_DEFER_LOSS,)
 FORM_NAMES = {1: "k_unroll", 2: "k_unroll_pair", 5: "k_unroll_lds", 6: "k_unroll_cu", 7: "k_unroll_cu8",
               8: "k_mlp_unroll (flat all-reduce)", 9: "k_mlp_unroll (XCD-hierarchical all-reduce)", 10: "k_mlp_unroll (generic loops)",
               11: "k_mlp_xcd (one optimizee instance per XCD)", 12: "k_cf_unroll (one workgroup per batch row)",
@@ -37,7 +40,7 @@
                 "fg_two_pass": OPT_FG_TWO_PASS, "mlp_generic": OPT_MLP_GENERIC, "bwd_blocks": OPT_BWD_BLOCKS,
                 "bwd_kernel": OPT_BWD_KERNEL, "mlp_unroll": OPT_MLP_UNROLL, "exact_gates": OPT_EXACT_GATES,
                 "mlp_hier": OPT_MLP_HIER, "one_lds": OPT_ONE_LDS, "mlp_xcd_waves": OPT_MLP_XCD_WAVES,
-                "pair_fast_load": OPT_PAIR_FAST_LOAD}
+                "pair_fast_load": OPT_PAIR_FAST_LOAD, "pair_defer_loss": OPT_PAIR_DEFER_LOSS}
 if os.environ.get("L2O_EXACT_GATES"):
     _options[OPT_EXACT_GATES] = 1
 for _item in filter(None, os.environ.get("L2O_OPTIONS", "").split(",")):
@@ -85,6 +88,8 @@
 def options_word():
     w = 0
     for o, v in _options.items():
+        if o in HOST_OPTIONS:
+            continue
         if o == OPT_BWD_BLOCKS:
             w |= (v & 0xfff) << 48
         else:
@@ -345,6 +350,19 @@
                                    "l2o_vgg16_abi.h", "l2o_nas_abi.h", "l2o_klstm_abi.h"))
 
 
+LATE_PROTOTYPES = {
+    "l2o_unroll_defer_slots": (C.c_int32, [C.POINTER(NetCfg), C.POINTER(Problem), C.c_int32]),
+    "l2o_unroll_defer": (C.c_int, [C.POINTER(NetCfg), C.c_void_p, C.POINTER(Problem)] + [C.c_void_p] * 5 +
+                         [C.c_int32] * 3 + [C.c_void_p, C.c_int32, C.c_void_p]),
+    "l2o_unroll_flush": (C.c_int, [C.POINTER(NetCfg), C.POINTER(Problem), C.c_int32, C.c_void_p, C.c_int32, C.c_int32,
+                                   C.c_void_p, C.c_int64, C.c_void_p]),
+}
+
+
+def has_deferred_unroll(library):
+    return all(hasattr(library, name) for name in LATE_PROTOTYPES)
+
+
 class L2OError(RuntimeError):
     def __init__(self, code, msg):
         super().__init__("libl2o_hip error %d: %s" % (code, msg))
@@ -404,6 +422,10 @@
         for name, (restype, argtypes) in protos.items():
             fn = getattr(library, name)
             fn.restype, fn.argtypes = restype, argtypes
+    for name, (restype, argtypes) in LATE_PROTOTYPES.items():
+        fn = getattr(library, name, None)
+        if fn is not None:
+            fn.restype, fn.argtypes = restype, argtypes
     return library
 
 
diff --git a/open_l2o_amd/_engine.py b/open_l2o_amd/_engine.py
--- a/open_l2o_amd/_engine.py
+++ b/open_l2o_amd/_engine.py
@@ -252,6 +252,9 @@
         return torch.empty(*shape, dtype=torch.float32, device=self.device)
 
     def to_numpy(self, t):
+        d = self.__dict__.get("_defer")
+        if d is not None and d["slots"]:
+            self.flush_unroll_losses()
         return t.detach().cpu().numpy()
 
     def _stream(self):
@@ -760,6 +763,7 @@
     def unroll(self, spec: NetSpec, wpack, p: ProblemDesc, x, st, m, v, T, step0, fx_part, hist=None, fx=None, x0=None,
                zero_state=False):
         assert fx is not None or (x0 is None and not zero_state)
+        self.flush_unroll_losses()
         cc, cp = spec.to_c(), self._cprob(p)
         nbytes = int(self.lib.l2o_unroll_workspace_bytes(C.byref(cc), C.byref(cp), int(T)))
         ws = None
@@ -802,18 +806,70 @@
         fn, check, stream = self.lib.l2o_unroll_reduce, _abi.check, self._stream
         keep = (cc, cp, wpack, p, x, st, m, v, fx_part, x0, ws)
         eng = self
-
-        def call(fx, step0=1, _keep=keep):
+        slots = 0
+        if ws is not None and _abi.get_option(_abi.OPT_PAIR_DEFER_LOSS) and _abi.has_deferred_unroll(self.lib):
+            slots = int(self.lib.l2o_unroll_defer_slots(C.byref(cc), C.byref(cp), int(T)))
+            cap = self.__dict__.get("defer_slots_cap")
+            if cap is not None:
+                slots = min(slots, int(cap))
+            if slots < 2:
+                slots = 0
+        defer_fn = self.lib.l2o_unroll_defer if slots else None
+        dkey = (layout, int(T), cp.B_global)
+
+        def call(fx, step0=1, slot=None, _keep=keep):
             if eng._workspace is not ws or (ws is not None and eng.__dict__.get("_ws_layout") != layout):
                 return False
-            rc = fn(*args_a, int(step0), *args_b, C.c_void_p(fx.data_ptr()), wsp, None, stream())
+            if slot is None:
+                eng.flush_unroll_losses()
+                rc = fn(*args_a, int(step0), *args_b, C.c_void_p(fx.data_ptr()), wsp, None, stream())
+            else:
+                if not 0 <= slot < slots:
+                    raise ValueError("prepared unroll: slot %r of %d" % (slot, slots))
+                d = eng.__dict__.get("_defer")
+                if d is not None and d["slots"] and (d["key"] != dkey or d["ws"] is not ws or slot in d["slots"]):
+                    eng.flush_unroll_losses()
+                    d = None
+                if d is None or d["key"] != dkey or d["ws"] is not ws:
+                    d = eng._defer = {"key": dkey, "ws": ws, "cc": cc, "cp": cp, "T": int(T), "slots": {}}
+                rc = defer_fn(*args_a, int(step0), flags, wsp, int(slot), stream())
+                if not rc:
+                    d["slots"][slot] = fx
             if rc:
                 check(rc)
             eng._last_ws = ws
             return True
+        call.defer_slots = slots
         return call
 
+    unroll_flushes = 0
+
+    def unroll_losses_pending(self, slot=None):
+        d = self.__dict__.get("_defer")
+        return bool(d is not None and d["slots"] and (slot is None or slot in d["slots"]))
+
+    def flush_unroll_losses(self):
+        d = self.__dict__.get("_defer")
+        if d is None or not d["slots"]:
+            return 0
+        pend, d["slots"] = d["slots"], {}
+        order, n, k = sorted(pend), 0, 0
+        wsp, esz = C.c_void_p(d["ws"].data_ptr()), 4
+        while k < len(order):
+            base, e, stride = pend[order[k]].data_ptr(), k, 0
+            while e + 1 < len(order) and order[e + 1] == order[e] + 1:
+                step = pend[order[e + 1]].data_ptr() - pend[order[e]].data_ptr()
+                if step % esz or step < esz * (d["T"] + 1) or (stride and step != stride):
+                    break
+                stride, e = step, e + 1
+            _abi.check(self.lib.l2o_unroll_flush(C.byref(d["cc"]), C.byref(d["cp"]), d["T"], wsp, int(order[k]), e - k + 1,
+                                                 C.c_void_p(base), (stride // esz) if stride else d["T"] + 1, self._stream()))
+            n, k = n + 1, e + 1
+        self.unroll_flushes = self.unroll_flushes + n
+        return n
+
     def prefetch_unroll_status(self):
+        self.flush_unroll_losses()
         ws = self._last_ws
         if ws is None:
             return
@@ -849,6 +905,7 @@
                 ws[8:12].view(torch.int32).fill_(1 if on else 0)
 
     def check_unroll_status(self):
+        self.flush_unroll_losses()
         ws = self._last_ws
         if ws is not None:
             if self.__dict__.pop("_status_pending", None) is ws:
diff --git a/open_l2o_amd/csrc/l2o_unroll.hip b/open_l2o_amd/csrc/l2o_unroll.hip
--- a/open_l2o_amd/csrc/l2o_unroll.hip
+++ b/open_l2o_amd/csrc/l2o_unroll.hip
@@ -11,6 +11,8 @@
 __global__ void k_combine_halves(const float* __restrict__ fx_half, float* __restrict__ fx_part, int nb, int nparts,
                                  float inv_bg, float* __restrict__ fx, unsigned long long* __restrict__ xbuf, long xwords,
                                  PairWs* ws, int b0, int B_local);
+__global__ void k_flush_halves(const float* __restrict__ ring, long slot_floats, int nb, int nparts, float inv_bg,
+                               float* __restrict__ fx_base, long fx_stride, unsigned long long* __restrict__ xbuf, long xwords);
 __global__ void k_coresident_probe(unsigned* ctr, unsigned* min_seen);
 
 static int check_problem(const l2o_problem* p) {
@@ -54,24 +56,40 @@
   const int chunk = (((p->B_local + n - 1) / n) + 7) & ~7;
   return chunk <= cap ? chunk : (cap & ~7);
 }
-struct PairLayout { size_t xbuf_off, xbuf_bytes, fxh_off, total; int npg; size_t lds; };
-static PairLayout pair_layout(const l2o_problem* p, const UnrollGeom& g, int T) {
+static int defer_cap_cus() { return coresident_cus(nullptr); }
+struct PairLayout { size_t xbuf_off, xbuf_bytes, pseq_off, fxh_off, fxh_bytes, ring_off, total; int npg, slots; size_t lds; };
+static constexpr int kDeferMaxSlots = 64;
+static constexpr size_t kDeferMaxBytes = (size_t)32 << 20;
+static PairLayout pair_layout(const l2o_problem* p, const UnrollGeom& g, int T, int cap_cus) {
   PairLayout L;
   const int SQ = 16 * g.CH;
   L.npg = SQ;
   L.xbuf_off = sizeof(PairWs);
   L.xbuf_bytes = (size_t)p->B_local * 2 * 2 * L.npg * sizeof(unsigned long long);
-  L.fxh_off = L.xbuf_off + L.xbuf_bytes;
-  L.total = L.fxh_off + sizeof(float) * (size_t)(T + 1) * g.CH * p->B_local;
+  L.pseq_off = L.xbuf_off + L.xbuf_bytes;
+  L.fxh_off = L.pseq_off + (((size_t)p->B_local * sizeof(unsigned) + 15) & ~(size_t)15);
+  L.fxh_bytes = (sizeof(float) * (size_t)(T + 1) * g.CH * p->B_local + 15) & ~(size_t)15;
+  L.ring_off = L.fxh_off + L.fxh_bytes;
+  size_t slots = 0;
+  if (cap_cus > 0 && p->B_local <= cap_cus / 2 && L.fxh_bytes > 0) {
+    slots = kDeferMaxBytes / L.fxh_bytes;
+    if (slots > (size_t)kDeferMaxSlots) slots = kDeferMaxSlots;
+    if (slots < 2) slots = 0;
+  }
+  L.slots = (int)slots;
+  L.total = L.ring_off + slots * L.fxh_bytes;
   L.lds = 0;
   return L;
 }
 
 template <int PRE, int KIND>
 static int launch_unroll_ch(const UnrollArgs& a, const UnrollGeom& g, hipStream_t s, const l2o_problem* prob,
-                            void* workspace, float* fx, bool* fx_done) {
+                            void* workspace, float* fx, bool* fx_done, int defer_slot) {
+  const bool defer = defer_slot >= 0;
   const bool hist = a.hist_st != nullptr;
   int chunk = workspace ? pair_chunk(prob, g, s) : 0;
+  if (defer && (hist || chunk < a.pp.B_local))
+    return fail(L2O_ERR_UNSUPPORTED, "l2o_unroll_defer: not a single plain launch of the two-CU unroll (l2o_unroll_defer_slots)");
   {
     const int one_lds = (int)opt(L2O_OPT_ONE_LDS);
 #ifdef L2O_LDS_ABL_ANYNW
@@ -80,7 +98,7 @@
     const bool shape_ok = g.CH == 8 && g.nw >= 5;
 #endif
     const bool plain = !(opt(L2O_OPT_EXACT_GATES) && !hist);
-    if ((one_lds == 2 || (one_lds == 1 && (chunk == 0 || a.pp.B_local > chunk))) && shape_ok && plain) {
+    if (!defer && (one_lds == 2 || (one_lds == 1 && (chunk == 0 || a.pp.B_local > chunk))) && shape_ok && plain) {
       UnrollArgs al = a;
       al.ticks = workspace ? &reinterpret_cast<PairWs*>(workspace)->ticks : nullptr;
       void (*fl)(UnrollArgs) = hist ? k_unroll_lds<PRE, KIND, true> : k_unroll_lds<PRE, KIND, false>;
@@ -93,12 +111,15 @@
     }
   }
   if (chunk > 0) {
-    const PairLayout L = pair_layout(prob, g, a.T);
+    const PairLayout L = pair_layout(prob, g, a.T, defer_cap_cus());
+    if (defer && defer_slot >= L.slots)
+      return fail(L2O_ERR_ARG, "l2o_unroll_defer: slot %d of %d", defer_slot, L.slots);
     UnrollPairArgs pa;
     pa.u = a;
     pa.ws = reinterpret_cast<PairWs*>(workspace);
     pa.xbuf = reinterpret_cast<unsigned long long*>(static_cast<char*>(workspace) + L.xbuf_off);
-    pa.fx_half = reinterpret_cast<float*>(static_cast<char*>(workspace) + L.fxh_off);
+    pa.fx_half = reinterpret_cast<float*>(static_cast<char*>(workspace) +
+                                          (defer ? L.ring_off + (size_t)defer_slot * L.fxh_bytes : L.fxh_off));
     pa.use_salt = a.T + 1 < 0xffff ? 1u : 0u;
     pa.plain_stores = opt(L2O_OPT_PAIR_PLAIN_STORES) ? 1u : 0u;
     pa.b0 = 0;
@@ -129,6 +150,7 @@
         pa.nb = B - b0 < chunk ? B - b0 : chunk;
         hipLaunchKernelGGL(fn, dim3((pa.nb + 7) / 8 * 16), dim3(64 * (g.CH / 2)), dyn_lds, s, pa);
         HIP_TRY(hipGetLastError());
+        if (defer) break;
         hipLaunchKernelGGL(k_combine_halves, dim3(a.T + 1), dim3(256), 0, s, pa.fx_half, a.fx_part, pa.nb, g.CH,
                            a.pp.inv_bg, one_launch ? fx : nullptr, pa.xbuf, (long)pa.nb * 2 * 2 * L.npg, pa.ws, b0, B);
         HIP_TRY(hipGetLastError());
@@ -136,9 +158,10 @@
     }
     note_form(L2O_FORM_UNROLL_PAIR, (B + chunk - 1) / chunk);
     note_variant(g.CH, hist, exact, fast_launched, 0, 0);
-    if (fx_done) *fx_done = fx != nullptr && one_launch;
+    if (fx_done) *fx_done = (fx != nullptr && one_launch) || defer;
     return L2O_OK;
   }
+  if (defer) return fail(L2O_ERR_UNSUPPORTED, "l2o_unroll_defer: the two-CU unroll does not apply (l2o_unroll_defer_slots)");
   void (*fn)(UnrollArgs) = nullptr;
   const bool exact1 = opt(L2O_OPT_EXACT_GATES) != 0 && !hist;
   switch (g.CH) {
@@ -156,12 +179,12 @@
 
 template <int PRE>
 static int launch_unroll_kind(const UnrollArgs& a, const UnrollGeom& g, int kind, hipStream_t s,
-                              const l2o_problem* prob, void* workspace, float* fx, bool* fx_done) {
+                              const l2o_problem* prob, void* workspace, float* fx, bool* fx_done, int defer_slot) {
   switch (kind) {
-    case L2O_PROB_QUADRATIC: return launch_unroll_ch<PRE, L2O_PROB_QUADRATIC>(a, g, s, prob, workspace, fx, fx_done);
-    case L2O_PROB_LASSO: return launch_unroll_ch<PRE, L2O_PROB_LASSO>(a, g, s, prob, workspace, fx, fx_done);
-    case L2O_PROB_RASTRIGIN: return launch_unroll_ch<PRE, L2O_PROB_RASTRIGIN>(a, g, s, prob, workspace, fx, fx_done);
-    case L2O_PROB_SQUARE_COS: return launch_unroll_ch<PRE, L2O_PROB_SQUARE_COS>(a, g, s, prob, workspace, fx, fx_done);
+    case L2O_PROB_QUADRATIC: return launch_unroll_ch<PRE, L2O_PROB_QUADRATIC>(a, g, s, prob, workspace, fx, fx_done, defer_slot);
+    case L2O_PROB_LASSO: return launch_unroll_ch<PRE, L2O_PROB_LASSO>(a, g, s, prob, workspace, fx, fx_done, defer_slot);
+    case L2O_PROB_RASTRIGIN: return launch_unroll_ch<PRE, L2O_PROB_RASTRIGIN>(a, g, s, prob, workspace, fx, fx_done, defer_slot);
+    case L2O_PROB_SQUARE_COS: return launch_unroll_ch<PRE, L2O_PROB_SQUARE_COS>(a, g, s, prob, workspace, fx, fx_done, defer_slot);
     default: return fail(L2O_ERR_UNSUPPORTED, "no fused kernel for problem kind %d", kind);
   }
 }
@@ -327,7 +350,34 @@
   if (!l2o_unroll_supported(cfg, prob) || T < 0) return 0;
   UnrollGeom g;
   if (!unroll_geom(prob, &g) || g.CH < 2) return 0;
-  return pair_layout(prob, g, T).total;
+  return pair_layout(prob, g, T, defer_cap_cus()).total;
+}
+
+int32_t l2o_unroll_defer_slots(const l2o_net_cfg* cfg, const l2o_problem* prob, int32_t T) {
+  OptScope opt_scope(cfg_optw(cfg));
+  if (!l2o_unroll_supported(cfg, prob) || T < 0) return 0;
+  UnrollGeom g;
+  if (!unroll_geom(prob, &g) || g.CH < 2 || !opt(L2O_OPT_PAIR) || opt(L2O_OPT_ONE_LDS) == 2) return 0;
+  return pair_layout(prob, g, T, defer_cap_cus()).slots;
+}
+
+int l2o_unroll_flush(const l2o_net_cfg* cfg, const l2o_problem* prob, int32_t T, void* workspace, int32_t slot0,
+                     int32_t count, float* fx_base, int64_t fx_stride, void* stream) {
+  OptScope opt_scope(cfg_optw(cfg));
+  const int slots = l2o_unroll_defer_slots(cfg, prob, T);
+  if (!workspace || !fx_base || slot0 < 0 || count < 1 || slot0 + count > slots || fx_stride < T + 1)
+    return fail(L2O_ERR_ARG, "l2o_unroll_flush: bad argument (slot0=%d count=%d of %d slots)", slot0, count, slots);
+  UnrollGeom g;
+  unroll_geom(prob, &g);
+  const PairLayout L = pair_layout(prob, g, T, defer_cap_cus());
+  char* w = static_cast<char*>(workspace);
+  const int B = prob->B_local;
+  hipLaunchKernelGGL(k_flush_halves, dim3(T + 1, count), dim3(256), 0, (hipStream_t)stream,
+                     reinterpret_cast<const float*>(w + L.ring_off + (size_t)slot0 * L.fxh_bytes),
+                     (long)(L.fxh_bytes / sizeof(float)), B, g.CH, make_prob_params(prob).inv_bg, fx_base, (long)fx_stride,
+                     reinterpret_cast<unsigned long long*>(w + L.xbuf_off), (long)B * 2 * 2 * L.npg);
+  HIP_TRY(hipGetLastError());
+  return L2O_OK;
 }
 
 int l2o_unroll_status(const void* workspace_header_host) {
@@ -348,7 +398,8 @@
 
 static int unroll_impl(const l2o_net_cfg* cfg, const float* wpack, const l2o_problem* prob, float* x, float* st,
                        float* m, float* v, int32_t T, int32_t step0, float* fx_part, void* workspace,
-                       const l2o_unroll_hist* hist, float* fx, void* stream, const float* x0 = nullptr, int flags = 0);
+                       const l2o_unroll_hist* hist, float* fx, void* stream, const float* x0 = nullptr, int flags = 0,
+                       int defer_slot = -1);
 
 int l2o_unroll(const l2o_net_cfg* cfg, const float* wpack, const l2o_problem* prob, float* x, float* st, float* m,
                float* v, int32_t T, int32_t step0, float* fx_part, void* workspace, void* stream) {
@@ -371,6 +422,18 @@
   if (flags & ~L2O_UNROLL_ZERO_STATE)
     return fail(L2O_ERR_ARG, "l2o_unroll_reduce: unknown flags %d", flags);
   return unroll_impl(cfg, wpack, prob, x, st, m, v, T, step0, fx_part, workspace, hist, fx, stream, x0, flags);
+}
+
+int l2o_unroll_defer(const l2o_net_cfg* cfg, const float* wpack, const l2o_problem* prob, const float* x0, float* x,
+                     float* st, float* m, float* v, int32_t T, int32_t step0, int32_t flags, void* workspace, int32_t slot,
+                     void* stream) {
+  OptScope opt_scope(cfg_optw(cfg));
+  if (flags & ~L2O_UNROLL_ZERO_STATE) return fail(L2O_ERR_ARG, "l2o_unroll_defer: unknown flags %d", flags);
+  if (!workspace || slot < 0) return fail(L2O_ERR_ARG, "l2o_unroll_defer: NULL workspace / negative slot");
+  if (slot >= l2o_unroll_defer_slots(cfg, prob, T))
+    return fail(L2O_ERR_UNSUPPORTED, "l2o_unroll_defer: slot %d, but l2o_unroll_defer_slots = %d", slot,
+                l2o_unroll_defer_slots(cfg, prob, T));
+  return unroll_impl(cfg, wpack, prob, x, st, m, v, T, step0, nullptr, workspace, nullptr, nullptr, stream, x0, flags, slot);
 }
 
 int32_t l2o_coresident_workgroups(void* scratch, void* stream) {
@@ -419,10 +482,10 @@
 
 static int unroll_impl(const l2o_net_cfg* cfg, const float* wpack, const l2o_problem* prob, float* x, float* st,
                        float* m, float* v, int32_t T, int32_t step0, float* fx_part, void* workspace,
-                       const l2o_unroll_hist* hist, float* fx, void* stream, const float* x0, int flags) {
+                       const l2o_unroll_hist* hist, float* fx, void* stream, const float* x0, int flags, int defer_slot) {
   int rc = check_problem(prob);
   if (rc) return rc;
-  if (!cfg || !wpack || !x || !st || !fx_part || T < 0) return fail(L2O_ERR_ARG, "l2o_unroll: bad argument");
+  if (!cfg || !wpack || !x || !st || (!fx_part && defer_slot < 0) || T < 0) return fail(L2O_ERR_ARG, "l2o_unroll: bad argument");
   if (hist && (!hist->st || !hist->g || !hist->g_final ||
                (cfg->preprocess == L2O_PRE_FC_ELU && (!hist->m || !hist->v))))
     return fail(L2O_ERR_ARG, "l2o_unroll_record: incomplete history buffers");
@@ -450,10 +513,11 @@
   rc = L2O_OK;
   if (cfg->preprocess == L2O_PRE_FC_ELU && (!m || !v)) return fail(L2O_ERR_ARG, "l2o_unroll: RNNProp needs m and v");
   if (!lds_form) {
+    if (defer_slot >= 0) return fail(L2O_ERR_UNSUPPORTED, "l2o_unroll_defer: the two-CU unroll does not apply");
     rc = with_pre(cfg->preprocess, [&](auto pre) { return launch_unroll_cu<decltype(pre)::value>(a, s); });
   } else {
     rc = with_pre(cfg->preprocess, [&](auto pre) {
-      return launch_unroll_kind<decltype(pre)::value>(a, g, prob->kind, s, prob, workspace, fx, &fx_done);
+      return launch_unroll_kind<decltype(pre)::value>(a, g, prob->kind, s, prob, workspace, fx, &fx_done, defer_slot);
     });
   }
   if (rc) return rc;
diff --git a/open_l2o_amd/csrc/l2o_unroll_pair.h b/open_l2o_amd/csrc/l2o_unroll_pair.h
--- a/open_l2o_amd/csrc/l2o_unroll_pair.h
+++ b/open_l2o_amd/csrc/l2o_unroll_pair.h
@@ -24,6 +24,11 @@
   int b0, nb;
   unsigned fast_load;
 };
+
+template <int SQ>
+__device__ __forceinline__ unsigned* pair_seq_word(const UnrollPairArgs& pa, int b) {
+  return reinterpret_cast<unsigned*>(pa.xbuf + (size_t)pa.u.pp.B_local * (2 * 2 * SQ)) + b;
+}
 
 __device__ __forceinline__ unsigned long long pack_granule(float v, unsigned tag) {
   return ((unsigned long long)tag << 32) | (unsigned long long)__float_as_uint(v);
@@ -122,15 +127,16 @@
   const int tid = threadIdx.x, lane = tid & 63, wv = tid >> 6;
   const int c = lane & 15, q = lane >> 4;
   const int bid = blockIdx.x;
-  const unsigned salt = pa.use_salt ? ((pa.ws->seq + 1u) & 0x7fffu) << 16 : 0u;
-#ifdef L2O_PROFILE_PHASES
-  asm volatile("" ::"s"(salt));
-#endif
-  L2O_LAUNCH_MARK(0);
   const int half = (bid >> 3) & 1;
   const int bl = ((bid >> 4) << 3) | (bid & 7);
   if (bl >= pa.nb) return;
   const int b = pa.b0 + bl;
+  const unsigned seq_w = *pair_seq_word<SQ>(pa, b);
+  const unsigned salt = pa.use_salt ? ((seq_w + 1u) & 0x7fffu) << 16 : 0u;
+#ifdef L2O_PROFILE_PHASES
+  asm volatile("" ::"s"(salt));
+#endif
+  L2O_LAUNCH_MARK(0);
   const int tile_in_prob = half * NWH + wv;
   const int gq = q, gr = c;
 
@@ -326,9 +332,7 @@
   }
   unsigned hdr_lane = 0;
   asm volatile("" : "+v"(hdr_lane));
-  const unsigned* hdr = &pa.ws->seq + hdr_lane;
-  const unsigned seq_v = hdr[0], fault_v = hdr[1];
-  static_assert(offsetof(PairWs, fault) == offsetof(PairWs, seq) + sizeof(unsigned), "seq and fault are neighbours");
+  const unsigned seq_v = pair_seq_word<SQ>(pa, b)[hdr_lane], fault_v = (&pa.ws->fault)[hdr_lane];
   const int myrow = (2 * wv + (gq & 1)) * kTile + gr;
   const float y_ld = pp.y[(size_t)b * M + (myrow < M ? myrow : 0)];
   const bool row_counted = gq < 2 && (half == 0 ? (myrow < NC) : (myrow >= NC));
diff --git a/open_l2o_amd/csrc/l2o_unroll_pair_loop.h b/open_l2o_amd/csrc/l2o_unroll_pair_loop.h
--- a/open_l2o_amd/csrc/l2o_unroll_pair_loop.h
+++ b/open_l2o_amd/csrc/l2o_unroll_pair_loop.h
@@ -47,7 +47,10 @@
     if (PRE == L2O_PRE_FC_ELU) { a.m[idx] = mv; a.v[idx] = vv; }
   }
   if (tile_real) store_tile_state(s, st_tile, lane);
-  if (bid == 0 && tid == 0) pa.ws->ticks_total = __builtin_readcyclecounter() - kernel_t0;
+  if (tid == 0) {
+    if (bid == 0) pa.ws->ticks_total = __builtin_readcyclecounter() - kernel_t0;
+    if (half == 0) *pair_seq_word<SQ>(pa, b) = seq_w + 1u;
+  }
   L2O_LAUNCH_MARK(6);
   L2O_LAUNCH_MARK_LANDED(7);
 #ifdef L2O_PROFILE_PHASES
diff --git a/open_l2o_amd/csrc/l2o_util_kernels.h b/open_l2o_amd/csrc/l2o_util_kernels.h
--- a/open_l2o_amd/csrc/l2o_util_kernels.h
+++ b/open_l2o_amd/csrc/l2o_util_kernels.h
@@ -36,22 +36,9 @@
   if (lane == 0) fx[t] = acc * inv_bg;
 }
 
-__global__ __launch_bounds__(256) void k_combine_halves(const float* __restrict__ fx_half, float* __restrict__ fx_part,
-                                                        int nb, int nparts, float inv_bg, float* __restrict__ fx,
-                                                        unsigned long long* __restrict__ xbuf, long xwords, PairWs* ws,
-                                                        int b0, int B_local) {
-  const int t = blockIdx.x, tid = threadIdx.x, lane = tid & 63;
-  if (tid >= 64) {
-    const long npairs = xwords >> 1;
-    const long per2 = (npairs + gridDim.x - 1) / gridDim.x;
-    const long lo = (long)t * per2, hi = lo + per2 < npairs ? lo + per2 : npairs;
-    ulonglong2* xpair = reinterpret_cast<ulonglong2*>(xbuf);
-    for (long e = lo + (tid - 64); e < hi; e += 192) xpair[e] = make_ulonglong2(0ull, 0ull);
-    return;
-  }
-  const bool bump = t == 0 && tid == 0;
-  unsigned seq0 = 0;
-  if (bump) seq0 = ws->seq;
+template <bool PART>
+__device__ __forceinline__ float pair_loss_sum(const float* __restrict__ fx_half, float* __restrict__ fx_part, int t, int nb,
+                                               int nparts, int lane, int b0, int B_local) {
   float acc = 0.0f;
   if (nb <= 128 && (nparts == 2 || nparts == 4 || nparts == 8)) {
     const int bA = lane, bB = lane + 64;
@@ -75,17 +62,40 @@
       fA = a0.x + a0.y;
       fB = c0.x + c0.y;
     }
-    if (hA) { fx_part[(size_t)t * B_local + b0 + bA] = fA; acc += fA; }
-    if (hB) { fx_part[(size_t)t * B_local + b0 + bB] = fB; acc += fB; }
+    if (hA) { if (PART) fx_part[(size_t)t * B_local + b0 + bA] = fA; acc += fA; }
+    if (hB) { if (PART) fx_part[(size_t)t * B_local + b0 + bB] = fB; acc += fB; }
   } else {
     for (int b = lane; b < nb; b += 64) {
       const float* p = fx_half + ((size_t)t * nb + b) * nparts;
       float f = p[0];
       for (int k = 1; k < nparts; ++k) f += p[k];
-      fx_part[(size_t)t * B_local + b0 + b] = f;
+      if (PART) fx_part[(size_t)t * B_local + b0 + b] = f;
       acc += f;
     }
   }
+  return acc;
+}
+__device__ __forceinline__ void pair_zero_granules(unsigned long long* __restrict__ xbuf, long xwords, int t, int nblk, int tid) {
+  const long npairs = xwords >> 1;
+  const long per2 = (npairs + nblk - 1) / nblk;
+  const long lo = (long)t * per2, hi = lo + per2 < npairs ? lo + per2 : npairs;
+  ulonglong2* xpair = reinterpret_cast<ulonglong2*>(xbuf);
+  for (long e = lo + (tid - 64); e < hi; e += 192) xpair[e] = make_ulonglong2(0ull, 0ull);
+}
+
+__global__ __launch_bounds__(256) void k_combine_halves(const float* __restrict__ fx_half, float* __restrict__ fx_part,
+                                                        int nb, int nparts, float inv_bg, float* __restrict__ fx,
+                                                        unsigned long long* __restrict__ xbuf, long xwords, PairWs* ws,
+                                                        int b0, int B_local) {
+  const int t = blockIdx.x, tid = threadIdx.x, lane = tid & 63;
+  if (tid >= 64) {
+    pair_zero_granules(xbuf, xwords, t, gridDim.x, tid);
+    return;
+  }
+  const bool bump = t == 0 && tid == 0;
+  unsigned seq0 = 0;
+  if (bump) seq0 = ws->seq;
+  float acc = pair_loss_sum<true>(fx_half, fx_part, t, nb, nparts, lane, b0, B_local);
   if (fx) {
     acc = l2o::wave_sum64(acc);
     if (lane == 0) fx[t] = acc * inv_bg;
@@ -94,6 +104,20 @@
     if (xwords & 1) xbuf[xwords - 1] = 0ull;
     ws->seq = seq0 + 1u;
   }
+}
+
+__global__ __launch_bounds__(256) void k_flush_halves(const float* __restrict__ ring, long slot_floats, int nb, int nparts,
+                                                      float inv_bg, float* __restrict__ fx_base, long fx_stride,
+                                                      unsigned long long* __restrict__ xbuf, long xwords) {
+  const int t = blockIdx.x, k = blockIdx.y, tid = threadIdx.x, lane = tid & 63;
+  if (tid >= 64) {
+    if (k == 0) pair_zero_granules(xbuf, xwords, t, gridDim.x, tid);
+    return;
+  }
+  float acc = pair_loss_sum<false>(ring + (size_t)k * slot_floats, nullptr, t, nb, nparts, lane, 0, nb);
+  acc = l2o::wave_sum64(acc);
+  if (lane == 0) fx_base[(size_t)k * fx_stride + t] = acc * inv_bg;
+  if (t == 0 && k == 0 && tid == 0 && (xwords & 1)) xbuf[xwords - 1] = 0ull;
 }
 
 __global__ __launch_bounds__(256) void k_coresident_probe(unsigned* ctr, unsigned* min_seen) {
diff --git a/open_l2o_amd/meta.py b/open_l2o_amd/meta.py
--- a/open_l2o_amd/meta.py
+++ b/open_l2o_amd/meta.py
@@ -359,17 +359,18 @@
         s0 = self.slots[0]
         objs = (None if restart is None else restart[0], self.x[0].value, s0.state.packed, s0.m, s0.v,
                 getattr(s0.net, "_wpack", None)) + tuple(v.value for v in self.constants)
-        key = (T, restart is not None, _abi.options_word()) + tuple(id(o) for o in objs)
+        key = (T, restart is not None, _abi.options_word(), _abi.get_option(_abi.OPT_PAIR_DEFER_LOSS)) + tuple(id(o) for o in objs)
         ent = self.__dict__.setdefault("_fast_unrolls", {}).get(key)
         if ent is not None:
             if restart is None and not recovering and self._wants_snapshot(False):
                 self._snapshot(self.slots)
-            ring = self._fx_cache[T]
+            ring = ent.get("ring") or self._fx_cache[T]
             i = ring["i"]
             ring["i"] = (i + 1) % len(ring["bufs"])
             self._claim_fx(ring, i)
             fx = ring["bufs"][i]
-            if ent["call"](fx, int(feed[self.step]) if self.rnnprop else 1):
+            step0 = int(feed[self.step]) if self.rnnprop else 1
+            if ent["call"](fx, step0, i) if "ring" in ent else ent["call"](fx, step0):
                 self.last_path = "fused"
                 if self.sharded:
                     self._queue_fx(ring, i)
@@ -385,7 +386,20 @@
         call = self.engine.prepared_unroll(s.net.spec, s.net.wpack(self.engine), d, b.panels[0], b.states[0].packed, b.ms[0],
                                            b.vs[0], T, fx_part, x0v, fold)
         if call is not None and getattr(s.net, "_wpack", None) is fast[1][5]:
-            fu[fast[0]] = {"call": call, "keep": fast[1]}
+            fu[fast[0]] = ent = {"call": call, "keep": fast[1]}
+            slots = getattr(call, "defer_slots", 0)
+            if slots >= 2:
+                ent["ring"] = self._defer_ring(T, min(self.FX_RING, slots))
+
+    def _defer_ring(self, T, n):
+        ring = self._fx_cache.get(("defer", T))
+        if ring is None or len(ring["bufs"]) != n:
+            if ring is not None:
+                self.wait_fx()
+            store = self.engine.zeros(n, T + 1)
+            ring = self._fx_cache[("defer", T)] = {"store": store, "bufs": [store[k] for k in range(n)], "work": [None] * n,
+                                                   "i": 0, "pending": [], "defer": True}
+        return ring
 
     def _launch_buffers(self, feed, commit):
         eng = self.engine
@@ -496,6 +510,8 @@
     def _claim_fx(self, ring, i):
         if i in ring.get("pending", ()):
             self._flush_fx(ring)
+        elif ring.get("defer") and self.engine.unroll_losses_pending(i):
+            self.engine.flush_unroll_losses()
         if ring["work"][i] is not None:
             ring["work"][i].wait()
             ring["work"][i] = None
@@ -506,6 +522,7 @@
             self._flush_fx(ring)
 
     def _flush_fx(self, ring):
+        self._flush_losses()
         pend = sorted(ring.get("pending", ()))
         ring["pending"] = []
         k = 0
@@ -518,7 +535,13 @@
                 ring["work"][pend[j]] = w
             k = e + 1
 
+    def _flush_losses(self):
+        flush = getattr(self.engine, "flush_unroll_losses", None)
+        if flush is not None:
+            flush()
+
     def wait_fx(self):
+        self._flush_losses()
         for ring in self._fx_cache.values():
             if ring.get("pending"):
                 self._flush_fx(ring)
```

After: 10.87 billion, median of 6. No clear change (+0.9%).
